# zhang-tao-whu/DVIS_Plus

Measured on AMD Instinct MI355X. Metric: frames/sec DVIS++ R50 offline, 720p T=30 synthetic, higher is better.
Workload: dtype f32 (storage, accumulation, results; the segmenter's dense layers - R50 convolutions from 128 channels on, pixel-decoder projections and FPN output convolution, the deformable encoder's projections and FFN, the decoder's key / value projections - multiply each fp32 operand as two f16 terms on the f1

## Files before the change

dvis_plus_amd/csrc/conv1x1_x3.hip:

```cpp
#include "dvis_common.h"
#include "x3_common.h"

DVIS_EXPORT int64_t dvis_conv_x3_image_bytes(int64_t N, int C, int H, int W);
DVIS_EXPORT int dvis_conv_x3_gn_fold_supported(int K, int G, int64_t HW);

namespace {

constexpr unsigned kOOB = 0x80000000u;

struct CxArgs {
  const float *x, *bias, *res;
  const void *wp;
  float *y;
  int N, C, K, relu, npass;
  int stride, W_in, OW, H_in;
  int taps;
  long long HW, HW_in, pixels;
  long long tiles;
  float xscale, inv;
  int *flag;
  int tag;
  const float *x2;
  int C2, stride2, W2_in;
  long long HW2_in;
// ... 193 lines not shown
              hi4[e] = a.in_relu ? fmaxf(t1, 0.f) : t1;
            }
            asm volatile("" : "+v"(lo4), "+v"(hi4));
            __builtin_amdgcn_sched_barrier(0);
          }
          split8(lo4, hi4, a.xscale, xh[s], xl[s]);
        }
        if constexpr (kAffine)
          if (kc + 1 == NC && more) load_tab(ntile);
        if (++cc == NCC) cc = 0, ++tap;
        const bool first = kc + 1 < NC1, sec = !first && kc + 1 < NC;
        const unsigned po = first ? cx_tap_offset(a, gm, tap) : (sec ? gm2 : cx_tap_offset(a, ngm, 0));
        load_raw(po, first ? cc : (sec ? kc + 1 - NC1 : 0), sec);
      }
#pragma unroll
      for (int part = 0; part < IPC; ++part) {
        const char *stage = ring.wait(false);
        ring.begin(ring.more() ? next_offset() : 0);
        mma_item<IK, NB, PW>(stage, lane, acc, xh + IK * part, xl + IK * part, [&](int i) { ring.piece(i); });
      }
    }
    float chk = 0.f;
    if constexpr (NB == 2 || IMGOUT) {
      if (a.img != nullptr) {
        const unsigned gs = (unsigned)(a.K / 64) * 8192u;
        const __amdgpu_buffer_rsrc_t ri = dvis_make_rsrc_uniform(a.img, (unsigned)((long long)a.N * a.OH * a.XG * gs));
        const __amdgpu_buffer_rsrc_t rb = dvis_make_rsrc_uniform(a.bias ? (const void *)a.bias : (const void *)a.img, a.bias ? (unsigned)a.K * 4u : 0u);
        unsigned ibase = kOOB;
        if (p < a.pixels) {
          const int pix = (int)(p - n * a.HW), oy = pix / a.OW, ox = pix - oy * a.OW;
          ibase = (unsigned)(((n * a.OH + oy) * a.XG + (ox >> 5)) * gs + (co0 / 64) * 8192 + g * 512 + (ox & 31) * 16);
        }
#pragma unroll
        for (int nb = 0; nb < NB; ++nb) {
          float v[16];
#pragma unroll
          for (int q = 0; q < 4; ++q) {
            const f4 b = __builtin_bit_cast(f4, __builtin_amdgcn_raw_buffer_load_b128(rb, (unsigned)(co0 + 32 * nb + 8 * q + 4 * g) * 4u, 0, 0));
#pragma unroll
            for (int i = 0; i < 4; ++i) {
              const float t = acc[nb][4 * q + i] * a.inv + b[i];
              chk = __builtin_fmaf(t, 0.f, chk);
              v[4 * q + i] = a.relu ? x3_relu(t) : t;
            }
          }
          h8 hi[2], lo[2];
#pragma unroll
          for (int u = 0; u < 2; ++u) {
            const f4 p0 = {v[8 * u], v[8 * u + 1], v[8 * u + 2], v[8 * u + 3]}, p1 = {v[8 * u + 4], v[8 * u + 5], v[8 * u + 6], v[8 * u + 7]};
            split8(p0, p1, a.oscale, hi[u], lo[u]);
          }
          const h8 ls = lo[0] + lo[1];
          chk = __builtin_fmaf((float)((ls[0] + ls[1]) + (ls[2] + ls[3]) + (ls[4] + ls[5]) + (ls[6] + ls[7])), 0.f, chk);
          store_fragments4(ri, ibase, hi[0], 4096 * nb, lo[0], 4096 * nb + 1024, hi[1], 4096 * nb + 2048, lo[1], 4096 * nb + 3072);
        }
        if (a.flag != nullptr && chk != chk && p < a.pixels) atomicCAS(a.flag, 0, a.tag);
        tile = ntile, pass = npass_, gm = ngm, gm2 = ngm2;
        continue;
      }
    }
    double gw[8], gw2[4], gw4[2], gtot = 0.0;
#pragma unroll
    for (int nb = 0; nb < NB; ++nb) {
      float rv[16];
      double gq[4];
#pragma unroll
      for (int r = 0; r < 16; ++r)
        rv[r] = a.res ? __builtin_bit_cast(float, __builtin_amdgcn_raw_buffer_load_b32(
                                                      rr, obase + (unsigned)(co0 + 32 * nb + 8 * (r >> 2) + 4 * g + (r & 3)) * ochan, 0, 0))
                      : 0.f;
#pragma unroll
      for (int q = 0; q < 4; ++q) {
        const int co = co0 + 32 * nb + 8 * q + 4 * g;
        f4 b = {0.f, 0.f, 0.f, 0.f};
        if (a.bias) b = *(const f4 *)(a.bias + co);
        double gsum = 0.0, gsq = 0.0;
#pragma unroll
        for (int i = 0; i < 4; ++i) {
          const unsigned o = obase + (unsigned)(co + i) * ochan;
          float v = acc[nb][4 * q + i] * a.inv + b[i] + rv[4 * q + i];
          chk = __builtin_fmaf(v, 0.f, chk);
          if (a.relu) v = x3_relu(v);
          __builtin_amdgcn_raw_buffer_store_b32(__builtin_bit_cast(unsigned, v), ry, o, 0, 0);
          if constexpr (kStats) {
            const double d = p < a.pixels ? (double)v : 0.0;
            gsum = i == 0 ? d : gsum + d;
            gsq = i == 0 ? d * d : __builtin_fma(d, d, gsq);
          }
        }
        if constexpr (kStats) gq[q] = cx_fold<5>(gsum, gsq, lane);
      }
      if constexpr (kStats) {
        gw[nb] = cx_fold<3>(cx_fold<4>(gq[0], gq[1], lane), cx_fold<4>(gq[2], gq[3], lane), lane);
        if (nb % 2 == 1) gw2[nb / 2] = cx_fold<2>(gw[nb - 1], gw[nb], lane);
        if (nb % 4 == 3) gw4[nb / 4] = cx_fold<1>(gw2[nb / 2 - 1], gw2[nb / 2], lane);
        if (nb == NB - 1) gtot = cx_fold<0>(gw4[0], gw4[1], lane);
      }
    }
    if constexpr (kStats) {
      const long long pw = tile * kTile + wave * 32;
      if (pw < a.pixels) {
        const long long nw = pw / a.HW, slot = (pw - nw * a.HW) >> 5;
        const int group = co0 / 8 + 4 * (((lane >> 2) & 1) + 2 * ((lane >> 1) & 1) + 4 * (lane & 1)) + ((lane >> 4) & 1) + 2 * ((lane >> 3) & 1);
        a.gn_part[((nw * (a.K / 8) + group) * a.slots + slot) * 2 + (lane >> 5)] = gtot;
      }
    }
    if (a.flag != nullptr && chk != chk && p < a.pixels) atomicCAS(a.flag, 0, a.tag);
    tile = ntile, pass = npass_, gm = ngm, gm2 = ngm2;
  }
}

__global__ __launch_bounds__(256) void upsample_add_image_kernel(const float *__restrict__ lateral, const float *__restrict__ top,
                                                                 void *__restrict__ img, int N, int C, int H, int W, int h, int w,
                                                                 const float *__restrict__ lat_scale, const float *__restrict__ lat_shift,
                                                                 float oscale) {
  const int NCC = C / 64, XG = (W + 31) / 32;
  const int cc = blockIdx.x, xg = blockIdx.y;
  const int x = threadIdx.x & 31, g = (threadIdx.x >> 5) & 1, S = threadIdx.x >> 6;
  const int px = 32 * xg + x;
  const float sy = (float)h / (float)H, sx = (float)w / (float)W;
  const int pxc = px < W ? px : W - 1;
  float fx = sx * ((float)pxc + 0.5f) - 0.5f;
  fx = fx < 0.f ? 0.f : fx;
  const int x0 = min((int)fx, w - 1), x1 = x0 + (x0 < w - 1 ? 1 : 0);
  const float lx1 = fx - (float)x0, lx0 = 1.f - lx1;
  const __amdgpu_buffer_rsrc_t ri = dvis_make_rsrc_uniform(img, (unsigned)((long long)N * H * XG * NCC * 8192));
  const unsigned rows = (unsigned)N * (unsigned)H;
  for (unsigned row = blockIdx.z * 16u; row < blockIdx.z * 16u + 16u && row < rows; ++row) {
    const unsigned n = row / (unsigned)H;
    const int y = (int)(row - n * (unsigned)H);
    float fy = sy * ((float)y + 0.5f) - 0.5f;
    fy = fy < 0.f ? 0.f : fy;
    const int y0 = min((int)fy, h - 1), y1 = y0 + (y0 < h - 1 ? 1 : 0);
    const float ly1 = fy - (float)y0, ly0 = 1.f - ly1;
    float v[8];
#pragma unroll
    for (int e = 0; e < 8; ++e) {
      const int c = 64 * cc + 32 * (S >> 1) + 16 * (S & 1) + 8 * (e >> 2) + 4 * g + (e & 3);
      const unsigned pl = n * (unsigned)C + (unsigned)c;
      const float *t0 = top + ((size_t)pl * h + y0) * (size_t)w, *t1 = top + ((size_t)pl * h + y1) * (size_t)w;
      float lat = lateral[((size_t)pl * H + y) * (size_t)W + pxc];
      if (lat_scale) lat = lat * lat_scale[pl] + lat_shift[pl];
      v[e] = lat + (ly0 * (lx0 * t0[x0] + lx1 * t0[x1]) + ly1 * (lx0 * t1[x0] + lx1 * t1[x1]));
    }
    const f4 p0 = {v[0], v[1], v[2], v[3]}, p1 = {v[4], v[5], v[6], v[7]};
    h8 hi, lo;
    split8(p0, p1, oscale, hi, lo);
    const unsigned G = row * (unsigned)XG + (unsigned)xg;
    const unsigned off = (G * (unsigned)NCC + (unsigned)cc) * 8192u + (unsigned)(S * 2048 + g * 512 + x * 16);
    store_fragments2(ri, off, hi, 0, lo, 1024);
  }
}

}

DVIS_EXPORT int dvis_upsample_add_image(const float *lateral, const float *lat_scale, const float *lat_shift, const float *top, void *image,
                                        int N, int C, int H, int W, int h, int w, int oexp, void *stream) {
  DVIS_REQUIRE(lateral && top && image, "dvis_upsample_add_image: null pointer");
  DVIS_REQUIRE((lat_scale == nullptr) == (lat_shift == nullptr), "dvis_upsample_add_image: scale and shift together");
  DVIS_REQUIRE(N > 0 && C > 0 && C % 64 == 0 && H > 0 && W > 0 && h > 0 && w > 0, "dvis_upsample_add_image: bad sizes");
  DVIS_REQUIRE((uintptr_t)image % 16 == 0 && dvis_conv_x3_image_bytes(N, C, H, W) < ((int64_t)1 << 31), "dvis_upsample_add_image: a 16-byte "
               "aligned image below 2 GiB");
  const int per = 16 * 65535 / H;
  DVIS_REQUIRE(per >= 1 && (W + 31) / 32 <= 65535, "dvis_upsample_add_image: map too large (%d x %d)", H, W);
  for (int i = 0; i < N; i += per) {
    const int n = N - i < per ? N - i : per;
    hipLaunchKernelGGL(upsample_add_image_kernel, dim3(C / 64, (W + 31) / 32, (n * H + 15) / 16), dim3(256), 0, (hipStream_t)stream,
                       lateral + (size_t)i * C * H * W, top + (size_t)i * C * h * w,
                       (char *)image + (size_t)i * H * ((W + 31) / 32) * (C / 64) * 8192, n, C, H, W, h, w,
                       lat_scale ? lat_scale + (size_t)i * C : nullptr, lat_shift ? lat_shift + (size_t)i * C : nullptr, ldexpf(1.f, oexp));
  }
  return dvis_check_launch("dvis_upsample_add_image");
}

DVIS_EXPORT int dvis_conv1x1_x3_supported(int C, int K, int64_t N, int64_t HW_in, int64_t HW_out) {
  if (C < 64 || C % 64 != 0 || C > 4096) return 0;
  if (!(K == 64 || K == 128 || (K > 0 && K % 256 == 0 && K <= 8192))) return 0;
  if (N <= 0 || HW_out <= 0 || HW_in < HW_out) return 0;
  if (N * C * HW_in * 4 >= ((int64_t)1 << 31) || N * K * HW_out * 4 >= ((int64_t)1 << 31)) return 0;
  return 1;
}

DVIS_EXPORT int64_t dvis_conv1x1_x3_packed_bytes(int C, int K) {
  if (!dvis_conv1x1_x3_supported(C, K, 1, 1, 1)) return -1;
  return (int64_t)(C / 16) * (K / 32) * 2 * kPiece;
}

DVIS_EXPORT int dvis_conv1x1_x3_pack(const float *w, int K, int C, int wexp, void *packed, void *stream) {
  DVIS_REQUIRE(w && packed, "dvis_conv1x1_x3_pack: null operand");
  DVIS_REQUIRE(dvis_conv1x1_x3_supported(C, K, 1, 1, 1), "dvis_conv1x1_x3_pack: (C, K) = (%d, %d) is not served", C, K);
  DVIS_REQUIRE(wexp >= -60 && wexp <= 60, "dvis_conv1x1_x3_pack: wexp = %d", wexp);
  const int NB = K == 64 ? 2 : K == 128 ? 4 : 8;
  const int64_t fragments = (int64_t)(C / 16) * (K / 32) * 64;
  hipLaunchKernelGGL(x3_pack_kernel, dim3((unsigned)((fragments + 255) / 256)), dim3(256), 0, (hipStream_t)stream, w, (int64_t)C, K, C,
                     NB, 0, ldexpf(1.f, wexp), (_Float16 *)packed, fragments);
  return dvis_check_launch("dvis_conv1x1_x3_pack");
}

struct CxFold {
  double *gn_part;
  const float *in_scale, *in_shift;
  int in_relu;
};

static int cx_launch(const float *x, const void *packed, const float *bias, const float *res, float *y, int N, int C, int K, int H, int W,
                     int stride, int taps, int xexp, int wexp, int relu, void *stream, const float *x2 = nullptr, int C2 = 0, int H2 = 0,
                     int W2 = 0, int stride2 = 1, void *image = nullptr, int oexp = 0, const void *ximg = nullptr,
                     const CxFold *fold = nullptr);

DVIS_EXPORT int dvis_conv1x1_x3_dual(const float *x, const float *x2, const void *packed, const float *bias, const float *res, float *y,
                                     int N, int C, int C2, int K, int H, int W, int H2, int W2, int stride2, int xexp, int wexp, int relu,
                                     void *stream) {
  DVIS_REQUIRE(x2 != nullptr && C2 >= 64 && C2 % 64 == 0 && C2 <= 4096, "dvis_conv1x1_x3_dual: C2 %% 64 == 0 (got %d)", C2);
  DVIS_REQUIRE((stride2 == 1 || stride2 == 2) && (H2 + stride2 - 1) / stride2 == H && (W2 + stride2 - 1) / stride2 == W,
               "dvis_conv1x1_x3_dual: x2 (%d x %d, stride %d) must down-sample onto x's %d x %d map", H2, W2, stride2, H, W);
  DVIS_REQUIRE((long long)N * C2 * H2 * W2 * 4 < ((long long)1 << 31) && (uintptr_t)x2 % 16 == 0, "dvis_conv1x1_x3_dual: x2 below 2 GiB, 16-byte aligned");
  return cx_launch(x, packed, bias, res, y, N, C, K, H, W, 1, 1, xexp, wexp, relu, stream, x2, C2, H2, W2, stride2);
}

DVIS_EXPORT int dvis_conv1x1_x3(const float *x, const void *packed, const float *bias, const float *res, float *y, int N, int C, int K,
                                int H, int W, int stride, int xexp, int wexp, int relu, void *stream, const float *in_scale,
                                const float *in_shift, int in_relu, double *gn_part) {
  DVIS_REQUIRE((in_scale == nullptr) == (in_shift == nullptr), "dvis_conv1x1_x3: in_scale and in_shift together");
  const CxFold fold = {gn_part, in_scale, in_shift, in_relu};
  return cx_launch(x, packed, bias, res, y, N, C, K, H, W, stride, 1, xexp, wexp, relu, stream, nullptr, 0, 0, 0, 1, nullptr, 0, nullptr,
                   (gn_part || in_scale) ? &fold : nullptr);
}

DVIS_EXPORT int dvis_conv_x3_gn_fold_supported(int K, int G, int64_t HW) {
  return K > 0 && K % 256 == 0 && G > 0 && K == 8 * G && HW > 0 && HW % 32 == 0;
}

DVIS_EXPORT int dvis_conv1x1_x3_image(const float *x, const void *packed, const float *bias, void *image, int N, int C, int H, int W, int xexp,
                                      int wexp, int oexp, int relu, void *stream) {
  DVIS_REQUIRE(image != nullptr && (uintptr_t)image % 16 == 0, "dvis_conv1x1_x3_image: null / unaligned image");
  DVIS_REQUIRE((long long)N * H * ((W + 31) / 32) * 8192 < ((long long)1 << 31), "dvis_conv1x1_x3_image: the image must stay below 2 GiB");
  return cx_launch(x, packed, bias, nullptr, nullptr, N, C, 64, H, W, 1, 1, xexp, wexp, relu, stream, nullptr, 0, 0, 0, 1, image, oexp);
}

DVIS_EXPORT int64_t dvis_conv_x3_image_bytes(int64_t N, int C, int H, int W) {
  if (N < 0 || C <= 0 || C % 64 != 0 || H <= 0 || W <= 0) return -1;
  return N * H * ((W + 31) / 32) * (int64_t)(C / 64) * 8192;
}

DVIS_EXPORT int dvis_conv_x3_pack_image(const float *w, int K, int C, int taps, int wexp, void *packed, void *stream) {
  DVIS_REQUIRE(w && packed, "dvis_conv_x3_pack_image: null operand");
  DVIS_REQUIRE(taps == 1 || taps == 9, "dvis_conv_x3_pack_image: taps = %d", taps);
  DVIS_REQUIRE(dvis_conv1x1_x3_supported(C, K, 1, 1, 1) && K >= 128, "dvis_conv_x3_pack_image: (C, K) = (%d, %d) is not served", C, K);
  DVIS_REQUIRE(wexp >= -60 && wexp <= 60, "dvis_conv_x3_pack_image: wexp = %d", wexp);
  const int NB = K == 128 ? 4 : 8;
  const int64_t fragments = (int64_t)(taps * C / 16) * (K / 32) * 64;
  hipLaunchKernelGGL(x3_pack_kernel, dim3((unsigned)((fragments + 255) / 256)), dim3(256), 0, (hipStream_t)stream, w, (int64_t)taps * C, K,
                     taps * C, NB, 1, ldexpf(1.f, wexp), (_Float16 *)packed, fragments, taps);
  return dvis_check_launch("dvis_conv_x3_pack_image");
}

DVIS_EXPORT int dvis_conv_x3_image(const void *ximg, const float *x, const void *packed, const float *bias, const float *res, float *y,
                                   void *image, int N, int C, int K, int H, int W, int stride, int taps, int xexp, int wexp, int oexp, int relu,
                                   void *stream, double *gn_part) {
  DVIS_REQUIRE(ximg != nullptr || image != nullptr, "dvis_conv_x3_image: neither side is an operand image (use dvis_conv1x1_x3 / dvis_conv3x3_x3)");
  DVIS_REQUIRE((ximg != nullptr) != (x != nullptr), "dvis_conv_x3_image: exactly one of ximg and x");
  DVIS_REQUIRE((image != nullptr) != (y != nullptr), "dvis_conv_x3_image: exactly one of image and y");
  DVIS_REQUIRE(K == 128 || K % 256 == 0, "dvis_conv_x3_image: K = %d (128 or a multiple of 256)", K);
  DVIS_REQUIRE(taps == 1 || taps == 9, "dvis_conv_x3_image: taps = %d", taps);
  DVIS_REQUIRE(image == nullptr || res == nullptr, "dvis_conv_x3_image: an image output takes no residual");
  DVIS_REQUIRE(((uintptr_t)ximg | (uintptr_t)image) % 16 == 0, "dvis_conv_x3_image: images must be 16-byte aligned");
  const int OH = (H + stride - 1) / stride, OW = (W + stride - 1) / stride;
  DVIS_REQUIRE(dvis_conv_x3_image_bytes(N, C, H, W) < ((int64_t)1 << 31) && dvis_conv_x3_image_bytes(N, K, OH, OW) < ((int64_t)1 << 31),
               "dvis_conv_x3_image: images must stay below 2 GiB");
  DVIS_REQUIRE(gn_part == nullptr || (ximg != nullptr && y != nullptr), "dvis_conv_x3_image: statistics with an image in and an fp32 map out");
  const CxFold fold = {gn_part, nullptr, nullptr, 0};
  return cx_launch(x, packed, bias, res, y, N, C, K, H, W, stride, taps, xexp, wexp, relu, stream, nullptr, 0, 0, 0, 1, image, oexp, ximg,
                   gn_part ? &fold : nullptr);
}

DVIS_EXPORT int64_t dvis_conv3x3_x3_packed_bytes(int C, int K) {
  const int64_t b = dvis_conv1x1_x3_packed_bytes(C, K);
  return b < 0 ? b : 9 * b;
}

DVIS_EXPORT int dvis_conv3x3_x3_pack(const float *w, int K, int C, int wexp, void *packed, void *stream) {
  DVIS_REQUIRE(w && packed, "dvis_conv3x3_x3_pack: null operand");
  DVIS_REQUIRE(dvis_conv1x1_x3_supported(C, K, 1, 1, 1), "dvis_conv3x3_x3_pack: (C, K) = (%d, %d) is not served", C, K);
  DVIS_REQUIRE(wexp >= -60 && wexp <= 60, "dvis_conv3x3_x3_pack: wexp = %d", wexp);
  const int NB = K == 64 ? 2 : K == 128 ? 4 : 8;
  const int64_t fragments = (int64_t)(9 * C / 16) * (K / 32) * 64;
  hipLaunchKernelGGL(x3_pack_kernel, dim3((unsigned)((fragments + 255) / 256)), dim3(256), 0, (hipStream_t)stream, w, (int64_t)9 * C, K, 9 * C,
                     NB, 0, ldexpf(1.f, wexp), (_Float16 *)packed, fragments, 9);
  return dvis_check_launch("dvis_conv3x3_x3_pack");
}

DVIS_EXPORT int dvis_conv3x3_x3(const float *x, const void *packed, const float *bias, const float *res, float *y, int N, int C, int K,
                                int H, int W, int stride, int xexp, int wexp, int relu, void *stream) {
  return cx_launch(x, packed, bias, res, y, N, C, K, H, W, stride, 9, xexp, wexp, relu, stream);
}

static int cx_launch(const float *x, const void *packed, const float *bias, const float *res, float *y, int N, int C, int K, int H, int W,
                     int stride, int taps, int xexp, int wexp, int relu, void *stream, const float *x2, int C2, int H2, int W2, int stride2,
                     void *image, int oexp, const void *ximg, const CxFold *fold) {
  DVIS_REQUIRE((x || ximg) && packed && (y || image), "dvis_conv1x1_x3: null operand");
  DVIS_REQUIRE(stride == 1 || stride == 2, "dvis_conv1x1_x3: stride %d", stride);
  const int OH = (H + stride - 1) / stride, OW = (W + stride - 1) / stride;
  DVIS_REQUIRE(dvis_conv1x1_x3_supported(C, K, N, (int64_t)H * W, (int64_t)OH * OW), "dvis_conv1x1_x3: shape (N %d, C %d, K %d, %d x %d, "
               "stride %d) is not served (C %% 64 == 0, K = 64 / 128 or K %% 256 == 0, tensors below 2 GiB)", N, C, K, H, W, stride);
  DVIS_REQUIRE((uintptr_t)x % 16 == 0 && (uintptr_t)y % 16 == 0 && (uintptr_t)packed % 16 == 0 && (bias == nullptr || (uintptr_t)bias % 16 == 0),
               "dvis_conv1x1_x3: operands must be 16-byte aligned");
  CxArgs a = {};
  a.x = x, a.bias = bias, a.res = res, a.wp = packed, a.y = y, a.N = N, a.C = C, a.K = K, a.relu = relu;
  a.stride = stride, a.W_in = W, a.H_in = H, a.taps = taps, a.OW = OW, a.HW = (long long)OH * OW, a.HW_in = (long long)H * W;
  a.pixels = a.HW * N;
  a.xscale = ldexpf(1.f, xexp), a.inv = ldexpf(1.f, -(xexp + wexp));
  const X3Guard gd = dvis_x3_guard();
  a.flag = gd.flag, a.tag = gd.tag;
  a.x2 = x2, a.C2 = x2 ? C2 : 0, a.stride2 = stride2, a.W2_in = W2, a.HW2_in = (long long)H2 * W2;
  a.img = image, a.XG = (OW + 31) / 32, a.oscale = ldexpf(1.f, oexp), a.OH = OH;
// ... 75 lines not shown
```

dvis_plus_amd/csrc/gemm_x3.hip:

```cpp
#define DVIS_X3_DMA_MUBUF 1
#include "dvis_common.h"
#include "x3_common.h"

#include <stdlib.h>

namespace {

template <int KS>
__device__ __forceinline__ void load_x(const float *x, int64_t ldx, int64_t row, int g, float s, h8 *xh, h8 *xl,
                                       const float *addp = nullptr) {
  const float *p = x + row * ldx + 8 * g;
  f4 raw[2 * KS];
#pragma unroll
  for (int S = 0; S < KS; ++S) raw[2 * S] = *(const f4 *)(p + 16 * S), raw[2 * S + 1] = *(const f4 *)(p + 16 * S + 4);
  if (addp != nullptr) {
#pragma unroll
    for (int S = 0; S < KS; ++S) raw[2 * S] += *(const f4 *)(addp + 16 * S), raw[2 * S + 1] += *(const f4 *)(addp + 16 * S + 4);
  }
#pragma unroll
  for (int S = 0; S < KS; ++S) split8(raw[2 * S], raw[2 * S + 1], s, xh[S], xl[S]);
}

__device__ __forceinline__ void store_block(char *scr, int lane, const f4 *v, float *dst, int64_t ld, int rows_valid,
                                            const float *radd = nullptr, int64_t ldr = 0) {
  const int j = lane & 31, g = lane >> 5, sw = (j >> 1) & 7;
#pragma unroll
  for (int q = 0; q < 4; ++q) *(f4 *)(scr + j * 128 + (((2 * q + g) ^ sw) << 4)) = v[q];
  __builtin_amdgcn_wave_barrier();
#pragma unroll
  for (int t = 0; t < 4; ++t) {
    const int jr = 8 * t + (lane >> 3), pp = lane & 7;
    f4 o = *(const f4 *)(scr + jr * 128 + ((pp ^ ((jr >> 1) & 7)) << 4));
    if (radd != nullptr && jr < rows_valid) o += *(const f4 *)(radd + jr * ldr + 4 * pp);
    if (jr < rows_valid) *(f4 *)(dst + jr * ld + 4 * pp) = o;
  }
  __builtin_amdgcn_wave_barrier();
}

struct EpiArgs {
  const float *bias;
  const float *res;
  int64_t ldres;
  const float *gamma, *beta;
  float eps;
  const float *pos;
  int64_t pos_rows;
  float *out, *out2;
  int64_t ldo;
  float inv;
  int relu;
  const float *radd;
  int *flag;
  int tag;
};

template <int NB, bool LN, bool EX = false>
__device__ __forceinline__ void epilogue(f16v *acc, const EpiArgs &e, const float *cb, const float *cg, const float *cbeta, char *scr,
                                         int lane, int64_t tok0, int64_t M, int col0 = 0) {
  const int j = lane & 31, g = lane >> 5;
  const int64_t tok = tok0 + j < M ? tok0 + j : M - 1;
  const int rows_valid = M - tok0 < 32 ? (int)(M - tok0) : 32;
  constexpr int N = 32 * NB;
  float mean = 0.f, rstd = 1.f;
  if constexpr (LN) {
    const float *rp = e.res + tok * e.ldres + 4 * g;
    f4 r[2][4];
    auto fetch = [&](int nb, f4 *dst) {
#pragma unroll
      for (int q = 0; q < 4; ++q) dst[q] = *(const f4 *)(rp + 32 * nb + 8 * q);
    };
    fetch(0, r[0]);
    float sum = 0.f;
#pragma unroll
    for (int nb = 0; nb < NB; ++nb) {
      if (nb + 1 < NB) fetch(nb + 1, r[(nb + 1) & 1]);
#pragma unroll
      for (int q = 0; q < 4; ++q) {
        const f4 b = *(const f4 *)(cb + 32 * nb + 8 * q + 4 * g);
#pragma unroll
        for (int i = 0; i < 4; ++i) {
          const float v = acc[nb][4 * q + i] * e.inv + b[i] + r[nb & 1][q][i];
          acc[nb][4 * q + i] = v;
          sum += v;
        }
      }
    }
    sum += __shfl_xor(sum, 32);
    if (e.flag != nullptr && !(fabsf(sum) <= 3.4028235e38f)) atomicCAS(e.flag, 0, e.tag);
    mean = sum * (1.f / N);
    float sq = 0.f;
#pragma unroll
    for (int nb = 0; nb < NB; ++nb)
#pragma unroll
      for (int i = 0; i < 16; ++i) {
        const float d = acc[nb][i] - mean;
        sq += d * d;
      }
    sq += __shfl_xor(sq, 32);
    rstd = rsqrtf(sq * (1.f / N) + e.eps);
  }
  float chk = 0.f;
  const float *pr = nullptr;
  f4 pv[2][4];
  auto fetch_pos = [&](int nb, f4 *dst) {
#pragma unroll
    for (int q = 0; q < 4; ++q) dst[q] = *(const f4 *)(pr + 32 * nb + 8 * q);
  };
  if constexpr (LN) {
    if (e.pos != nullptr) {
      pr = e.pos + (tok % e.pos_rows) * N + 4 * g;
      fetch_pos(0, pv[0]);
    }
  }
#pragma unroll
  for (int nb = 0; nb < NB; ++nb) {
    f4 v[4];
    if constexpr (LN) {
      if (e.pos != nullptr && nb + 1 < NB) fetch_pos(nb + 1, pv[(nb + 1) & 1]);
    }
#pragma unroll
    for (int q = 0; q < 4; ++q) {
      const int n = 32 * nb + 8 * q + 4 * g;
      if constexpr (LN) {
        const f4 ga = *(const f4 *)(cg + n), be = *(const f4 *)(cbeta + n);
#pragma unroll
        for (int i = 0; i < 4; ++i) v[q][i] = (acc[nb][4 * q + i] - mean) * rstd * ga[i] + be[i];
      } else {
        const f4 b = *(const f4 *)(cb + n);
#pragma unroll
        for (int i = 0; i < 4; ++i) {
          const float t = acc[nb][4 * q + i] * e.inv + b[i];
          chk = __builtin_fmaf(t, 0.f, chk);
          if constexpr (EX)
            v[q][i] = e.relu == 1 ? x3_relu(t) : e.relu == 2 ? 0.5f * t * (1.f + erff(t * 0.70710678118654752440f)) : t;
          else
            v[q][i] = e.relu ? x3_relu(t) : t;
        }
      }
    }
    if constexpr (!EX)
      store_block(scr, lane, v, e.out + tok0 * e.ldo + col0 + 32 * nb, e.ldo, rows_valid);
    else
      store_block(scr, lane, v, e.out + tok0 * e.ldo + col0 + 32 * nb, e.ldo, rows_valid,
                  e.radd ? e.radd + tok0 * e.ldres + col0 + 32 * nb : nullptr, e.ldres);
    if constexpr (LN) {
      if (e.pos != nullptr) {
#pragma unroll
        for (int q = 0; q < 4; ++q) v[q] += pv[nb & 1][q];
        store_block(scr, lane, v, e.out2 + tok0 * e.ldo + 32 * nb, e.ldo, rows_valid);
      }
    }
  }
  if constexpr (!LN) {
    if (e.flag != nullptr && chk != chk) atomicCAS(e.flag, 0, e.tag);
  }
}

template <int NB>
__global__ __launch_bounds__(kThreads) void x3_linear_kernel(const float *__restrict__ x, int64_t ldx, int64_t M,
                                                             const void *__restrict__ wp, float xscale, int npass,
                                                             const float *__restrict__ xadd, int64_t xadd_rows, EpiArgs e) {
  extern __shared__ __attribute__((aligned(1024))) char lds[];
  constexpr int K = 256, KS = K / 16, NI = K / 32;
  const int wave = threadIdx.x >> 6, lane = threadIdx.x & 63, j = lane & 31, g = lane >> 5;
  const int64_t ntiles = (M + kTileTok - 1) / kTileTok;
  const int64_t my = blockIdx.x < ntiles ? (ntiles - blockIdx.x + gridDim.x - 1) / gridDim.x : 0;
  Ring<NB> ring;
  ring.start(wp, lds, NI * npass, (int)(my * NI * npass), wave, lane);
  char *scr = lds + kStages * Ring<NB>::kItemBytes + wave * kScratch;
  float *cst = (float *)(lds + kStages * Ring<NB>::kItemBytes + kWaves * kScratch);
  const int ntot = 32 * NB * npass;
  for (int i = threadIdx.x; i < ntot; i += kThreads) cst[i] = e.bias ? e.bias[i] : 0.f;
  __syncthreads();
  for (int64_t tile = blockIdx.x; tile < ntiles; tile += gridDim.x) {
    const int64_t tok0 = tile * kTileTok + wave * 32;
    const int64_t row = tok0 + j < M ? tok0 + j : M - 1;
    h8 xh[KS], xl[KS];
    load_x<KS>(x, ldx, row, g, xscale, xh, xl, xadd ? xadd + (row % xadd_rows) * K + 8 * g : nullptr);
    for (int pass = 0; pass < npass; ++pass) {
      f16v acc[NB];
#pragma unroll
      for (int nb = 0; nb < NB; ++nb)
#pragma unroll
        for (int i = 0; i < 16; ++i) acc[nb][i] = 0.f;
#pragma unroll
      for (int c = 0; c < NI; ++c) {
        const char *stage = ring.wait(c == 0);
        ring.begin_periodic();
        mma_item<2, NB, NB>(stage, lane, acc, xh + 2 * c, xl + 2 * c, [&](int i) { ring.piece(i); });
      }
      if (tok0 < M) epilogue<NB, false>(acc, e, cst + pass * 32 * NB, cst + ntot, cst + ntot + 32 * NB, scr, lane, tok0, M, pass * 32 * NB);
    }
  }
}

constexpr int x3_stream_layout_blocks(int nb) { return 4 * nb % 8 == 0 ? nb : nb + 1; }

template <int NB, bool LN, bool EX = false, bool ADD = false>
__global__ __launch_bounds__(512) void x3_linear_stream_kernel(const float *__restrict__ x, int64_t ldx, int64_t M, int K,
                                                               const void *__restrict__ wp, float xscale, int npass,
                                                               const float *__restrict__ xadd, int64_t xadd_rows, EpiArgs e) {
  extern __shared__ __attribute__((aligned(1024))) char lds[];
  constexpr int NBL = x3_stream_layout_blocks(NB);
  constexpr int NW = 8, PW = 4 * NBL / NW, kTile = NW * 32;
  typedef Ring<PW, 8, NW> RingT;
  const int wave = threadIdx.x >> 6, lane = threadIdx.x & 63, j = lane & 31, g = lane >> 5;
  const int NI = K / 32, NC = K / 64;
  const int64_t ntiles = (M + kTile - 1) / kTile;
  const int64_t my = blockIdx.x < ntiles ? (ntiles - blockIdx.x + gridDim.x - 1) / gridDim.x : 0;
  if (my == 0) return;
  RingT ring;
  ring.start(wp, lds, NI * npass, (int)(my * NI * npass), wave, lane);
  char *scr = lds + kStages * RingT::kItemBytes + wave * kScratch;
  float *cst = (float *)(lds + kStages * RingT::kItemBytes + NW * kScratch);
  const int ntot = 32 * NB * npass;
  for (int i = threadIdx.x; i < ntot; i += 512) cst[i] = e.bias ? e.bias[i] : 0.f;
  if constexpr (LN)
    for (int i = threadIdx.x; i < 32 * NB; i += 512) cst[ntot + i] = e.gamma[i], cst[ntot + 32 * NB + i] = e.beta[i];
  __syncthreads();
  auto products = [&](const char *stage, f16v *acc, const h8 *xh, const h8 *xl) {
    if constexpr (NBL == NB) {
      mma_item<2, NB, PW>(stage, lane, acc, xh, xl, [&](int i) { ring.piece(i); });
    } else {
      mma_item<1, NB, 3>(stage, lane, acc, xh, xl, [&](int i) { ring.piece(i); });
      mma_item<1, NB, PW - 3>(stage + NBL * 2 * kPiece, lane, acc, xh + 1, xl + 1, [&](int i) { ring.piece(3 + i); });
    }
  };
  auto row_of = [&](int64_t tile) {
    const int64_t t = tile * kTile + wave * 32 + j;
    return t < M ? t : M - 1;
  };
  if constexpr (ADD) {
    f4 raw[4], rawp[4];
    auto load_raw = [&](const float *rowp, const float *posp, int it) {
#pragma unroll
      for (int s = 0; s < 2; ++s) {
        raw[2 * s] = *(const f4 *)(rowp + 32 * it + 16 * s), raw[2 * s + 1] = *(const f4 *)(rowp + 32 * it + 16 * s + 4);
        rawp[2 * s] = *(const f4 *)(posp + 32 * it + 16 * s), rawp[2 * s + 1] = *(const f4 *)(posp + 32 * it + 16 * s + 4);
      }
    };
    int64_t r0 = row_of(blockIdx.x);
    const float *rowp = x + r0 * ldx + 8 * g, *posp = xadd + (r0 % xadd_rows) * K + 8 * g;
    load_raw(rowp, posp, 0);
    for (int64_t tile = blockIdx.x; tile < ntiles; tile += gridDim.x) {
      const int64_t tok0 = tile * kTile + wave * 32;
      const int64_t rn = row_of(tile + gridDim.x < ntiles ? tile + gridDim.x : tile);
      const float *nrowp = x + rn * ldx + 8 * g, *nposp = xadd + (rn % xadd_rows) * K + 8 * g;
      for (int pass = 0; pass < npass; ++pass) {
        f16v acc[NB];
#pragma unroll
        for (int nb = 0; nb < NB; ++nb)
#pragma unroll
          for (int i = 0; i < 16; ++i) acc[nb][i] = 0.f;
        for (int it = 0; it < NI; ++it) {
#pragma unroll
          for (int i = 0; i < 4; ++i) asm volatile("" : "+v"(raw[i]), "+v"(rawp[i]));
          h8 xh[2], xl[2];
#pragma unroll
          for (int s = 0; s < 2; ++s) split8(raw[2 * s] + rawp[2 * s], raw[2 * s + 1] + rawp[2 * s + 1], xscale, xh[s], xl[s]);
          if (it + 1 < NI)
            load_raw(rowp, posp, it + 1);
          else if (pass + 1 < npass)
            load_raw(rowp, posp, 0);
          else
            load_raw(nrowp, nposp, 0);
          const char *stage = ring.wait(false);
          ring.begin_periodic();
          products(stage, acc, xh, xl);
        }
        if (tok0 < M) epilogue<NB, LN, EX>(acc, e, cst + pass * 32 * NB, cst + ntot, cst + ntot + 32 * NB, scr, lane, tok0, M, pass * 32 * NB);
      }
      rowp = nrowp, posp = nposp;
    }
    return;
  }
  f4 raw[8];
  auto load_raw = [&](const float *rowp, int kc) {
#pragma unroll
    for (int s = 0; s < 4; ++s) raw[2 * s] = *(const f4 *)(rowp + 64 * kc + 16 * s), raw[2 * s + 1] = *(const f4 *)(rowp + 64 * kc + 16 * s + 4);
  };
  auto row_ptr = [&](int64_t tile) { return x + row_of(tile) * ldx + 8 * g; };
  const float *rowp = row_ptr(blockIdx.x);
  load_raw(rowp, 0);
  for (int64_t tile = blockIdx.x; tile < ntiles; tile += gridDim.x) {
    const int64_t tok0 = tile * kTile + wave * 32;
    const float *nrowp = row_ptr(tile + gridDim.x < ntiles ? tile + gridDim.x : tile);
    for (int pass = 0; pass < npass; ++pass) {
      f16v acc[NB];
#pragma unroll
      for (int nb = 0; nb < NB; ++nb)
#pragma unroll
        for (int i = 0; i < 16; ++i) acc[nb][i] = 0.f;
      for (int kc = 0; kc < NC; ++kc) {
#pragma unroll
        for (int i = 0; i < 8; ++i) asm volatile("" : "+v"(raw[i]));
        h8 xh[4], xl[4];
#pragma unroll
        for (int s = 0; s < 4; ++s) split8(raw[2 * s], raw[2 * s + 1], xscale, xh[s], xl[s]);
        if (kc + 1 < NC)
          load_raw(rowp, kc + 1);
        else
          load_raw(pass + 1 < npass ? rowp : nrowp, 0);
#pragma unroll
        for (int half = 0; half < 2; ++half) {
          const char *stage = ring.wait(false);
          ring.begin_periodic();
          products(stage, acc, xh + 2 * half, xl + 2 * half);
        }
      }
      if (tok0 < M) epilogue<NB, LN, EX>(acc, e, cst + pass * 32 * NB, cst + ntot, cst + ntot + 32 * NB, scr, lane, tok0, M, pass * 32 * NB);
    }
    rowp = nrowp;
  }
}

struct FfnArgs {
  const float *b1;
  float inv1, hscale;
  int HB;
};

__global__ __launch_bounds__(kThreads) void x3_ffn_kernel(const float *__restrict__ x, int64_t ldx, int64_t M,
                                                          const void *__restrict__ wp, float xscale, FfnArgs f, EpiArgs e) {
  extern __shared__ __attribute__((aligned(1024))) char lds[];
  constexpr int KS = 16;
  const int wave = threadIdx.x >> 6, lane = threadIdx.x & 63, j = lane & 31, g = lane >> 5;
  const int64_t ntiles = (M + kTileTok - 1) / kTileTok;
  const int64_t my = blockIdx.x < ntiles ? (ntiles - blockIdx.x + gridDim.x - 1) / gridDim.x : 0;
  const int per_tile = 8 * f.HB;
  Ring<8> ring;
  ring.start(wp, lds, per_tile, (int)(my * per_tile), wave, lane);
  char *scr = lds + kStages * Ring<8>::kItemBytes + wave * kScratch;
  float *b1s = (float *)(lds + kStages * Ring<8>::kItemBytes + kWaves * kScratch);
  for (int i = threadIdx.x; i < 128 * f.HB; i += kThreads) b1s[i] = f.b1[i];
  float *cst = b1s + 128 * f.HB;
  for (int i = threadIdx.x; i < 256; i += kThreads) cst[i] = e.bias[i], cst[256 + i] = e.gamma[i], cst[512 + i] = e.beta[i];
  __syncthreads();
  for (int64_t tile = blockIdx.x; tile < ntiles; tile += gridDim.x) {
    const int64_t tok0 = tile * kTileTok + wave * 32;
    const int64_t row = tok0 + j < M ? tok0 + j : M - 1;
    h8 xh[KS], xl[KS];
    load_x<KS>(x, ldx, row, g, xscale, xh, xl);
    f16v acc2[8];
#pragma unroll
    for (int nb = 0; nb < 8; ++nb)
#pragma unroll
      for (int i = 0; i < 16; ++i) acc2[nb][i] = 0.f;
    for (int hb = 0; hb < f.HB; ++hb) {
      f16v acc1[4];
#pragma unroll
      for (int t = 0; t < 4; ++t)
#pragma unroll
        for (int i = 0; i < 16; ++i) acc1[t][i] = 0.f;
      h8 hh[8], hl[8];
      f2 cv = {0.f, 0.f};
      auto convert = [&](int tc, int t) {
        const int pair = t >> 1, u = pair >> 2, pp = pair & 3;
        if ((t & 1) == 0) {
          const f2 b = *(const f2 *)(b1s + 128 * hb + 32 * tc + 16 * u + 8 * (pp >> 1) + 4 * g + 2 * (pp & 1));
          cv[0] = x3_relu(acc1[tc][8 * u + 2 * pp] * f.inv1 + b[0]) * f.hscale;
          cv[1] = x3_relu(acc1[tc][8 * u + 2 * pp + 1] * f.inv1 + b[1]) * f.hscale;
        } else {
          const h2 h = __builtin_convertvector(cv, h2);
          const f2 r = cv - __builtin_convertvector(h, f2);
          const h2 l = __builtin_convertvector(r, h2);
          hh[2 * tc + u][2 * pp] = h.x, hh[2 * tc + u][2 * pp + 1] = h.y;
          hl[2 * tc + u][2 * pp] = l.x, hl[2 * tc + u][2 * pp + 1] = l.y;
        }
      };
#pragma unroll
      for (int c = 0; c < 4; ++c) {
        const char *stage = ring.wait(hb == 0 && c == 0);
        ring.begin_periodic();
        mma_item<16, 1, 8>(stage, lane, acc1 + c, xh, xl, [&](int i) { ring.piece(i); }, [&](int t) {
          if (c > 0) convert(c - 1, t);
        });
      }
#pragma unroll
      for (int c = 0; c < 4; ++c) {
        const char *stage = ring.wait(false);
        ring.begin_periodic();
        if (c == 0) {
          mma_item<2, 8, 8>(stage, lane, acc2, hh, hl, [&](int i) { ring.piece(i); }, [&](int t) { convert(3, t); });
        } else {
          mma_item<2, 8, 8>(stage, lane, acc2, hh + 2 * c, hl + 2 * c, [&](int i) { ring.piece(i); });
        }
      }
    }
    if (tok0 < M) epilogue<8, true>(acc2, e, cst, cst + 256, cst + 512, scr, lane, tok0, M);
  }
}

__global__ void x3_ffn_pack_kernel(const float *w1, int64_t ldw1, const float *w2, int64_t ldw2, int H, float s1, float s2,
                                   _Float16 *out, int64_t fragments) {
  const int64_t idx = (int64_t)blockIdx.x * blockDim.x + threadIdx.x;
  if (idx >= fragments) return;
  const int lane = idx & 63;
  int64_t t = idx >> 6;
  const int fr = t & 15;
  t >>= 4;
  const int item = t & 7, hb = t >> 3;
  _Float16 *o = out + (((int64_t)hb * 8 + item) * 16 + fr) * 1024 + lane * 8;
  if (item < 4) {
    x3_pack_fragment(w1, ldw1, H, 256, 128 * hb + 32 * item + (lane & 31), 0, fr, lane >> 5, s1, o, o + 512);
  } else {
    const int s = fr >> 3, nb = fr & 7;
    x3_pack_fragment(w2, ldw2, 256, H, 32 * nb + (lane & 31), 1, 8 * hb + 2 * (item - 4) + s, lane >> 5, s2, o, o + 512);
  }
}

int x3_grid(int64_t ntiles) {
  const int cus = dvis_x3_persistent_cus();
  return (int)(ntiles < cus ? ntiles : cus);
}

float x3_pow2(int e) { return ldexpf(1.f, e); }

template <typename Kern, typename... Args>
int x3_launch(Kern kern, DvisLdsOptIn *opted, size_t lds_bytes, int64_t M, hipStream_t st, const char *what, Args... args) {
  const int rc = dvis_lds_opt_in((const void *)kern, lds_bytes, opted, what);
  if (rc != DVIS_OK) return rc;
  const int64_t ntiles = (M + kTileTok - 1) / kTileTok;
  hipLaunchKernelGGL(kern, dim3(x3_grid(ntiles)), dim3(kThreads), lds_bytes, st, args...);
  return dvis_check_launch(what);
}

int x3_check_common(const float *x, int64_t ldx, int64_t M, const void *wp, const float *out, int64_t ldo) {
  DVIS_REQUIRE(x && wp && out, "dvis_x3: null operand");
  DVIS_REQUIRE(M >= 0 && M < (int64_t)1 << 31, "dvis_x3: M = %lld out of range", (long long)M);
  DVIS_REQUIRE(ldx % 4 == 0 && ldo % 4 == 0 && (uintptr_t)x % 16 == 0 && (uintptr_t)out % 16 == 0 && (uintptr_t)wp % 16 == 0,
               "dvis_x3: operands must be 16-byte aligned with row strides %% 4 == 0");
  return DVIS_OK;
}

}

static int x3_passes(int N, int *nb) {
  if (N == 128 || N == 192 || N == 256 || N == 288) return *nb = N / 32, 1;
  if (N > 0 && N % 256 == 0 && N <= 8192) return *nb = 8, N / 256;
  return *nb = 0, 0;
}

static int g_x3_reserve = [] {
  const char *e = getenv("DVIS_X3_RESERVE");
  const int r = e ? atoi(e) : 0;
  return r < 0 ? 0 : r / 8 * 8;
}();

int dvis_x3_persistent_cus() {
  int dev = 0, cus = 256;
  if (hipGetDevice(&dev) == hipSuccess) {
    int v = 0;
    if (hipDeviceGetAttribute(&v, hipDeviceAttributeMultiprocessorCount, dev) == hipSuccess && v >= 8) cus = v;
  }
  cus = cus / 8 * 8;
  const int r = __atomic_load_n(&g_x3_reserve, __ATOMIC_RELAXED);
  return cus - r >= 8 ? cus - r : cus;
}

DVIS_EXPORT int dvis_x3_set_reserve(int cus) {
  const int r = cus < 0 ? 0 : cus / 8 * 8;
  return __atomic_exchange_n(&g_x3_reserve, r, __ATOMIC_RELAXED);
}

static int *g_x3_flag[64] = {};
static thread_local int t_x3_tag = 1;

X3Guard dvis_x3_guard() {
  int dev = 0;
  if (hipGetDevice(&dev) != hipSuccess || dev < 0 || dev >= 64) return X3Guard{nullptr, 0};
  return X3Guard{__atomic_load_n(&g_x3_flag[dev], __ATOMIC_RELAXED), t_x3_tag};
}

DVIS_EXPORT int dvis_x3_set_range_flag(int32_t *flag) {
  int dev = 0;
  if (hipGetDevice(&dev) != hipSuccess || dev < 0 || dev >= 64) {
    dvis_set_error("dvis_x3_set_range_flag: no current device");
    return DVIS_E_ARG;
  }
  __atomic_store_n(&g_x3_flag[dev], (int *)flag, __ATOMIC_RELAXED);
  return DVIS_OK;
}

DVIS_EXPORT int dvis_x3_set_tag(int tag) {
  const int prev = t_x3_tag;
  t_x3_tag = tag > 0 ? tag : 1;
  return prev;
}

DVIS_EXPORT int dvis_x3_linear_supported(int N, int K, int ln) {
  int nb;
  if (K < 64 || K % 64 != 0 || K > 8192) return 0;
  if (ln) return N == 256;
  if (N == 288) return K == 256;
  return x3_passes(N, &nb) > 0;
}

DVIS_EXPORT int64_t dvis_x3_packed_bytes(int N, int K) {
  if (!dvis_x3_linear_supported(N, K, 0)) return -1;
  int NB;
  const int npass = x3_passes(N, &NB);
  return (int64_t)(K / 16) * npass * x3_stream_layout_blocks(NB) * 2 * kPiece;
}

DVIS_EXPORT int dvis_x3_pack(const float *w, int64_t ldw, int N, int K, int wexp, void *packed, void *stream) {
  DVIS_REQUIRE(w && packed, "dvis_x3_pack: null operand");
  DVIS_REQUIRE(dvis_x3_linear_supported(N, K, 0), "dvis_x3_pack: (N, K) = (%d, %d) is not served (K %% 64 == 0; N in 128 / 192 / 256 or N %% 256 == 0; N = 288 at K = 256)", N, K);
  DVIS_REQUIRE(wexp >= -60 && wexp <= 60, "dvis_x3_pack: wexp = %d", wexp);
  int NB;
  const int npass = x3_passes(N, &NB);
  const int NBL = x3_stream_layout_blocks(NB);
  const int64_t fragments = (int64_t)(K / 16) * npass * NBL * 64;
  hipLaunchKernelGGL(x3_pack_kernel, dim3((unsigned)((fragments + 255) / 256)), dim3(256), 0, (hipStream_t)stream, w, ldw, N, K,
                     NBL, 0, x3_pow2(wexp), (_Float16 *)packed, fragments);
  return dvis_check_launch("dvis_x3_pack");
}

static int x3_linear_impl(const float *x, int64_t ldx, int64_t M, int K, const void *wp, int N, int xexp, int wexp, const float *xadd,
                          int64_t xadd_rows, const float *bias, int relu, float *out, int64_t ldo, void *stream,
                          const float *radd = nullptr, int64_t ldr = 0);

DVIS_EXPORT int dvis_x3_linear(const float *x, int64_t ldx, int64_t M, int K, const void *wp, int N, int xexp, int wexp,
                               const float *bias, int relu, float *out, int64_t ldo, void *stream) {
  return x3_linear_impl(x, ldx, M, K, wp, N, xexp, wexp, nullptr, 0, bias, relu, out, ldo, stream);
}

DVIS_EXPORT int dvis_x3_linear_add(const float *x, int64_t ldx, int64_t M, int K, const void *wp, int N, int xexp, int wexp,
                                   const float *xadd, int64_t xadd_rows, const float *bias, int relu, float *out, int64_t ldo,
                                   void *stream) {
  DVIS_REQUIRE(xadd && xadd_rows > 0 && (uintptr_t)xadd % 16 == 0, "dvis_x3_linear_add: xadd (xadd_rows x K, 16-byte aligned) is required");
  DVIS_REQUIRE(K == 256 && dvis_x3_linear_supported(N, K, 0), "dvis_x3_linear_add: served for K = 256 (N %d, K %d)", N, K);
  return x3_linear_impl(x, ldx, M, K, wp, N, xexp, wexp, xadd, xadd_rows, bias, relu, out, ldo, stream);
}

DVIS_EXPORT int dvis_x3_linear_res(const float *x, int64_t ldx, int64_t M, int K, const void *wp, int N, int xexp, int wexp,
                                   const float *bias, int act, const float *res, int64_t ldres, float *out, int64_t ldo, void *stream) {
  DVIS_REQUIRE(act >= 0 && act <= 2, "dvis_x3_linear_res: act must be 0 (none), 1 (ReLU) or 2 (GELU)");
  DVIS_REQUIRE(res == nullptr || ((uintptr_t)res % 16 == 0 && ldres % 4 == 0 && ldres >= N),
               "dvis_x3_linear_res: res must be 16-byte aligned with a row stride that is a multiple of 4 floats and >= N");
  return x3_linear_impl(x, ldx, M, K, wp, N, xexp, wexp, nullptr, 0, bias, act, out, ldo, stream, res, ldres);
}

static int x3_linear_impl(const float *x, int64_t ldx, int64_t M, int K, const void *wp, int N, int xexp, int wexp, const float *xadd,
                          int64_t xadd_rows, const float *bias, int relu, float *out, int64_t ldo, void *stream, const float *radd,
                          int64_t ldr) {
  DVIS_REQUIRE(dvis_x3_linear_supported(N, K, 0), "dvis_x3_linear: (N, K) = (%d, %d) is not served (K %% 64 == 0; N in 128 / 192 / 256 or N %% 256 == 0; N = 288 at K = 256)", N, K);
  const int rc = x3_check_common(x, ldx, M, wp, out, ldo);
  if (rc != DVIS_OK) return rc;
  if (M == 0) return DVIS_OK;
  EpiArgs e = {};
  e.bias = bias, e.out = out, e.ldo = ldo, e.inv = x3_pow2(-(xexp + wexp)), e.relu = relu;
  e.radd = radd, e.ldres = ldr;
  const X3Guard gd = dvis_x3_guard();
  e.flag = gd.flag, e.tag = gd.tag;
  const float xs = x3_pow2(xexp);
  hipStream_t st = (hipStream_t)stream;
  int NB;
  const int npass = x3_passes(N, &NB);
#define DVIS_X3_STREAM_FORM(NBV, LNV, EXV, ADDV, XADD, XROWS, WHAT, LDS_EXTRA)                                        \
  {                                                                                                                  \
    static DvisLdsOptIn opted;                                                                                       \
    typedef Ring<4 * x3_stream_layout_blocks(NBV) / 8, 8, 8> R;                                                      \
    const size_t lds_bytes = kStages * R::kItemBytes + 8 * kScratch + (LDS_EXTRA);                                   \
    const int rc2 = dvis_lds_opt_in((const void *)x3_linear_stream_kernel<NBV, LNV, EXV, ADDV>, lds_bytes, &opted, WHAT);  \
    if (rc2 != DVIS_OK) return rc2;                                                                                  \
    const int64_t ntiles = (M + 255) / 256;                                                                          \
    hipLaunchKernelGGL((x3_linear_stream_kernel<NBV, LNV, EXV, ADDV>), dim3(x3_grid(ntiles)), dim3(512), lds_bytes, st, x, ldx, M, K, wp, \
                       xs, npass, XADD, XROWS, e);                                                                   \
    return dvis_check_launch(WHAT);                                                                                  \
  }
#define DVIS_X3_STREAM_EX(NBV, LNV, EXV, WHAT, LDS_EXTRA) DVIS_X3_STREAM_FORM(NBV, LNV, EXV, false, (const float *)nullptr, (int64_t)0, WHAT, LDS_EXTRA)
#define DVIS_X3_STREAM(NBV, LNV, WHAT, LDS_EXTRA) DVIS_X3_STREAM_EX(NBV, LNV, false, WHAT, LDS_EXTRA)
#define DVIS_X3_RESIDENT(NBV)                                                                                        \
  {                                                                                                                  \
    static DvisLdsOptIn opted;                                                                                       \
    return x3_launch(x3_linear_kernel<NBV>, &opted, kStages * Ring<NBV>::kItemBytes + kWaves * kScratch + (size_t)N * 4, \
                     M, st, "dvis_x3_linear", x, ldx, M, wp, xs, npass, xadd, xadd_rows, e);                         \
  }
  if (relu == 2 || radd) {
    DVIS_REQUIRE(NB == 8 && !xadd, "dvis_x3_linear_res: the GELU / residual epilogue is served for N %% 256 == 0 (N = %d)", N);
    DVIS_X3_STREAM_EX(8, false, true, "dvis_x3_linear_res", (size_t)N * 4)
  }
  if (xadd) {
    switch (NB) {
      case 4: DVIS_X3_RESIDENT(4)
      case 6: DVIS_X3_RESIDENT(6)
      case 8: DVIS_X3_RESIDENT(8)
      default: DVIS_X3_STREAM_FORM(9, false, false, true, xadd, xadd_rows, "dvis_x3_linear_add", (size_t)N * 4)
    }
  }
  switch (NB) {
    case 4: DVIS_X3_STREAM(4, false, "dvis_x3_linear", (size_t)N * 4)
    case 6: DVIS_X3_STREAM(6, false, "dvis_x3_linear", (size_t)N * 4)
    case 8: DVIS_X3_STREAM(8, false, "dvis_x3_linear", (size_t)N * 4)
    default: DVIS_X3_STREAM(9, false, "dvis_x3_linear", (size_t)N * 4)
  }
#undef DVIS_X3_RESIDENT
}

DVIS_EXPORT int dvis_x3_linear_ln(const float *x, int64_t ldx, int64_t M, int K, const void *wp, int N, int xexp, int wexp,
                                  const float *bias, const float *res, int64_t ldres, const float *gamma, const float *beta,
                                  float eps, const float *pos, int64_t pos_rows, float *out, float *out2, int64_t ldo,
                                  void *stream) {
  DVIS_REQUIRE(dvis_x3_linear_supported(N, K, 1), "dvis_x3_linear_ln: (N, K) = (%d, %d) is not served (256, 256)", N, K);
  DVIS_REQUIRE(bias && res && gamma && beta, "dvis_x3_linear_ln: bias, res, gamma, beta are required");
  DVIS_REQUIRE(ldres % 4 == 0 && (uintptr_t)res % 16 == 0, "dvis_x3_linear_ln: res must be 16-byte aligned, ldres %% 4 == 0");
  DVIS_REQUIRE(pos == nullptr || (out2 && pos_rows > 0 && (uintptr_t)pos % 16 == 0 && (uintptr_t)out2 % 16 == 0),
               "dvis_x3_linear_ln: pos needs out2, pos_rows > 0 and 16-byte alignment");
  const int rc = x3_check_common(x, ldx, M, wp, out, ldo);
  if (rc != DVIS_OK) return rc;
  if (M == 0) return DVIS_OK;
  EpiArgs e = {};
  e.bias = bias, e.res = res, e.ldres = ldres, e.gamma = gamma, e.beta = beta, e.eps = eps, e.pos = pos, e.pos_rows = pos_rows;
  e.out = out, e.out2 = out2, e.ldo = ldo, e.inv = x3_pow2(-(xexp + wexp));
  const X3Guard gd = dvis_x3_guard();
  e.flag = gd.flag, e.tag = gd.tag;
  const float xs = x3_pow2(xexp);
  const int npass = 1;
  hipStream_t st = (hipStream_t)stream;
  DVIS_X3_STREAM(8, true, "dvis_x3_linear_ln", (size_t)3 * 256 * 4)
#undef DVIS_X3_STREAM
#undef DVIS_X3_STREAM_EX
#undef DVIS_X3_STREAM_FORM
}

DVIS_EXPORT int64_t dvis_x3_ffn_packed_bytes(int K, int H, int N) {
  if (K != 256 || N != 256 || H <= 0 || H % 128 != 0 || H > 4096) return -1;
  return (int64_t)(H / 128) * 8 * Ring<8>::kItemBytes;
}

DVIS_EXPORT int dvis_x3_ffn_pack(const float *w1, int64_t ldw1, const float *w2, int64_t ldw2, int K, int H, int N, int w1exp,
                                 int w2exp, void *packed, void *stream) {
  DVIS_REQUIRE(w1 && w2 && packed, "dvis_x3_ffn_pack: null operand");
  DVIS_REQUIRE(dvis_x3_ffn_packed_bytes(K, H, N) > 0, "dvis_x3_ffn_pack: needs K = N = 256, H %% 128 == 0 (K %d, H %d, N %d)", K, H, N);
  const int64_t fragments = (int64_t)(H / 128) * 8 * 16 * 64;
  hipLaunchKernelGGL(x3_ffn_pack_kernel, dim3((unsigned)((fragments + 255) / 256)), dim3(256), 0, (hipStream_t)stream, w1, ldw1,
                     w2, ldw2, H, x3_pow2(w1exp), x3_pow2(w2exp), (_Float16 *)packed, fragments);
  return dvis_check_launch("dvis_x3_ffn_pack");
}

DVIS_EXPORT int dvis_x3_ffn_ln(const float *x, int64_t ldx, int64_t M, int K, int H, int N, const void *wp, int xexp, int w1exp,
                               int hexp, int w2exp, const float *b1, const float *b2, const float *gamma, const float *beta,
                               float eps, const float *pos, int64_t pos_rows, float *out, float *out2, int64_t ldo,
                               void *stream) {
  DVIS_REQUIRE(dvis_x3_ffn_packed_bytes(K, H, N) > 0, "dvis_x3_ffn_ln: needs K = N = 256, H %% 128 == 0 (K %d, H %d, N %d)", K, H, N);
  DVIS_REQUIRE(b1 && b2 && gamma && beta, "dvis_x3_ffn_ln: biases, gamma, beta are required");
  DVIS_REQUIRE(pos == nullptr || (out2 && pos_rows > 0 && (uintptr_t)pos % 16 == 0 && (uintptr_t)out2 % 16 == 0),
               "dvis_x3_ffn_ln: pos needs out2, pos_rows > 0 and 16-byte alignment");
  const int rc = x3_check_common(x, ldx, M, wp, out, ldo);
  if (rc != DVIS_OK) return rc;
  if (M == 0) return DVIS_OK;
  EpiArgs e = {};
  e.bias = b2, e.res = x, e.ldres = ldx, e.gamma = gamma, e.beta = beta, e.eps = eps, e.pos = pos, e.pos_rows = pos_rows;
  e.out = out, e.out2 = out2, e.ldo = ldo, e.inv = x3_pow2(-(hexp + w2exp));
  const X3Guard gd = dvis_x3_guard();
  e.flag = gd.flag, e.tag = gd.tag;
  FfnArgs f = {b1, x3_pow2(-(xexp + w1exp)), x3_pow2(hexp), H / 128};
  static DvisLdsOptIn opted;
  return x3_launch(x3_ffn_kernel, &opted, kStages * Ring<8>::kItemBytes + kWaves * kScratch + (size_t)(H + 3 * 256) * 4, M,
                   (hipStream_t)stream, "dvis_x3_ffn_ln", x, ldx, M, wp, x3_pow2(xexp), f, e);
}
```

dvis_plus_amd/functions.py:

```python
import collections
import ctypes
import math
import os
import threading

import torch
from torch.autograd import Function
from torch.autograd.function import once_differentiable

from . import cpu_ops, derived, native
from .cpu_ops import ms_deform_attn_core_pytorch


def _torch_path(op, x, why):
    if os.environ.get("DVIS_STRICT", "1") != "0" and x.is_cuda and not torch.is_grad_enabled():
        raise RuntimeError(f"DVIS_STRICT: {op} would run its torch formulation on a GPU tensor ({why}; shape "
                           f"{tuple(x.shape)}, dtype {x.dtype}, contiguous {x.is_contiguous()})")


class no_autocast:

    def __enter__(self):
        import contextlib
        self._stack = contextlib.ExitStack()
# ... 1569 lines not shown
        return n


def _rows_image_buffer(M, K, device):
    nbytes = native.lib().dvis_x3_rows_image_bytes(M, K)
    if nbytes < 0:
        raise RuntimeError(f"row image: K % 32 == 0 is required (K {K})")
    return torch.empty(nbytes, dtype=torch.uint8, device=device)


def x3_rows_image(x, xexp=None):
    K = x.shape[-1]
    x2, ldx = _x3_rows(x, "x")
    e = X3_XEXP if xexp is None else xexp
    buf = _rows_image_buffer(x2.shape[0], K, x.device)
    with torch.cuda.device(x.device):
        native.check(native.lib().dvis_x3_rows_image(ctypes.c_void_p(x2.data_ptr()), ldx, x2.shape[0], K, e, ctypes.c_void_p(buf.data_ptr()),
                                                     native.stream_ptr(x.device)), "dvis_x3_rows_image")
    return RowImage(buf, x.shape, e, 0)


def layer_norm_rows_image_ok(x, norm):
    C = x.shape[-1]
    return (X3_ROW_IMAGES and x3_on() and x.is_cuda and x.dtype == torch.float32 and x.is_contiguous() and x.data_ptr() % 16 == 0
            and C % 32 == 0 and C <= 1024 and norm.weight is not None and norm.bias is not None and not torch.is_grad_enabled()
            and not torch.is_autocast_enabled())


def layer_norm_rows_image(x, norm, xexp=None):
    C = x.shape[-1]
    M = x.numel() // C
    e = X3_XEXP if xexp is None else xexp
    buf = _rows_image_buffer(M, C, x.device)
    with torch.cuda.device(x.device):
        native.check(native.lib().dvis_layernorm_rows_image(
            ctypes.c_void_p(x.data_ptr()), native.dev_ptr(norm.weight, "gamma"), native.dev_ptr(norm.bias, "beta"), M, C, float(norm.eps), e,
            ctypes.c_void_p(buf.data_ptr()), native.stream_ptr(x.device)), "dvis_layernorm_rows_image")
    return RowImage(buf, x.shape, e, 0)


def x3_tile_linear(x, weight, bias, act=None, residual=None, xexp=None):
    N, K = weight.shape
    if isinstance(x, RowImage):
        return _x3_tile_linear_image(x, weight, bias, act, residual)
    x2, ldx = _x3_rows(x, "x")
    buf, wexp = x3_tile_pack(weight)
    out = torch.empty((*x.shape[:-1], N), dtype=torch.float32, device=x.device)
    rptr, ldr = None, 0
    if residual is not None:
        if residual.shape != out.shape or residual.dtype != torch.float32 or not residual.is_cuda:
            raise RuntimeError("x3_tile_linear: residual must be a float32 GPU tensor of the output's shape")
        r2, ldr = _rows2d(residual, N)
        rptr = ctypes.c_void_p(r2.data_ptr())
    with torch.cuda.device(x.device):
        native.check(native.lib().dvis_x3_tile_linear(
            ctypes.c_void_p(x2.data_ptr()), ldx, x2.shape[0], K, ctypes.c_void_p(buf.data_ptr()), N,
            X3_XEXP if xexp is None else xexp, wexp, None if bias is None else native.dev_ptr(bias.detach(), "bias"),
            {None: 0, "relu": 1, "gelu": 2}[act], rptr, ldr, ctypes.c_void_p(out.data_ptr()), N, native.stream_ptr(x.device)),
            "dvis_x3_tile_linear")
    return out


def _x3_tile_linear_image(img, weight, bias, act, residual):
    N, K = weight.shape
    if img.shape[-1] != K:
        raise RuntimeError(f"x3_tile_linear: image of {img.shape} rows against a weight of {tuple(weight.shape)}")
    M = img.rows
    buf, wexp = x3_tile_pack(weight, img.order)
    bptr = None if bias is None else native.dev_ptr(bias.detach(), "bias")
    lib = native.lib()
    with torch.cuda.device(img.device):
        if act == "gelu":
            if residual is not None:
                raise RuntimeError("x3_tile_linear: the GELU form of a row image writes a row image (no residual)")
            out = _rows_image_buffer(M, N, img.device)
            native.check(lib.dvis_x3_tile_linear_image(ctypes.c_void_p(img.data.data_ptr()), M, K, ctypes.c_void_p(buf.data_ptr()), N, img.exp, wexp,
                                                       bptr, 2, None, 0, None, 0, ctypes.c_void_p(out.data_ptr()), X3_XEXP,
                                                       native.stream_ptr(img.device)), "dvis_x3_tile_linear_image")
            return RowImage(out, (*img.shape[:-1], N), X3_XEXP, 1)
        out = torch.empty((*img.shape[:-1], N), dtype=torch.float32, device=img.device)
        rptr, ldr = None, 0
        if residual is not None:
            if residual.shape != out.shape or residual.dtype != torch.float32 or not residual.is_cuda:
                raise RuntimeError("x3_tile_linear: residual must be a float32 GPU tensor of the output's shape")
            r2, ldr = _rows2d(residual, N)
            rptr = ctypes.c_void_p(r2.data_ptr())
        native.check(lib.dvis_x3_tile_linear_image(ctypes.c_void_p(img.data.data_ptr()), M, K, ctypes.c_void_p(buf.data_ptr()), N, img.exp, wexp,
                                                   bptr, {None: 0, "relu": 1}[act], rptr, ldr, ctypes.c_void_p(out.data_ptr()), N, None, 0,
                                                   native.stream_ptr(img.device)), "dvis_x3_tile_linear_image")
    return out


X3_QKV_FUSED = os.environ.get("DVIS_X3_QKV_FUSED", "1") != "0"


def x3_qkv_attention_ok(x, weight, heads):
    if isinstance(x, RowImage):
        if len(x.shape) != 3 or not (X3_QKV_FUSED and weight.dim() == 2 and weight._base is None):
            return False
        B, L, C = x.shape
        return (C == heads * 64 and weight.shape == (3 * C, C) and L >= 1024 and C >= X3_TILE_MIN_K
                and bool(native.lib().dvis_x3_tile_supported(3 * C, C)))
    if not (X3_QKV_FUSED and x.dim() == 3 and x.is_cuda and x.dtype == torch.float32 and not torch.is_grad_enabled()
            and not torch.is_autocast_enabled() and x3_on() and weight.dim() == 2 and weight._base is None):
        return False
    B, L, C = x.shape
    return (C == heads * 64 and weight.shape == (3 * C, C) and L >= 1024 and x.is_contiguous() and x.data_ptr() % 16 == 0
            and x3_tile_ok(x, 3 * C, C))


def x3_qkv_attention(x, weight, bias, heads, out_image=False):
    B, L, C = x.shape
    image_in = isinstance(x, RowImage)
    buf, wexp = x3_tile_pack(weight, x.order if image_in else 0)
    lib = native.lib()
    nbytes = lib.dvis_attention_ws_bytes_k(B * heads, L, L, 64, 2)
    ws = torch.empty((nbytes + 3) // 4, dtype=torch.float32, device=x.device)
    qscale = (1.0 / 8.0) * 1.4426950408889634 * 16.0
    bptr = None if bias is None else native.dev_ptr(bias.detach(), "bias")
    with torch.cuda.device(x.device):
        if image_in:
            native.check(lib.dvis_x3_tile_linear_qkv_image(
                ctypes.c_void_p(x.data.data_ptr()), B * L, C, ctypes.c_void_p(buf.data_ptr()), 3 * C, x.exp, wexp, bptr, heads, L, qscale,
                ctypes.c_void_p(ws.data_ptr()), native.stream_ptr(x.device)), "dvis_x3_tile_linear_qkv_image")
        else:
            native.check(lib.dvis_x3_tile_linear_qkv(
                ctypes.c_void_p(x.data_ptr()), C, B * L, C, ctypes.c_void_p(buf.data_ptr()), 3 * C, X3_XEXP, wexp, bptr, heads, L, qscale,
                ctypes.c_void_p(ws.data_ptr()), native.stream_ptr(x.device)), "dvis_x3_tile_linear_qkv")
        if out_image:
            out = _rows_image_buffer(B * L, C, x.device)
            native.check(lib.dvis_attention_x3_packed_image(ctypes.c_void_p(ws.data_ptr()), ctypes.c_void_p(out.data_ptr()), B, heads, L, X3_XEXP,
                                                            native.stream_ptr(x.device)), "dvis_attention_x3_packed_image")
            return RowImage(out, (B, L, C), X3_XEXP, 2)
        out = torch.empty((B, L, C), dtype=torch.float32, device=x.device)
        strides = (ctypes.c_int64 * 3)(L * C, 64, C)
        native.check(lib.dvis_attention_x3_packed(ctypes.c_void_p(ws.data_ptr()), ctypes.c_void_p(out.data_ptr()), strides, B, heads, L,
                                                  native.stream_ptr(x.device)), "dvis_attention_x3_packed")
    return out


def x3_ok(x, N, K, ln=False, add=False):
    return (x.is_cuda and x.dtype == torch.float32 and not torch.is_grad_enabled() and x.shape[-1] == K
            and (not add or K == 256) and bool(native.lib().dvis_x3_linear_supported(N, K, int(ln))))


def _x3_rows(x, name):
    K = x.shape[-1]
    x2, ld = _rows2d(x, K)
    if x2.data_ptr() % 16 or ld % 4:
        raise RuntimeError(f"x3: {name} must be 16-byte aligned with a row stride % 4 == 0")
    return x2, ld


def x3_linear(x, weight, bias, relu=False, xexp=None, xadd=None, act=None, residual=None):
    N, K = weight.shape
    x2, ldx = _x3_rows(x, "x")
    buf, wexp = x3_pack(weight)
    out = torch.empty((*x.shape[:-1], N), dtype=torch.float32, device=x.device)
    if act is not None or residual is not None:
        if xadd is not None:
            raise RuntimeError("x3_linear: xadd and act / residual are served by different entry points")
        code = {None: int(bool(relu)), "relu": 1, "gelu": 2}[act]
        rptr, ldr = None, 0
        if residual is not None:
            if residual.shape != out.shape or residual.dtype != torch.float32 or not residual.is_cuda:
                raise RuntimeError("x3_linear: residual must be a float32 GPU tensor of the output's shape")
            r2, ldr = _x3_rows(residual, "residual")
            rptr = ctypes.c_void_p(r2.data_ptr())
        with torch.cuda.device(x.device):
            native.check(native.lib().dvis_x3_linear_res(
                ctypes.c_void_p(x2.data_ptr()), ldx, x2.shape[0], K, ctypes.c_void_p(buf.data_ptr()), N,
                X3_XEXP if xexp is None else xexp, wexp, None if bias is None else native.dev_ptr(bias.detach(), "bias"), code,
                rptr, ldr, ctypes.c_void_p(out.data_ptr()), N, native.stream_ptr(x.device)), "dvis_x3_linear_res")
        return out
    if xadd is not None:
        if x.dim() != 3 or xadd.numel() != x.shape[1] * K or xadd.dtype != torch.float32 or not xadd.is_cuda:
            raise RuntimeError("x3_linear: xadd must be a float32 GPU (S, K) embedding for x of shape (B, S, K)")
        xadd = xadd.contiguous()
        with torch.cuda.device(x.device):
            native.check(native.lib().dvis_x3_linear_add(
                ctypes.c_void_p(x2.data_ptr()), ldx, x2.shape[0], K, ctypes.c_void_p(buf.data_ptr()), N,
                X3_XEXP if xexp is None else xexp, wexp, ctypes.c_void_p(xadd.data_ptr()), x.shape[1],
                None if bias is None else native.dev_ptr(bias.detach(), "bias"), int(relu), ctypes.c_void_p(out.data_ptr()), N,
                native.stream_ptr(x.device)), "dvis_x3_linear_add")
        return out
    with torch.cuda.device(x.device):
        native.check(native.lib().dvis_x3_linear(
            ctypes.c_void_p(x2.data_ptr()), ldx, x2.shape[0], K, ctypes.c_void_p(buf.data_ptr()), N,
            X3_XEXP if xexp is None else xexp, wexp, None if bias is None else native.dev_ptr(bias.detach(), "bias"), int(relu),
            ctypes.c_void_p(out.data_ptr()), N, native.stream_ptr(x.device)), "dvis_x3_linear")
    return out


def _x3_pos(pos, x, N):
    if pos is None:
        return None, 0, None
    if x.dim() != 3 or pos.numel() != x.shape[1] * N or pos.dtype != torch.float32 or not pos.is_cuda:
        raise RuntimeError("x3: pos must be a float32 GPU (S, C) embedding for x of shape (N, S, C)")
    return pos.contiguous(), x.shape[1], torch.empty((*x.shape[:-1], N), dtype=torch.float32, device=x.device)


def x3_linear_ln(x, weight, bias, res, norm, pos=None, xexp=None):
    N, K = weight.shape
    x2, ldx = _x3_rows(x, "x")
    r2, ldr = _x3_rows(res, "res")
    buf, wexp = x3_pack(weight)
    out = torch.empty((*x.shape[:-1], N), dtype=torch.float32, device=x.device)
    pos, pos_rows, out2 = _x3_pos(pos, x, N)
    with torch.cuda.device(x.device):
        native.check(native.lib().dvis_x3_linear_ln(
            ctypes.c_void_p(x2.data_ptr()), ldx, x2.shape[0], K, ctypes.c_void_p(buf.data_ptr()), N,
            X3_XEXP if xexp is None else xexp, wexp, native.dev_ptr(bias.detach(), "bias"), ctypes.c_void_p(r2.data_ptr()), ldr,
            native.dev_ptr(norm.weight.detach(), "gamma"), native.dev_ptr(norm.bias.detach(), "beta"), float(norm.eps),
            None if pos is None else ctypes.c_void_p(pos.data_ptr()), pos_rows, ctypes.c_void_p(out.data_ptr()),
            None if out2 is None else ctypes.c_void_p(out2.data_ptr()), N, native.stream_ptr(x.device)), "dvis_x3_linear_ln")
    return out if out2 is None else (out, out2)


def x3_ffn_ok(x, lin1, lin2):
    K, H, N = lin1.weight.shape[1], lin1.weight.shape[0], lin2.weight.shape[0]
    return (x.is_cuda and x.dtype == torch.float32 and not torch.is_grad_enabled() and x.shape[-1] == K
            and lin2.weight.shape[1] == H and lin1.bias is not None and lin2.bias is not None
            and native.lib().dvis_x3_ffn_packed_bytes(K, H, N) > 0)


def x3_ffn_ln(x, lin1, lin2, norm, pos=None, xexp=None, hexp=None):
    w1, w2 = lin1.weight, lin2.weight
    H, K = w1.shape
    N = w2.shape[0]
    x2, ldx = _x3_rows(x, "x")

    def make():
        a, b = w1.detach().contiguous(), w2.detach().contiguous()
        e1, e2 = _x3_wexp(a), _x3_wexp(b)
        buf = torch.empty(native.lib().dvis_x3_ffn_packed_bytes(K, H, N), dtype=torch.uint8, device=a.device)
        with torch.cuda.device(a.device):
            native.check(native.lib().dvis_x3_ffn_pack(ctypes.c_void_p(a.data_ptr()), K, ctypes.c_void_p(b.data_ptr()), H, K, H,
                                                       N, e1, e2, ctypes.c_void_p(buf.data_ptr()),
                                                       native.stream_ptr(a.device)), "dvis_x3_ffn_pack")
        return buf, e1, e2
    buf, e1, e2 = _x3_cache(w1, [w1, w2], make, kind="ffn")
    out = torch.empty((*x.shape[:-1], N), dtype=torch.float32, device=x.device)
    pos, pos_rows, out2 = _x3_pos(pos, x, N)
    with torch.cuda.device(x.device):
        native.check(native.lib().dvis_x3_ffn_ln(
            ctypes.c_void_p(x2.data_ptr()), ldx, x2.shape[0], K, H, N, ctypes.c_void_p(buf.data_ptr()),
            X3_XEXP if xexp is None else xexp, e1, X3_XEXP if hexp is None else hexp, e2,
            native.dev_ptr(lin1.bias.detach(), "b1"), native.dev_ptr(lin2.bias.detach(), "b2"),
            native.dev_ptr(norm.weight.detach(), "gamma"), native.dev_ptr(norm.bias.detach(), "beta"), float(norm.eps),
            None if pos is None else ctypes.c_void_p(pos.data_ptr()), pos_rows, ctypes.c_void_p(out.data_ptr()),
            None if out2 is None else ctypes.c_void_p(out2.data_ptr()), N, native.stream_ptr(x.device)), "dvis_x3_ffn_ln")
    return out if out2 is None else (out, out2)


def maps_to_tokens(maps, affines=None, pos=None):
    affines = affines or [None] * len(maps)
    N, C = maps[0].shape[:2]
    if not all(m.is_cuda and m.dtype == torch.float32 and m.is_contiguous() for m in maps) or torch.is_grad_enabled():
        _torch_path("maps_to_tokens", maps[0], "needs contiguous fp32 NCHW maps")
        maps = [m if a is None else m * a[0].view(N, C, 1, 1) + a[1].view(N, C, 1, 1) for m, a in zip(maps, affines)]
        out = torch.cat([m.flatten(2).transpose(1, 2) for m in maps], 1)
        return out if pos is None else (out, out + pos.reshape(1, -1, C))
    S = sum(m.shape[2] * m.shape[3] for m in maps)
    out = torch.empty((N, S, C), dtype=torch.float32, device=maps[0].device)
    out_pos = pp = None
    if pos is not None:
        if pos.numel() != S * C or pos.dtype != torch.float32 or not pos.is_cuda:
            raise RuntimeError("maps_to_tokens: pos must be a float32 GPU (S, C) embedding")
        pos = pos.contiguous()
        out_pos = torch.empty_like(out)
        pp = native.dev_ptr(pos, "pos")
    row0 = 0
    with torch.cuda.device(out.device):
        for m, a in zip(maps, affines):
            HW = m.shape[2] * m.shape[3]
            rc = native.lib().dvis_nchw_to_tokens_affine(
                ctypes.c_void_p(m.data_ptr()), None if a is None else native.dev_ptr(a[0], "scale"),
                None if a is None else native.dev_ptr(a[1], "shift"), pp, ctypes.c_void_p(out.data_ptr()),
                None if out_pos is None else ctypes.c_void_p(out_pos.data_ptr()), N, C, HW, S, row0,
                native.stream_ptr(out.device))
            native.check(rc, "dvis_nchw_to_tokens_affine")
            row0 += HW
    return out if pos is None else (out, out_pos)


def normalize_pad_ok(x, mean):
    return bool(x.is_cuda and x.dim() == 4 and x.dtype in (torch.uint8, torch.float32) and x.is_contiguous()
                and mean.numel() == x.shape[1] and mean.dtype == torch.float32 and not torch.is_grad_enabled())


def normalize_pad(x, mean, std, Hp, Wp):
    N, C, H, W = x.shape
    out = torch.empty((N, C, Hp, Wp), dtype=torch.float32, device=x.device)
    with torch.cuda.device(x.device):
        native.check(native.lib().dvis_normalize_pad(
            native.dev_ptr(x, "frames"), int(x.dtype == torch.uint8), native.dev_ptr(out, "out"), N * C, C, H, W, Hp, Wp,
            native.dev_ptr(mean.detach().reshape(-1), "pixel_mean"), native.dev_ptr(std.detach().reshape(-1), "pixel_std"),
            native.stream_ptr(x.device)), "dvis_normalize_pad")
    return out


def tokens_to_map(tokens, row0, h, w):
    N, S, C = tokens.shape
    if not (tokens.is_cuda and tokens.dtype == torch.float32 and tokens.is_contiguous() and not torch.is_grad_enabled()):
        return tokens[:, row0:row0 + h * w].transpose(1, 2).reshape(N, C, h, w)
    out = torch.empty((N, C, h, w), dtype=torch.float32, device=tokens.device)
    with torch.cuda.device(tokens.device):
        native.check(native.lib().dvis_tokens_to_nchw(ctypes.c_void_p(tokens.data_ptr()), ctypes.c_void_p(out.data_ptr()), N, C, h * w,
# ... 65 lines not shown
def gn_fold_ok(norm, K, HW):
    return bool(PD_GN_FOLD and isinstance(norm, torch.nn.GroupNorm) and norm.num_channels == K
                and native.lib().dvis_conv_x3_gn_fold_supported(K, norm.num_groups, HW))


def affine_in_ok(x, weight):
    return bool(PD_GN_FOLD and conv1x1_x3_ok(x, weight) and x.shape[1] == 256 and x.shape[0] > 0
                and native.lib().dvis_conv_x3_gn_fold_supported(weight.shape[0], weight.shape[0] // 8, x.shape[2] * x.shape[3]))


def _gn_partials(N, K, HW, device):
    return torch.empty((N, K // 8, HW // 32, 2), dtype=torch.float64, device=device)


def _gn_finalize(part, norm, N, K, HW):
    scale = torch.empty(N * K, dtype=torch.float32, device=part.device)
    shift = torch.empty(N * K, dtype=torch.float32, device=part.device)
    with torch.cuda.device(part.device):
        native.check(native.lib().dvis_group_norm_finalize(
            native.dev_ptr(part, "partials"), None if norm.weight is None else native.dev_ptr(norm.weight.detach(), "gamma"),
            None if norm.bias is None else native.dev_ptr(norm.bias.detach(), "beta"), native.dev_ptr(scale, "scale"),
            native.dev_ptr(shift, "shift"), N, K, norm.num_groups, HW, float(norm.eps), native.stream_ptr(part.device)),
            "dvis_group_norm_finalize")
    return scale, shift


def conv1x1_x3(x, weight, bias=None, res=None, relu=False, stride=1, xexp=None, affine=None, affine_relu=False, gn=None):
    N, Ci, H, W = x.shape
    Co = weight.shape[0]

    def make():
        return _x3_pack_conv1x1(weight.detach().reshape(Co, Ci).contiguous())
    buf, wexp = _x3_cache(weight, [weight], make, kind="conv1x1")
    OH, OW = (H + stride - 1) // stride, (W + stride - 1) // stride
    out = torch.empty((N, Co, OH, OW), dtype=torch.float32, device=x.device)
    step = _conv_x3_chunks(N, Ci, Co, H * W, OH * OW)
    if affine is not None and not (affine_in_ok(x, weight) and stride == 1 and gn is None):
        raise RuntimeError("conv1x1_x3: this launch takes no input affine (see affine_in_ok); apply scale_shift_act_ first")
    part = _gn_partials(N, Co, OH * OW, x.device) if gn is not None and N > 0 and gn_fold_ok(gn, Co, OH * OW) else None
    with torch.cuda.device(x.device):
        for i in range(0, N, step):
            n = min(step, N - i)
            native.check(native.lib().dvis_conv1x1_x3(
                native.dev_ptr(x[i:i + n], "x"), ctypes.c_void_p(buf.data_ptr()),
                None if bias is None else native.dev_ptr(bias.detach(), "bias"),
                None if res is None else native.dev_ptr(res[i:i + n], "res"), native.dev_ptr(out[i:i + n], "out"), n, Ci, Co, H, W,
                stride, X3_CONV_XEXP if xexp is None else xexp, wexp, 1 if relu else 0, native.stream_ptr(x.device),
                None if affine is None else native.dev_ptr(affine[0].reshape(N, Ci)[i:i + n], "scale"),
                None if affine is None else native.dev_ptr(affine[1].reshape(N, Ci)[i:i + n], "shift"), 1 if affine_relu else 0,
                None if part is None else native.dev_ptr(part[i:i + n], "partials")), "dvis_conv1x1_x3")
    if gn is None:
        return out
    return out, (_gn_finalize(part, gn, N, Co, OH * OW) if part is not None else group_norm_affine(out, gn))


X3_DUAL = os.environ.get("DVIS_X3_DUAL", "1") != "0"


def conv1x1_x3_dual_ok(a, w3, x, ws, stride2):
    if not (X3_DUAL and conv1x1_x3_ok(a, w3) and x.is_cuda and x.dim() == 4 and x.dtype == torch.float32 and x.is_contiguous()
            and ws.dtype == torch.float32 and ws.shape[0] == w3.shape[0] and stride2 in (1, 2)):
        return False
    N, C, H, W = a.shape
    N2, C2, H2, W2 = x.shape
    Co = w3.shape[0]
    return (N2 == N and C2 % 64 == 0 and 64 <= C2 <= 4096 and (H2 + stride2 - 1) // stride2 == H and (W2 + stride2 - 1) // stride2 == W
            and (C + C2) <= 4096 and bool(native.lib().dvis_conv1x1_x3_supported(C + C2, Co, 1, H * W, H * W))
            and C2 * H2 * W2 * 4 < 2 ** 31)


def conv1x1_x3_dual(a, w3, b3, x, ws, bs, relu=True, stride2=1, xexp=None):
    N, C, H, W = a.shape
    _, C2, H2, W2 = x.shape
    Co = w3.shape[0]

    def make():
        wcat = torch.cat([w3.detach().reshape(Co, C), ws.detach().reshape(Co, C2)], 1).contiguous()
        buf, e = _x3_pack_conv1x1(wcat)
        bias = None
        if b3 is not None or bs is not None:
            bias = (0 if b3 is None else b3.detach()) + (0 if bs is None else bs.detach())
        return buf, e, bias
    buf, wexp, bias = _x3_cache(w3, [w3, ws, b3, bs], make, kind="conv1x1 + shortcut")
    out = torch.empty((N, Co, H, W), dtype=torch.float32, device=a.device)
    step = min(_conv_x3_chunks(N, C, Co, H * W, H * W), _conv_x3_chunks(N, C2, Co, H2 * W2, H * W))
    with torch.cuda.device(a.device):
        for i in range(0, N, step):
            n = min(step, N - i)
            native.check(native.lib().dvis_conv1x1_x3_dual(
                native.dev_ptr(a[i:i + n], "a"), native.dev_ptr(x[i:i + n], "x"), ctypes.c_void_p(buf.data_ptr()),
                None if bias is None else native.dev_ptr(bias, "bias"), None, native.dev_ptr(out[i:i + n], "out"), n, C, C2, Co, H, W,
                H2, W2, stride2, X3_CONV_XEXP if xexp is None else xexp, wexp, 1 if relu else 0, native.stream_ptr(a.device)),
                "dvis_conv1x1_x3_dual")
    return out


def conv3x3_x3_ok(x, weight, stride=1, res=None):
    return weight.dim() == 4 and tuple(weight.shape[2:]) == (3, 3) and conv1x1_x3_ok(x, weight, stride, res)


def conv3x3_x3(x, weight, bias=None, res=None, relu=False, stride=1, xexp=None):
    N, Ci, H, W = x.shape
    Co = weight.shape[0]

    def make():
        return _x3_pack_conv3x3(weight.detach().contiguous())
    buf, wexp = _x3_cache(weight, [weight], make, kind="conv3x3")
    OH, OW = (H + stride - 1) // stride, (W + stride - 1) // stride
    out = torch.empty((N, Co, OH, OW), dtype=torch.float32, device=x.device)
    step = _conv_x3_chunks(N, Ci, Co, H * W, OH * OW)
    with torch.cuda.device(x.device):
        for i in range(0, N, step):
            n = min(step, N - i)
            native.check(native.lib().dvis_conv3x3_x3(
                native.dev_ptr(x[i:i + n], "x"), ctypes.c_void_p(buf.data_ptr()),
                None if bias is None else native.dev_ptr(bias.detach(), "bias"),
                None if res is None else native.dev_ptr(res[i:i + n], "res"), native.dev_ptr(out[i:i + n], "out"), n, Ci, Co, H, W,
                stride, X3_CONV_XEXP if xexp is None else xexp, wexp, 1 if relu else 0, native.stream_ptr(x.device)),
                "dvis_conv3x3_x3")
    return out


X3_IMAGES = os.environ.get("DVIS_X3_IMAGES", "1") != "0"


class OperandImage:

    def __init__(self, data, N, C, H, W, exp):
        self.data, self.N, self.C, self.H, self.W, self.exp = data, N, C, H, W, exp

    @property
    def device(self):
        return self.data.device

    def images(self, i, n):
        per = self.data.numel() // self.N
        return self.data[i * per:(i + n) * per]


def x3_images_ok(N, C, K, H, W, device, taps=1, stride=1):
    if not (X3_IMAGES and x3_on() and device.type == "cuda" and not torch.is_grad_enabled()):
        return False
    if taps not in (1, 9) or C % 64 != 0 or not (K == 128 or K % 256 == 0) or N <= 0:
        return False
    OH, OW = (H + stride - 1) // stride, (W + stride - 1) // stride
    return bool(native.lib().dvis_conv1x1_x3_supported(C, K, 1, H * W, OH * OW))


def _image_chunks(N, C, K, H, W, OH, OW):
    per = max(C * H * ((W + 31) // 32 * 32), K * OH * ((OW + 31) // 32 * 32)) * 4
    return max(1, min(N, (2 ** 31 - 1) // per))


def upsample_add_image(lateral, top, lat_affine=None, oexp=None):
    N, C, H, W = lateral.shape
    lib = native.lib()
    oe = X3_CONV_XEXP if oexp is None else oexp
    top = top.contiguous()
    data = torch.empty(lib.dvis_conv_x3_image_bytes(N, C, H, W), dtype=torch.uint8, device=lateral.device)
    img = OperandImage(data, N, C, H, W, oe)
    step = _image_chunks(N, C, C, H, W, H, W)
    with torch.cuda.device(lateral.device):
        for i in range(0, N, step):
            n = min(step, N - i)
            sc = None if lat_affine is None else native.dev_ptr(lat_affine[0].reshape(N, C)[i:i + n], "scale")
            sh = None if lat_affine is None else native.dev_ptr(lat_affine[1].reshape(N, C)[i:i + n], "shift")
            native.check(lib.dvis_upsample_add_image(native.dev_ptr(lateral[i:i + n], "lateral"), sc, sh, native.dev_ptr(top[i:i + n], "top"),
                                                     ctypes.c_void_p(img.images(i, n).data_ptr()), n, C, H, W, top.shape[-2], top.shape[-1], oe,
                                                     native.stream_ptr(lateral.device)), "dvis_upsample_add_image")
    return img


def conv_x3_image(src, weight, bias=None, res=None, relu=False, stride=1, out_image=False, oexp=None, xexp=None, gn=None):
    lib = native.lib()
    from_img = isinstance(src, OperandImage)
    if not (from_img or out_image):
        raise ValueError("conv_x3_image: neither side is an operand image")
    N, C, H, W = (src.N, src.C, src.H, src.W) if from_img else src.shape
    K, taps = weight.shape[0], weight.shape[2] * weight.shape[3]
    dev = weight.device

    def make():
        w2 = weight.detach().contiguous()
        if from_img:
            return _x3_packed(w2, lib.dvis_conv1x1_x3_packed_bytes(C, K) * taps, lambda e, buf, st: lib.dvis_conv_x3_pack_image(
                native.dev_ptr(w2, "weight"), K, C, taps, e, buf, st), "dvis_conv_x3_pack_image")
        return _x3_pack_conv1x1(w2.reshape(K, C)) if taps == 1 else _x3_pack_conv3x3(w2)
    kind = ("conv%dx%d" % ((1, 1) if taps == 1 else (3, 3))) + (" image-in" if from_img else "")
    buf, wexp = _x3_cache(weight, [weight], make, kind=kind)
    OH, OW = (H + stride - 1) // stride, (W + stride - 1) // stride
    xe = src.exp if from_img else (X3_CONV_XEXP if xexp is None else xexp)
    oe = X3_CONV_XEXP if oexp is None else oexp
    if out_image:
        out = OperandImage(torch.empty(lib.dvis_conv_x3_image_bytes(N, K, OH, OW), dtype=torch.uint8, device=dev), N, K, OH, OW, oe)
    else:
        out = torch.empty((N, K, OH, OW), dtype=torch.float32, device=dev)
    step = _image_chunks(N, C, K, H, W, OH, OW)
    if gn is not None and not (from_img and not out_image):
        raise ValueError("conv_x3_image: gn needs an operand image in and an fp32 map out")
    part = _gn_partials(N, K, OH * OW, dev) if gn is not None and N > 0 and gn_fold_ok(gn, K, OH * OW) else None
    with torch.cuda.device(dev):
        for i in range(0, N, step):
            n = min(step, N - i)
            native.check(lib.dvis_conv_x3_image(
                ctypes.c_void_p(src.images(i, n).data_ptr()) if from_img else None, None if from_img else native.dev_ptr(src[i:i + n], "x"),
                ctypes.c_void_p(buf.data_ptr()), None if bias is None else native.dev_ptr(bias.detach(), "bias"),
                None if res is None else native.dev_ptr(res[i:i + n], "res"), None if out_image else native.dev_ptr(out[i:i + n], "out"),
                ctypes.c_void_p(out.images(i, n).data_ptr()) if out_image else None, n, C, K, H, W, stride, taps, xe, wexp, oe, 1 if relu else 0,
                native.stream_ptr(dev), None if part is None else native.dev_ptr(part[i:i + n], "partials")), "dvis_conv_x3_image")
    if gn is None:
        return out
    return out, (_gn_finalize(part, gn, N, K, OH * OW) if part is not None else group_norm_affine(out, gn))


X3_BNECK = os.environ.get("DVIS_X3_BNECK", "1") != "0"


def bneck_stage_x3_ok(x, blocks):
    if not (X3_BNECK and x3_on() and x.is_cuda and x.dim() == 4 and x.dtype == torch.float32 and x.is_contiguous()
            and not torch.is_grad_enabled() and len(blocks) >= 2 and x.shape[1] == 64 and x.shape[0] > 0):
        return False
    for i, b in enumerate(blocks):
        cin = 64 if i == 0 else 256
        if tuple(b["w1"].shape) != (64, cin, 1, 1) or tuple(b["w2"].shape) != (64, 64, 3, 3) or tuple(b["w3"].shape) != (256, 64, 1, 1):
            return False
        if (b["ws"] is not None) != (i == 0) or (i == 0 and tuple(b["ws"].shape) != (256, 64, 1, 1)):
            return False
        if any(b[k] is not None and (b[k].dtype != torch.float32 or b[k].device != x.device) for k in b):
            return False
    return bool(native.lib().dvis_bneck_x3_supported(1, x.shape[2], x.shape[3]))


def bneck_stage_x3(x, blocks, xexp=None):
    N, _, H, W = x.shape
    lib = native.lib()
    xe = X3_CONV_XEXP if xexp is None else xexp
    dev = x.device

    def packed_conv1():
        w = blocks[0]["w1"]

        return _x3_cache(w, [w], lambda: _x3_pack_conv1x1(w.detach().reshape(64, 64).contiguous()), kind="conv1x1")

    def packed_block(i):
        b, nxt = blocks[i], (blocks[i + 1] if i + 1 < len(blocks) else None)
        ws, w1n = b["ws"], (None if nxt is None else nxt["w1"])

        def make():
            w2 = b["w2"].detach().contiguous()
            w3 = b["w3"].detach().reshape(256, 64).contiguous()
            wsd = None if ws is None else ws.detach().reshape(256, 64).contiguous()
            w1d = None if w1n is None else w1n.detach().reshape(64, 256).contiguous()
            e2, e1 = _x3_wexp(w2), (0 if w1d is None else _x3_wexp(w1d))
            e3 = _x3_wexp(w3 if wsd is None else torch.cat([w3, wsd], 1))
            buf = torch.empty(lib.dvis_bneck_x3_packed_bytes(0 if w1d is None else 1, 0 if wsd is None else 1), dtype=torch.uint8, device=dev)
            with torch.cuda.device(dev):
                native.check(lib.dvis_bneck_x3_pack(native.dev_ptr(w2, "w2"), native.dev_ptr(w3, "w3"),
                                                    None if wsd is None else native.dev_ptr(wsd, "ws"),
                                                    None if w1d is None else native.dev_ptr(w1d, "w1"), e2, e3, e1,
                                                    ctypes.c_void_p(buf.data_ptr()), native.stream_ptr(dev)), "dvis_bneck_x3_pack")
            b3 = b["b3"]
            if b["bs"] is not None:
                b3 = b["bs"].detach() if b3 is None else b3.detach() + b["bs"].detach()
            return buf, e2, e3, e1, (None if b3 is None else b3.detach().clone())
        return _x3_cache(b["w2"], [b["w2"], b["w3"], ws, w1n, b["b3"], b["bs"]], make, kind="bottleneck chain")

    img_bytes = lib.dvis_bneck_x3_image_bytes(N, H, W)
    imgs = [torch.empty(img_bytes, dtype=torch.uint8, device=dev) for _ in range(2)]
    ys = [torch.empty((N, 256, H, W), dtype=torch.float32, device=dev) for _ in range(min(2, len(blocks)))]
    step = max(1, min(N, (2 ** 31 - 1) // (256 * H * W * 4)))
    per_img = img_bytes // N

    def ptr(t):
        return None if t is None else native.dev_ptr(t.detach(), "shift")

    with torch.cuda.device(dev):
        for i0 in range(0, N, step):
            n = min(step, N - i0)
            isl = slice(i0 * per_img, (i0 + n) * per_img)
            buf1, e1 = packed_conv1()
            native.check(lib.dvis_conv1x1_x3_image(native.dev_ptr(x[i0:i0 + n], "x"), ctypes.c_void_p(buf1.data_ptr()), ptr(blocks[0]["b1"]),
                                                   ctypes.c_void_p(imgs[0][isl].data_ptr()), n, 64, H, W, xe, e1, xe, 1, native.stream_ptr(dev)),
                         "dvis_conv1x1_x3_image")
            for i, b in enumerate(blocks):
                buf, e2, e3, e1n, b3 = packed_block(i)
                last = i + 1 == len(blocks)
                y, yprev = ys[i % 2], ys[(i + 1) % 2]
                native.check(lib.dvis_bneck_x3(
                    ctypes.c_void_p(imgs[i % 2][isl].data_ptr()), None if i == 0 else native.dev_ptr(yprev[i0:i0 + n], "res"),
                    native.dev_ptr(x[i0:i0 + n], "x") if i == 0 else None, ctypes.c_void_p(buf.data_ptr()), ptr(b["b2"]), ptr(b3),
                    None if last else ptr(blocks[i + 1]["b1"]), native.dev_ptr(y[i0:i0 + n], "y"),
                    None if last else ctypes.c_void_p(imgs[(i + 1) % 2][isl].data_ptr()), n, H, W, xe, e2, e3, e1n, native.stream_ptr(dev)),
                    "dvis_bneck_x3")
    return ys[(len(blocks) - 1) % 2]


def _fp32_pack(weight, kind, numel, pack, name):
    def make():
        w = weight.detach().contiguous()
        uf = torch.empty(numel, dtype=torch.float32, device=w.device)
        with torch.cuda.device(w.device):
            native.check(pack(native.dev_ptr(w, "weight"), native.dev_ptr(uf, "uf"), native.stream_ptr(w.device)), name)
        return uf
    return derived.TABLE.get(weight, kind, [weight], make)


CONV1X1_MFMA = os.environ.get("DVIS_CONV1X1_MFMA", "1") != "0"


def conv1x1s2_supported(x, weight):
    N, Ci, H, W = x.shape
    return CONV1X1_MFMA and x.is_cuda and x.dtype == torch.float32 and x.is_contiguous() and not torch.is_grad_enabled() \
        and bool(native.lib().dvis_conv1x1_mfma_supported(Ci, weight.shape[0], ((H + 1) // 2) * ((W + 1) // 2))) \
        and 2 * Ci * H * W * 4 < 2 ** 31


def conv1x1_mfma(x, weight, bias=None, res=None, relu=False, stride=1):
    N, Ci, H, W = x.shape
    Co = weight.shape[0]
# ... 822 lines not shown
```

dvis_plus_amd/native.py:

```python
import ctypes
import os

import torch

_HERE = os.path.dirname(os.path.abspath(__file__))
LIB_PATH = os.environ.get("DVIS_HIP_LIB") or os.path.join(_HERE, "lib", "libdvis_hip.so")

F32, F64, F16, BF16 = 0, 1, 2, 3
_DTYPE = {torch.float32: F32, torch.float64: F64, torch.float16: F16, torch.bfloat16: BF16}

_c = ctypes
_i, _i64, _p, _f = _c.c_int, _c.c_int64, _c.c_void_p, _c.c_float

SIGNATURES = {
    "dvis_last_error": (_c.c_char_p, []),
    "dvis_version": (_i, []),
    "dvis_msda_forward": (_i, [_i, _p, _p, _p, _p, _p, _i, _i, _i, _i, _i, _i, _i, _p, _p]),
    "dvis_msda_backward": (_i, [_i, _p, _p, _p, _p, _p, _p, _i, _i, _i, _i, _i, _i, _i, _p, _p, _p, _p]),
    "dvis_msda_backward_det_ws_bytes": (_i64, [_i, _i, _i, _i]),
    "dvis_msda_backward_det": (_i, [_p, _p, _p, _p, _p, _p, _i, _i, _i, _i, _i, _i, _i, _p, _p, _p, _p, _p]),
    "dvis_msda_fused_backward_ws_bytes": (_i64, [_i, _i, _i, _i]),
    "dvis_msda_fused_backward": (_i, [_p, _p, _p, _p, _i, _p, _i64, _p, _i64, _p, _i, _i, _i, _i, _i, _i, _i, _p, _p, _p, _p, _p]),
    "dvis_msda_fused_forward": (_i, [_p, _p, _p, _p, _i, _p, _i64, _p, _i64, _i, _i, _i, _i, _i, _i, _i, _p, _p, _p]),
    "dvis_msda_fused_forward_h": (_i, [_i, _p, _p, _p, _p, _i, _p, _i64, _p, _i64, _i, _i, _i, _i, _i, _i, _i, _p, _p, _p]),
    "dvis_nchw_to_tokens": (_i, [_p, _p, _i64, _i, _i64, _i64, _i64, _p]),
    "dvis_tokens_to_nchw": (_i, [_p, _p, _i64, _i, _i64, _i64, _i64, _p]),
    "dvis_normalize_pad": (_i, [_p, _i, _p, _i64, _i, _i, _i, _i, _i, _p, _p, _p]),
    "dvis_nchw_to_tokens_affine": (_i, [_p, _p, _p, _p, _p, _p, _i64, _i, _i64, _i64, _i64, _p]),
    "dvis_mask_logits": (_i, [_p, _p, _i, _i, _i, _i64, _p, _p]),
    "dvis_mask_logits_backward_ws_bytes": (_i64, [_i, _i, _i, _i64]),
    "dvis_mask_logits_backward": (_i, [_p, _p, _i, _i, _i, _i64, _p, _p, _p, _p]),
    "dvis_attn_mask": (_i, [_p, _p, _i, _i, _i, _i, _i, _i, _i, _p, _p, _p]),
    "dvis_center_pool3": (_i, [_p, _i64, _i, _i, _p, _p, _p, _p]),
    "dvis_attn_mask_pooled": (_i, [_p, _p, _i, _i, _i, _i, _i, _p, _p, _p]),
    "dvis_mask_gemm_plan": (_i, [_i, _i, _i, _i, _i, _i, _i, _i, _i, _i, _p, _i]),
    "dvis_attention_ws_bytes": (_i64, [_i, _i, _i, _i]),
    "dvis_attention_ws_bytes_k": (_i64, [_i, _i, _i, _i, _i]),
    "dvis_attention_plan": (_i, [_i, _i, _i, _i, _i, _i64, _i64, _i, _p]),
    "dvis_attention_forward": (_i, [_p, _p, _p, _p, _p, _p, _p, _p, _p, _p, _i, _i, _i, _i, _i, _f, _p, _p]),
    "dvis_attention_forward_k": (_i, [_p, _p, _p, _p, _p, _p, _p, _p, _p, _p, _i, _i, _i, _i, _i, _f, _p, _p, _i]),
    "dvis_attention_backward": (_i, [_p, _p, _p, _p, _p, _p, _p, _p, _p, _p, _p, _i, _i, _i, _i, _i, _f, _p]),
    "dvis_attention_backward_threads": (_i, [_i]),
    "dvis_masked_attention_backward_ws_bytes": (_i64, [_i, _i, _i, _i]),
    "dvis_masked_attention_backward": (_i, [_p, _p, _p, _p, _p, _p, _p, _p, _p, _p, _p, _p, _p, _i, _i, _i, _i, _i, _f, _p, _p]),
    "dvis_masked_attention_backward_plan": (_i, [_i, _i, _i, _p]),
    "dvis_add_layernorm": (_i, [_p, _p, _i64, _p, _p, _p, _i64, _i, _f, _p]),
    "dvis_add_layernorm_pos": (_i, [_p, _p, _i64, _p, _p, _p, _p, _i64, _p, _i64, _i, _f, _p]),
    "dvis_bias_act": (_i, [_p, _p, _p, _i64, _i, _i64, _i, _p]),
    "dvis_conv3x3_winograd_supported": (_i, [_i, _i, _i, _i]),
    "dvis_conv3x3_winograd_pack": (_i, [_p, _p, _i, _i, _p]),
    "dvis_conv3x3_winograd": (_i, [_p, _p, _p, _p, _i, _i, _i, _i, _i, _i, _p]),
    "dvis_conv3x3s2_supported": (_i, [_i, _i, _i, _i]),
    "dvis_conv3x3s2_pack": (_i, [_p, _p, _i, _i, _p]),
    "dvis_conv3x3s2": (_i, [_p, _p, _p, _p, _i, _i, _i, _i, _i, _i, _p]),
    "dvis_conv7x7s2_supported": (_i, [_i, _i, _i, _i]),
    "dvis_conv7x7s2_pack": (_i, [_p, _p, _p]),
    "dvis_conv7x7s2": (_i, [_p, _p, _p, _p, _i, _i, _i, _i, _p]),
    "dvis_conv1x1_mfma_supported": (_i, [_i, _i, _i64]),
    "dvis_conv1x1_mfma_pack": (_i, [_p, _p, _i, _i, _p]),
    "dvis_conv1x1_mfma": (_i, [_p, _p, _p, _p, _p, _i, _i, _i, _i64, _i, _p]),
    "dvis_conv1x1s2_mfma": (_i, [_p, _p, _p, _p, _p, _i, _i, _i, _i, _i, _i, _p]),
    "dvis_conv1x1_supported": (_i, [_i, _i, _i64]),
    "dvis_conv1x1_bias_act": (_i, [_p, _p, _p, _p, _p, _i, _i, _i, _i64, _i, _p]),
    "dvis_bias_relu_maxpool": (_i, [_p, _p, _p, _i64, _i, _i, _i, _p]),
    "dvis_group_norm_affine": (_i, [_p, _p, _p, _p, _p, _i64, _i, _i, _i64, _f, _p]),
    "dvis_scale_shift_act": (_i, [_p, _p, _p, _i64, _i64, _i, _p]),
    "dvis_group_norm_finalize": (_i, [_p, _p, _p, _p, _p, _i64, _i, _i, _i64, _f, _p]),
    "dvis_upsample_add_affine": (_i, [_p, _p, _p, _p, _p, _i64, _i, _i, _i, _i, _p]),
    "dvis_upsample_add": (_i, [_p, _p, _p, _i64, _i, _i, _i, _i, _p]),
    "dvis_dwconv3x3_tokens": (_i, [_p, _p, _i64, _i, _i, _i, _i, _p, _p, _i, _p]),
    "dvis_dwconv3x3_tokens_backward_ws_bytes": (_i64, [_i, _i, _i, _i]),
    "dvis_dwconv3x3_tokens_backward": (_i, [_p, _p, _p, _p, _i, _i64, _i, _i, _i, _i, _p, _p, _p, _p, _p]),
    "dvis_adapter_res2": (_i, [_p, _p, _p, _p, _p, _p, _i, _i, _i, _i, _p]),
    "dvis_vps_argmax": (_i, [_p, _i64, _i64, _p, _i, _i, _i, _i, _i, _i, _i, _i, _i, _i, _p, _p, _p, _p]),
    "dvis_vss_argmax": (_i, [_p, _i64, _i64, _p, _i, _i, _i, _i, _i, _i, _i, _i, _i, _i, _i, _i, _p, _p]),
    "dvis_resize2_gt0": (_i, [_p, _i64, _i64, _i, _i, _i, _i, _i, _i, _i, _i, _i, _i, _p, _p]),
    "dvis_resize2": (_i, [_p, _i64, _i64, _i, _i, _i, _i, _i, _i, _i, _i, _i, _i, _i, _p, _p]),
    "dvis_lsap_solve": (_i, [_p, _i, _i, _p]),
    "dvis_match_chain": (_i, [_p, _i, _i, _p]),
    "dvis_gemm_nt": (_i, [_p, _i64, _i64, _p, _i64, _i64, _p, _p, _i64, _i64, _p, _i64, _i64, _i, _i, _i, _i, _i, _i, _p]),
    "dvis_gemm_nt_bb": (_i, [_p, _i64, _i64, _p, _i64, _i64, _p, _i64, _p, _i64, _i64, _p, _i64, _i64, _i, _i, _i, _i, _i, _i,
                             _p]),
    "dvis_gemm_ln": (_i, [_p, _i64, _p, _i64, _p, _p, _f, _p, _p, _f, _p, _i64, _p, _i64, _p, _p, _i64, _p, _i64, _i, _i, _i,
                          _i, _i, _p]),
    "dvis_gemm_ln_supported": (_i, [_i, _i, _i, _i]),
    "dvis_gemm_ln_num_configs": (_i, []),
    "dvis_gemm_ln_pick_config": (_i, [_i, _i, _i]),
    "dvis_x3_packed_bytes": (_i64, [_i, _i]),
    "dvis_x3_set_reserve": (_i, [_i]),
    "dvis_x3_set_range_flag": (_i, [_p]),
    "dvis_x3_set_tag": (_i, [_i]),
    "dvis_x3_pack": (_i, [_p, _i64, _i, _i, _i, _p, _p]),
    "dvis_x3_linear_supported": (_i, [_i, _i, _i]),
    "dvis_x3_linear": (_i, [_p, _i64, _i64, _i, _p, _i, _i, _i, _p, _i, _p, _i64, _p]),
    "dvis_x3_tile_supported": (_i, [_i, _i]),
    "dvis_x3_tile_packed_bytes": (_i64, [_i, _i]),
    "dvis_x3_tile_pack": (_i, [_p, _i64, _i, _i, _i, _p, _p]),
    "dvis_x3_tile_linear_qkv": (_i, [_p, _i64, _i64, _i, _p, _i, _i, _i, _p, _i, _i, _f, _p, _p]),
    "dvis_attention_x3_packed": (_i, [_p, _p, _p, _i, _i, _i, _p]),
    "dvis_x3_rows_image_bytes": (_i64, [_i64, _i]),
    "dvis_x3_rows_image": (_i, [_p, _i64, _i64, _i, _i, _p, _p]),
    "dvis_layernorm_rows_image": (_i, [_p, _p, _p, _i64, _i, _f, _i, _p, _p]),
    "dvis_x3_tile_pack_order": (_i, [_p, _i64, _i, _i, _i, _i, _p, _p]),
    "dvis_x3_tile_linear_image": (_i, [_p, _i64, _i, _p, _i, _i, _i, _p, _i, _p, _i64, _p, _i64, _p, _i, _p]),
    "dvis_x3_tile_linear_qkv_image": (_i, [_p, _i64, _i, _p, _i, _i, _i, _p, _i, _i, _f, _p, _p]),
    "dvis_attention_x3_packed_image": (_i, [_p, _p, _i, _i, _i, _i, _p]),
    "dvis_x3_tile_linear": (_i, [_p, _i64, _i64, _i, _p, _i, _i, _i, _p, _i, _p, _i64, _p, _i64, _p]),
    "dvis_x3_linear_res": (_i, [_p, _i64, _i64, _i, _p, _i, _i, _i, _p, _i, _p, _i64, _p, _i64, _p]),
    "dvis_x3_linear_add": (_i, [_p, _i64, _i64, _i, _p, _i, _i, _i, _p, _i64, _p, _i, _p, _i64, _p]),
    "dvis_x3_linear_ln": (_i, [_p, _i64, _i64, _i, _p, _i, _i, _i, _p, _p, _i64, _p, _p, _f, _p, _i64, _p, _p, _i64, _p]),
    "dvis_x3_ffn_packed_bytes": (_i64, [_i, _i, _i]),
    "dvis_x3_ffn_pack": (_i, [_p, _i64, _p, _i64, _i, _i, _i, _i, _i, _p, _p]),
    "dvis_x3_ffn_ln": (_i, [_p, _i64, _i64, _i, _i, _i, _p, _i, _i, _i, _i, _p, _p, _p, _p, _f, _p, _i64, _p, _p, _i64, _p]),
    "dvis_conv1x1_x3_supported": (_i, [_i, _i, _i64, _i64, _i64]),
    "dvis_conv1x1_x3_packed_bytes": (_i64, [_i, _i]),
    "dvis_conv1x1_x3_pack": (_i, [_p, _i, _i, _i, _p, _p]),
    "dvis_conv_x3_gn_fold_supported": (_i, [_i, _i, _i64]),
    "dvis_conv1x1_x3": (_i, [_p, _p, _p, _p, _p, _i, _i, _i, _i, _i, _i, _i, _i, _i, _p, _p, _p, _i, _p]),
    "dvis_conv1x1_x3_dual": (_i, [_p, _p, _p, _p, _p, _p, _i, _i, _i, _i, _i, _i, _i, _i, _i, _i, _i, _i, _p]),
    "dvis_conv3x3_x3_packed_bytes": (_i64, [_i, _i]),
    "dvis_conv3x3_x3_pack": (_i, [_p, _i, _i, _i, _p, _p]),
    "dvis_conv3x3_x3": (_i, [_p, _p, _p, _p, _p, _i, _i, _i, _i, _i, _i, _i, _i, _i, _p]),
    "dvis_bneck_x3_supported": (_i, [_i64, _i, _i]),
    "dvis_bneck_x3_image_bytes": (_i64, [_i64, _i, _i]),
    "dvis_bneck_x3_packed_bytes": (_i64, [_i, _i]),
    "dvis_bneck_x3_pack": (_i, [_p, _p, _p, _p, _i, _i, _i, _p, _p]),
    "dvis_bneck_x3": (_i, [_p, _p, _p, _p, _p, _p, _p, _p, _p, _i, _i, _i, _i, _i, _i, _i, _p]),
    "dvis_conv1x1_x3_image": (_i, [_p, _p, _p, _p, _i, _i, _i, _i, _i, _i, _i, _i, _p]),
    "dvis_conv_x3_image_bytes": (_i64, [_i64, _i, _i, _i]),
    "dvis_conv_x3_pack_image": (_i, [_p, _i, _i, _i, _i, _p, _p]),
    "dvis_conv_x3_image": (_i, [_p, _p, _p, _p, _p, _p, _p, _i, _i, _i, _i, _i, _i, _i, _i, _i, _i, _i, _p, _p]),
    "dvis_upsample_add_image": (_i, [_p, _p, _p, _p, _p, _i, _i, _i, _i, _i, _i, _i, _p]),
    "dvis_gemm_num_configs": (_i, []),
    "dvis_gemm_pick_config": (_i, [_i, _i, _i, _i]),
    "dvis_gemm_pick_config_nw": (_i, [_i, _i, _i, _i, _i]),
    "dvis_gemm_config_waves": (_i, [_i]),
    "dvis_pan_pair_hist": (_i, [_p, _p, _p, _i, _i, _i, _i64, _p, _p, _p]),
    "dvis_sem_confusion": (_i, [_p, _p, _i64, _i, _p, _p, _p]),
    "dvis_video_consistency": (_i, [_p, _p, _i, _i64, _p, _i, _p, _p, _p]),
    "dvis_rle_encode": (_i, [_p, _i64, _i, _i, _i, _p, _p, _p, _p, _p, _p, _p]),
    "dvis_rle_strings": (_i, [_p, _p, _i64, _p, _p, _p, _p]),
    "dvis_rle_decode": (_i, [_p, _p, _i64, _i, _i, _p, _p]),
    "dvis_track_intersections": (_i, [_p, _i64, _i, _p, _i64, _i, _i, _i64, _i, _p, _p]),
    "dvis_pan_segment_stats": (_i, [_p, _i, _i, _i, _i, _p, _p, _p]),
    "dvis_pan_paint_rgb": (_i, [_p, _i64, _p, _i, _p, _p]),
    "dvis_sem_paint": (_i, [_p, _i64, _p, _p, _p, _p]),
    "dvis_resize_frames_u8": (_i, [_p, _i, _i, _i, _p, _i, _i, _p, _i, _p, _i, _i, _p]),
    "dvis_match_cost_ws_bytes": (_i64, [_i, _i, _i, _i]),
    "dvis_match_cost": (_i, [_p, _p, _i, _p, _p, _p, _i, _i, _i, _i, _i, _i, _i, _i, _i, _f, _f, _f, _p, _p, _p, _p]),
    "dvis_point_sample_rows": (_i, [_p, _i, _p, _i64, _i, _i, _i, _p, _p]),
    "dvis_point_loss_ws_bytes": (_i64, [_i64]),
    "dvis_point_loss_fwd": (_i, [_p, _p, _i, _p, _i, _i, _i, _i, _i, _i, _p, _p, _p]),
    "dvis_point_loss_bwd": (_i, [_p, _p, _i, _p, _p, _p, _p, _i, _i, _i, _i, _i, _i, _f, _p, _p, _p]),
    "dvis_contrastive_items_tile": (_i, []),
    "dvis_contrastive_items": (_i, [_p, _i64, _i, _p, _p, _p, _p, _p, _i, _i64, _p, _p, _p, _p, _p, _p]),
    "dvis_contrastive_items_backward_ws_bytes": (_i64, [_i, _i64, _i]),
    "dvis_contrastive_items_backward": (_i, [_p, _i64, _i, _p, _p, _p, _p, _p, _i, _i64, _p, _p, _p, _p, _p, _p, _p, _p, _p, _p,
                                             _p, _p, _p]),
    "dvis_window_attention_supported": (_i, [_i, _i]),
    "dvis_window_attention": (_i, [_p, _p, _p, _p, _i, _i, _i, _i, _i, _i, _i, _f, _p]),
    "dvis_mask_pool_plan": (_i, [_i, _i, _i, _i64, _p]),
    "dvis_mask_pool_ws_bytes": (_i64, [_i, _i, _i, _i64]),
    "dvis_mask_pool": (_i, [_p, _p, _i64, _i64, _i, _i, _i, _i64, _p, _p, _p, _p]),
    "dvis_text_class_logits": (_i, [_p, _i64, _p, _i64, _p, _p, _i, _i, _i, _i, _p, _p]),
    "dvis_ov_ensemble": (_i, [_p, _p, _p, _p, _f, _f, _i, _i, _p, _p]),
}

_lib = None


def lib():
    global _lib
    if _lib is None:
        if not os.path.exists(LIB_PATH):
            raise RuntimeError(
                f"{LIB_PATH} not found: build it with `python -m dvis_plus_amd.build` "
                "(__graft_entry__.build()).  dvis_plus_amd has no CPU/eager fallback.")
        l = ctypes.CDLL(LIB_PATH)
        for name, (res, args) in SIGNATURES.items():
            fn = getattr(l, name)
            fn.restype, fn.argtypes = res, args
        _lib = l
    return _lib


def check(rc, what):
    if rc != 0:
        msg = lib().dvis_last_error().decode()
        raise RuntimeError(f"{what} failed (code {rc}): {msg}")


def dtype_code(t):
    try:
        return _DTYPE[t.dtype]
    except KeyError:
        raise RuntimeError(f"unsupported dtype {t.dtype}") from None


def dev_ptr(t, name):
    if not t.is_cuda:
        raise RuntimeError(f"{name} must be a GPU tensor (dvis_plus_amd has no CPU path); got device {t.device}")
    if not t.is_contiguous():
        raise RuntimeError(f"{name} tensor has to be contiguous")
    return ctypes.c_void_p(t.data_ptr())


def stream_ptr(device=None):
    return ctypes.c_void_p(torch.cuda.current_stream(device).cuda_stream)
```

dvis_plus_amd/pixel_decoder.py:

```python
import math
import warnings

import torch
import torch.nn.functional as F
from torch import nn
from torch.nn.init import constant_, normal_, xavier_uniform_

from . import derived, functions as Fn
from .d2 import configurable
from .registry import SEM_SEG_HEADS_REGISTRY, ShapeSpec


def _is_power_of_2(n):
    if (not isinstance(n, int)) or (n < 0):
        raise ValueError("invalid input for _is_power_of_2: {} (type: {})".format(n, type(n)))
    return (n & (n - 1) == 0) and n != 0


class PositionEmbeddingSine(nn.Module):

    def __init__(self, num_pos_feats=64, temperature=10000, normalize=False, scale=None):
        super().__init__()
        if scale is not None and normalize is False:
            raise ValueError("normalize should be True if scale is passed")
# ... 323 lines not shown

    def __init__(self, *args, norm=None, activation=None, **kwargs):
        super().__init__(*args, **kwargs)
        self.norm, self.activation = norm, activation

    def _plain_1x1(self):
        return self.kernel_size == (1, 1) and self.stride == (1, 1) and self.groups == 1 and self.padding == (0, 0)

    def affine_input_ok(self, x):
        return self._plain_1x1() and torch.is_tensor(x) and Fn.affine_in_ok(x, self.weight)

    def conv(self, x, in_affine=None):
        if in_affine is not None:
            return Fn.conv1x1_x3(x, self.weight, self.bias, affine=in_affine[:2], affine_relu=in_affine[2])
        if self._plain_1x1():
            return Fn.conv1x1(x, self.weight, self.bias)
        if self.kernel_size == (3, 3) and self.stride == (1, 1) and self.padding == (1, 1) and self.dilation == (1, 1) \
                and self.groups == 1 and x.is_cuda and not torch.is_grad_enabled():
            return Fn.conv3x3_bias_act(x, self.weight, self.bias)
        return F.conv2d(x, self.weight, self.bias, self.stride, self.padding, self.dilation, self.groups)

    def conv_and_affine(self, x):
        if isinstance(self.norm, nn.GroupNorm) and self.activation is None:
            if self._plain_1x1() and Fn.conv1x1_x3_ok(x, self.weight) \
                    and Fn.gn_fold_ok(self.norm, self.out_channels, x.shape[2] * x.shape[3]):
                return Fn.conv1x1_x3(x, self.weight, self.bias, gn=self.norm)
            y = self.conv(x)
            aff = Fn.group_norm_affine(y, self.norm)
            if aff is not None:
                return y, aff
            return self.norm(y), None
        return self.forward(x), None

    def image_input_ok(self, N, C, H, W, device):
        return self.stride == (1, 1) and self.dilation == (1, 1) and self.groups == 1 and self.weight.dtype == torch.float32 \
            and ((self.kernel_size == (3, 3) and self.padding == (1, 1)) or (self.kernel_size == (1, 1) and self.padding == (0, 0))) \
            and C == self.in_channels and Fn.x3_images_ok(N, C, self.out_channels, H, W, device, taps=self.kernel_size[0] ** 2)

    def forward(self, x, in_affine=None, defer_to=None):
        aff = None
        gn_relu = isinstance(self.norm, nn.GroupNorm) and self.activation in (None, F.relu)
        if isinstance(x, Fn.OperandImage):
            if gn_relu:
                x, aff = Fn.conv_x3_image(x, self.weight, self.bias, gn=self.norm)
            else:
                x = Fn.conv_x3_image(x, self.weight, self.bias)
        else:
            x = self.conv(x, in_affine)
        if gn_relu:
            if aff is None:
                aff = Fn.group_norm_affine(x, self.norm)
            if aff is not None:
                if defer_to is not None and defer_to.affine_input_ok(x):
                    return x, (aff[0], aff[1], self.activation is not None)
                return Fn.scale_shift_act_(x, aff[0], aff[1], relu=self.activation is not None)
        if self.norm is not None:
            x = self.norm(x)
        if self.activation is not None:
            x = self.activation(x)
        return x


def get_norm(norm, out_channels):
    if norm is None or norm == "":
        return None
    if norm != "GN":
        raise NotImplementedError(f"norm {norm!r}: the DVIS++ configs use GN")
    return nn.GroupNorm(32, out_channels)


def c2_xavier_fill(module):
    nn.init.kaiming_uniform_(module.weight, a=1)
    if module.bias is not None:
        nn.init.constant_(module.bias, 0)


@SEM_SEG_HEADS_REGISTRY.register()
class MSDeformAttnPixelDecoder(nn.Module):
    @configurable
    def __init__(self, input_shape, *, transformer_dropout, transformer_nheads, transformer_dim_feedforward,
                 transformer_enc_layers, conv_dim, mask_dim, norm=None, transformer_in_features, common_stride):
        super().__init__()
        transformer_input_shape = {k: v for k, v in input_shape.items() if k in transformer_in_features}
        input_shape = sorted(input_shape.items(), key=lambda x: x[1].stride)
        self.in_features = [k for k, v in input_shape]
        self.feature_strides = [v.stride for k, v in input_shape]
        self.feature_channels = [v.channels for k, v in input_shape]
        transformer_input_shape = sorted(transformer_input_shape.items(), key=lambda x: x[1].stride)
        self.transformer_in_features = [k for k, v in transformer_input_shape]
        transformer_in_channels = [v.channels for k, v in transformer_input_shape]
        self.transformer_feature_strides = [v.stride for k, v in transformer_input_shape]
        self.transformer_num_feature_levels = len(self.transformer_in_features)
        chans = transformer_in_channels[::-1] if self.transformer_num_feature_levels > 1 \
            else [transformer_in_channels[-1]]
        self.input_proj = nn.ModuleList([
            nn.Sequential(nn.Conv2d(c, conv_dim, kernel_size=1), nn.GroupNorm(32, conv_dim)) for c in chans])
        for proj in self.input_proj:
            nn.init.xavier_uniform_(proj[0].weight, gain=1)
            nn.init.constant_(proj[0].bias, 0)
        self.transformer = MSDeformAttnTransformerEncoderOnly(
            d_model=conv_dim, dropout=transformer_dropout, nhead=transformer_nheads,
            dim_feedforward=transformer_dim_feedforward, num_encoder_layers=transformer_enc_layers,
            num_feature_levels=self.transformer_num_feature_levels)
        self.pe_layer = PositionEmbeddingSine(conv_dim // 2, normalize=True)
        self.mask_dim = mask_dim
        self.mask_features = ConvNorm(conv_dim, mask_dim, kernel_size=1, stride=1, padding=0)
        c2_xavier_fill(self.mask_features)
        self.maskformer_num_feature_levels = 3
        self.common_stride = common_stride
        stride = min(self.transformer_feature_strides)
        self.num_fpn_levels = int(math.log2(stride) - math.log2(self.common_stride))
        lateral_convs, output_convs = [], []
        use_bias = norm == ""
        for idx, in_channels in enumerate(self.feature_channels[:self.num_fpn_levels]):
            lateral_conv = ConvNorm(in_channels, conv_dim, kernel_size=1, bias=use_bias, norm=get_norm(norm, conv_dim))
            output_conv = ConvNorm(conv_dim, conv_dim, kernel_size=3, stride=1, padding=1, bias=use_bias,
                                   norm=get_norm(norm, conv_dim), activation=F.relu)
            c2_xavier_fill(lateral_conv)
            c2_xavier_fill(output_conv)
            self.add_module("adapter_{}".format(idx + 1), lateral_conv)
            self.add_module("layer_{}".format(idx + 1), output_conv)
            lateral_convs.append(lateral_conv)
            output_convs.append(output_conv)
        self.lateral_convs = lateral_convs[::-1]
        self.output_convs = output_convs[::-1]

    @classmethod
    def from_config(cls, cfg, input_shape):
        hd = cfg.MODEL.SEM_SEG_HEAD
        return dict(
            input_shape={k: v for k, v in input_shape.items() if k in hd.IN_FEATURES},
            conv_dim=hd.CONVS_DIM, mask_dim=hd.MASK_DIM, norm=hd.NORM,
            transformer_dropout=cfg.MODEL.MASK_FORMER.DROPOUT, transformer_nheads=cfg.MODEL.MASK_FORMER.NHEADS,
            transformer_dim_feedforward=1024, transformer_enc_layers=hd.TRANSFORMER_ENC_LAYERS,
            transformer_in_features=hd.DEFORMABLE_TRANSFORMER_ENCODER_IN_FEATURES, common_stride=hd.COMMON_STRIDE)

    def forward_features(self, features):
        with torch.autocast(device_type="cuda", enabled=False), Fn.x3_stage("pd_proj"):
            if self.training:
                return self._train_features(features)
            srcs, pos, affines = [], [], []
            for idx, f in enumerate(self.transformer_in_features[::-1]):
                x = features[f].float().contiguous()
                conv, gn = self.input_proj[idx][0], self.input_proj[idx][1]
                s_ = Fn.conv1x1(x, conv.weight, conv.bias) if conv.kernel_size == (1, 1) and conv.stride == (1, 1) \
                    and conv.padding == (0, 0) and conv.groups == 1 else conv(x)
                affine = Fn.group_norm_affine(s_, gn)
                srcs.append(s_ if affine is not None else gn(s_))
                affines.append(affine)
                pos.append(self.pe_layer.compute(x.shape[2], x.shape[3], x.device))
            with Fn.x3_stage("encoder"):
                y, _, _, shapes_py = self.transformer(srcs, pos, affines)
            bs = y.shape[0]
            out, tokens, start = [], [], 0
            for li, (h, w) in enumerate(shapes_py):
                tokens.append(y[:, start:start + h * w])
                if li + 1 == len(shapes_py) and self.num_fpn_levels > 0:
                    out.append(Fn.tokens_to_map(y, start, h, w))
                else:
                    out.append(tokens[-1].transpose(1, 2).reshape(bs, -1, h, w))
                start += h * w
            with Fn.x3_stage("mask_path"):
                deferred = None
                for idx, f in enumerate(self.in_features[:self.num_fpn_levels][::-1]):
                    x = features[f].float().contiguous()
                    cur_fpn, affine = self.lateral_convs[idx].conv_and_affine(x)
                    oc = self.output_convs[idx]
                    if cur_fpn.is_cuda and cur_fpn.dtype == torch.float32 and cur_fpn.is_contiguous() and out[-1].dtype == torch.float32 \
                            and oc.image_input_ok(*cur_fpn.shape, cur_fpn.device):
                        last = idx + 1 == self.num_fpn_levels and len(out) >= self.maskformer_num_feature_levels
                        y = oc(Fn.upsample_add_image(cur_fpn, out[-1], affine), defer_to=self.mask_features if last else None)
                        if isinstance(y, tuple):
                            y, deferred = y
                        out.append(y)
                    else:
                        out.append(oc(Fn.upsample_add(cur_fpn, out[-1], affine)))
                multi_scale_features = TokenMaps(out[:self.maskformer_num_feature_levels])
                multi_scale_features.tokens = tokens[:self.maskformer_num_feature_levels]
                return self.mask_features(out[-1], in_affine=deferred), out[0], multi_scale_features

    @staticmethod
    def _conv_norm(layer, x):
        x = F.conv2d(x, layer.weight, layer.bias, layer.stride, layer.padding, layer.dilation, layer.groups)
        if layer.norm is not None:
            x = F.group_norm(x, layer.norm.num_groups, layer.norm.weight, layer.norm.bias, layer.norm.eps)
        return x if layer.activation is None else layer.activation(x)

    def _train_features(self, features):
        dtype = self.mask_features.weight.dtype
        cast = lambda t: t.to(dtype) if dtype == torch.float64 else t.float()
        srcs, pos = [], []
        for idx, f in enumerate(self.transformer_in_features[::-1]):
            x = cast(features[f])
            conv, gn = self.input_proj[idx][0], self.input_proj[idx][1]
            s_ = F.conv2d(x, conv.weight, conv.bias, conv.stride, conv.padding, conv.dilation, conv.groups)
            srcs.append(F.group_norm(s_, gn.num_groups, gn.weight, gn.bias, gn.eps))
            pos.append(self.pe_layer.compute(x.shape[2], x.shape[3], x.device))
        y, shapes_py = self.transformer.train_forward(srcs, pos)
        bs = y.shape[0]
        out, start = [], 0
        for h, w in shapes_py:
            out.append(y[:, start:start + h * w].transpose(1, 2).reshape(bs, -1, h, w))
            start += h * w
        for idx, f in enumerate(self.in_features[:self.num_fpn_levels][::-1]):
            cur_fpn = self._conv_norm(self.lateral_convs[idx], cast(features[f]))
            top = F.interpolate(out[-1], size=cur_fpn.shape[-2:], mode="bilinear", align_corners=False)
            out.append(self._conv_norm(self.output_convs[idx], cur_fpn + top))
        return self._conv_norm(self.mask_features, out[-1]), out[0], TokenMaps(out[:self.maskformer_num_feature_levels])


class TokenMaps(list):
    tokens = None


def r50_input_shape():
    return {"res2": ShapeSpec(channels=256, stride=4), "res3": ShapeSpec(channels=512, stride=8),
            "res4": ShapeSpec(channels=1024, stride=16), "res5": ShapeSpec(channels=2048, stride=32)}
```

dvis_plus_amd/transformer_decoder.py:

```python
import math

import torch
import torch.nn.functional as F
from torch import nn

from . import derived, functions as Fn
from .pixel_decoder import ConvNorm, PositionEmbeddingSine, c2_xavier_fill
from .d2 import configurable
from .registry import TRANSFORMER_DECODER_REGISTRY


def _xavier_(module):
    for p in module.parameters():
        if p.dim() > 1:
            nn.init.xavier_uniform_(p)


class SelfAttentionLayer(nn.Module):
    own_gemm = None

    def __init__(self, d_model, nhead, dropout=0.0, activation="relu", normalize_before=False):
        super().__init__()
        if normalize_before:
            raise NotImplementedError("PRE_NORM=True is not used by the DVIS++ configs")
# ... 87 lines not shown
        self.linear2 = nn.Linear(dim_feedforward, d_model)
        self.norm = nn.LayerNorm(d_model)
        _xavier_(self)

    def forward(self, tgt):
        h = Fn.linear_relu(tgt, self.linear1, own=self.own_gemm)
        return Fn.add_layer_norm(Fn.linear(h, self.linear2.weight, self.linear2.bias, own=self.own_gemm), tgt, self.norm)

    def train_forward(self, tgt):
        h = torch.relu(F.linear(tgt, self.linear1.weight, self.linear1.bias))
        return self.norm(tgt + F.linear(h, self.linear2.weight, self.linear2.bias))


class MLP(nn.Module):
    own_gemm = None

    def __init__(self, input_dim, hidden_dim, output_dim, num_layers):
        super().__init__()
        self.num_layers = num_layers
        h = [hidden_dim] * (num_layers - 1)
        self.layers = nn.ModuleList(nn.Linear(n, k) for n, k in zip([input_dim] + h, h + [output_dim]))

    def forward(self, x):
        for i, layer in enumerate(self.layers):
            x = Fn.linear(x, layer.weight, layer.bias, relu=i < self.num_layers - 1, own=self.own_gemm)
        return x

    def train_forward(self, x):
        for i, layer in enumerate(self.layers):
            x = F.linear(x, layer.weight, layer.bias)
            x = torch.relu(x) if i < self.num_layers - 1 else x
        return x


def layer_predictions(logits, masks):
    return {"pred_logits": logits[-1], "pred_masks": masks[-1],
            "aux_outputs": [{"pred_logits": a, "pred_masks": m} for a, m in zip(logits[:-1], masks[:-1])]}


def layer_mask_logits(mask_embed, mask_features, mask_logits):
    L, _, T, Q, cm = mask_embed.shape
    h, w = mask_features.shape[-2:]
    rows = mask_embed[:, 0].permute(1, 0, 2, 3).reshape(T, L * Q, cm)
    logits = mask_logits(rows, mask_features[0].detach().contiguous())
    return logits.view(T, L, Q, h, w).permute(1, 2, 0, 3, 4).unsqueeze(1)


class _MaskedDecoderBase(nn.Module):

    _version = 2

    @configurable
    def __init__(self, in_channels, mask_classification=True, *, num_classes, hidden_dim, num_queries, nheads,
                 dim_feedforward, dec_layers, pre_norm, mask_dim, enforce_input_project):
        super().__init__()
        assert mask_classification, "Only support mask classification model"
        self.mask_classification = mask_classification
        self.pe_layer = PositionEmbeddingSine(hidden_dim // 2, normalize=True)
        self.num_heads, self.num_layers = nheads, dec_layers
        self.transformer_self_attention_layers = nn.ModuleList()
        self.transformer_cross_attention_layers = nn.ModuleList()
        self.transformer_ffn_layers = nn.ModuleList()
        for _ in range(self.num_layers):
            self.transformer_self_attention_layers.append(
                SelfAttentionLayer(d_model=hidden_dim, nhead=nheads, dropout=0.0, normalize_before=pre_norm))
            self.transformer_cross_attention_layers.append(
                CrossAttentionLayer(d_model=hidden_dim, nhead=nheads, dropout=0.0, normalize_before=pre_norm))
            self.transformer_ffn_layers.append(
                FFNLayer(d_model=hidden_dim, dim_feedforward=dim_feedforward, dropout=0.0, normalize_before=pre_norm))
        self.decoder_norm = nn.LayerNorm(hidden_dim)
        self.num_queries = num_queries
        self.query_feat = nn.Embedding(num_queries, hidden_dim)
        self.query_embed = nn.Embedding(num_queries, hidden_dim)
        self.num_feature_levels = 3
        self.level_embed = nn.Embedding(self.num_feature_levels, hidden_dim)
        self.input_proj = nn.ModuleList()
        for _ in range(self.num_feature_levels):
            if in_channels != hidden_dim or enforce_input_project:
                self.input_proj.append(ConvNorm(in_channels, hidden_dim, kernel_size=1))
                c2_xavier_fill(self.input_proj[-1])
            else:
                self.input_proj.append(nn.Sequential())
        self.class_embed = nn.Linear(hidden_dim, num_classes + 1)
        self.mask_embed = MLP(hidden_dim, hidden_dim, mask_dim, 3)
        self._kv_cache = derived.Derived()
        self.debug_masks = None

    def _load_from_state_dict(self, state_dict, prefix, local_metadata, strict, missing_keys, unexpected_keys,
                              error_msgs):
        version = local_metadata.get("version", None)
        if version is None or version < 2:
            for k in list(state_dict.keys()):
                if k.startswith(prefix) and "static_query" in k:
                    state_dict[k.replace("static_query", "query_feat")] = state_dict.pop(k)
        super()._load_from_state_dict(state_dict, prefix, local_metadata, strict, missing_keys, unexpected_keys,
                                      error_msgs)

    @staticmethod
    def _base_from_config(cfg, in_channels, mask_classification):
        mf = cfg.MODEL.MASK_FORMER
        assert mf.DEC_LAYERS >= 1
        return dict(in_channels=in_channels, mask_classification=mask_classification,
                    num_classes=cfg.MODEL.SEM_SEG_HEAD.NUM_CLASSES, hidden_dim=mf.HIDDEN_DIM,
                    num_queries=mf.NUM_OBJECT_QUERIES, nheads=mf.NHEADS, dim_feedforward=mf.DIM_FEEDFORWARD,
                    dec_layers=mf.DEC_LAYERS - 1, pre_norm=mf.PRE_NORM, enforce_input_project=mf.ENFORCE_INPUT_PROJ,
                    mask_dim=cfg.MODEL.SEM_SEG_HEAD.MASK_DIM)

    def _level_kv_weights(self):
        def make():
            per_level = []
            for lvl in range(self.num_feature_levels):
                idx = [i for i in range(self.num_layers) if i % self.num_feature_levels == lvl]
                ws = [self.transformer_cross_attention_layers[i].kv_weights() for i in idx]
                if not ws:
                    per_level.append(None)
                    continue
                Wv, bv = torch.cat([w[2] for w in ws], 0).detach(), torch.cat([w[3] for w in ws], 0).detach()
                bv_le = (bv.double() + Wv.double() @ self.level_embed.weight[lvl].detach().double()).float()
                per_level.append((tuple(idx), torch.cat([w[0] for w in ws], 0).detach(), torch.cat([w[1] for w in ws], 0).detach(),
                                  Wv, bv, bv_le))
            return tuple(per_level)
        return self._kv_cache.get([t for l in self.transformer_cross_attention_layers
                                   for t in (l.multihead_attn.in_proj_weight, l.multihead_attn.in_proj_bias)]
                                  + [self.level_embed.weight], make)

    @staticmethod
    def _f32_inputs(x, mask_features):
        if any(m.dtype != torch.float32 for m in x):
            tokens = getattr(x, "tokens", None)
            x = type(x)(Fn.f32(m) for m in x)
            if tokens is not None:
                x.tokens = [Fn.f32(t) for t in tokens]
        return x, Fn.f32(mask_features)

    def _run_layers(self, x, mask_features):
        C = self.decoder_norm.weight.shape[0]
        N = x[0].shape[0]
        size_list, kproj, vproj = [], {}, {}
        kvw = self._level_kv_weights()
        tokens = getattr(x, "tokens", None)
        with Fn.x3_stage("decoder_kv"):
            for lvl in range(self.num_feature_levels):
                h, w = x[lvl].shape[-2:]
                size_list.append((h, w))
                if kvw[lvl] is None:
                    continue
                idx, Wk, bk, Wv, bv, bv_le = kvw[lvl]
                le = self.level_embed.weight[lvl]
                ident = isinstance(self.input_proj[lvl], nn.Sequential) and len(self.input_proj[lvl]) == 0
                if tokens is not None and ident and not torch.is_grad_enabled():
                    tok = tokens[lvl]
                    pos_t = self.pe_layer.compute(h, w, tok.device).flatten(2).transpose(1, 2)
                    if Fn.x3_on() and Fn.x3_ok(tok, Wk.shape[0], Wk.shape[1], add=True):
                        tok = tok.contiguous()
                        kall = Fn.x3_linear(tok, Wk, bk, xadd=pos_t + le).transpose(0, 1)
                        vall = Fn.x3_linear(tok, Wv, bv_le).transpose(0, 1)
                    else:
                        kall = Fn.linear(tok + (pos_t + le), Wk, bk, tall=True).transpose(0, 1)
                        vall = Fn.linear(tok, Wv, bv_le, tall=True).transpose(0, 1)
                else:
                    src = (self.input_proj[lvl](x[lvl]).flatten(2) + le[None, :, None]).permute(2, 0, 1)
                    pos = self.pe_layer.compute(h, w, x[lvl].device).flatten(2).permute(2, 0, 1)
                    kall = Fn.linear(src + pos, Wk, bk, tall=True)
                    vall = Fn.linear(src, Wv, bv, tall=True)
                for n, i in enumerate(idx):
                    kproj[i], vproj[i] = kall[..., n * C:(n + 1) * C], vall[..., n * C:(n + 1) * C]
        query_embed = self.query_embed.weight.unsqueeze(1)
        output = self.query_feat.weight.unsqueeze(1).repeat(1, N, 1)
        pyramid = Fn.center_pool3(mask_features)
        if pyramid is not None and [tuple(p.shape[-2:]) for p in pyramid] != [tuple(sz) for sz in size_list[:3]]:
            pyramid = None
        for i in range(self.num_layers):
            lvl = i % self.num_feature_levels
            emb = self.mask_embed(self.decoder_norm(output).transpose(0, 1))
            if pyramid is not None:
                mask, allowed = Fn.attn_mask_pooled(emb.contiguous(), pyramid[lvl])
            else:
                mask, allowed = Fn.attn_mask(emb.contiguous(), mask_features, size_list[lvl])
            if self.debug_masks is not None:
                self.debug_masks.append(mask.bool() & (allowed > 0)[..., None])
            layer = self.transformer_cross_attention_layers[i]
            output = layer.attend(output, output + query_embed, kproj[i], vproj[i], mask, allowed)
            output = self.transformer_self_attention_layers[i](output, query_pos=query_embed)
            output = self.transformer_ffn_layers[i](output)
        return output

    def _final_heads(self, output, mask_features, need_masks):
        dec = self.decoder_norm(output).transpose(0, 1)
        logits = Fn.linear(dec, self.class_embed.weight, self.class_embed.bias)
        masks = Fn.mask_logits(self.mask_embed(dec).contiguous(), mask_features) if need_masks else None
        return dec, logits, masks


    def _train_layers(self, x, mask_features):
        N = x[0].shape[0]
        nh, L = self.num_heads, self.num_layers
        size_list, src, pos = [], [], []
        for lvl in range(self.num_feature_levels):
            h, w = x[lvl].shape[-2:]
            size_list.append((h, w))
            proj = self.input_proj[lvl]
            m = F.conv2d(x[lvl], proj.weight, proj.bias) if isinstance(proj, nn.Conv2d) else proj(x[lvl])
            src.append((m.flatten(2) + self.level_embed.weight[lvl][None, :, None]).permute(2, 0, 1))
            pos.append(self.pe_layer.compute(h, w, x[lvl].device).to(m.dtype).flatten(2).permute(2, 0, 1))
        query_embed = self.query_embed.weight.unsqueeze(1)
        output = self.query_feat.weight.unsqueeze(1).repeat(1, N, 1)
        feats = mask_features.detach()
        logits, embs = [], []

        def heads(output):
            dec = self.decoder_norm(output).transpose(0, 1)
            logits.append(F.linear(dec, self.class_embed.weight, self.class_embed.bias))
            embs.append(self.mask_embed.train_forward(dec))
            return dec

        dec = heads(output)
        for i in range(L):
            lvl = i % self.num_feature_levels
            with torch.no_grad():
                mask, allowed = Fn.attn_mask(embs[-1].detach().contiguous(), feats, size_list[lvl])
            if self.debug_masks is not None:
                self.debug_masks.append(mask.bool() & (allowed > 0)[..., None])
            output = self.transformer_cross_attention_layers[i].train_forward(
                output, output + query_embed, src[lvl] + pos[lvl], src[lvl],
                lambda q, k, v: Fn.masked_attention(q, k, v, nh, mask, allowed))
            output = self.transformer_self_attention_layers[i].train_forward(
                output, lambda q, k, v: Fn.attention(q, k, v, nh), query_pos=query_embed)
            output = self.transformer_ffn_layers[i].train_forward(output)
            dec = heads(output)
        Q = output.shape[0]
        if mask_features.requires_grad and torch.is_grad_enabled():
            masks = [Fn.mask_logits(e.contiguous(), mask_features) for e in embs]
        else:
            masks = list(Fn.mask_logits(torch.cat(embs, dim=1), feats).split(Q, dim=1))
        return output, dec, logits, masks

    def _train_inputs(self, x, mask_features):
        assert len(x) == self.num_feature_levels
        dt = self.decoder_norm.weight.dtype
        return [m.to(dt) for m in x], mask_features.to(dt).contiguous()

    @staticmethod
    def _train_video_outputs(b, t, logits, masks):
        return layer_predictions([z.unflatten(0, (b, t)) for z in logits],
                                 [z.unflatten(0, (b, t)).transpose(1, 2) for z in masks])

    @staticmethod
    def _train_bctq(z, b, t):
        return z.unflatten(0, (b, t)).permute(0, 3, 1, 2)

    def _train_clips(self, N):
        t = self.num_frames
        if t < 1 or N % t:
            raise ValueError(f"{type(self).__name__}: a training batch holds (b t) frames with t = num_frames = {t}; got {N} frames")
        return N // t, t


@TRANSFORMER_DECODER_REGISTRY.register()
class MultiScaleMaskedTransformerDecoder(_MaskedDecoderBase):

    @classmethod
    def from_config(cls, cfg, in_channels, mask_classification):
        return cls._base_from_config(cfg, in_channels, mask_classification)

    @Fn.fp32_island
    def forward(self, x, mask_features, mask=None):
        assert len(x) == self.num_feature_levels
        if self.training:
            x, mask_features = self._train_inputs(x, mask_features)
            _, _, logits, masks = self._train_layers(x, mask_features)
            return layer_predictions(logits, masks)
        x, mask_features = self._f32_inputs(x, mask_features)
        output = self._run_layers(x, mask_features)
        _, logits, masks = self._final_heads(output, mask_features, True)
        return {"pred_logits": logits, "pred_masks": masks, "aux_outputs": []}


@TRANSFORMER_DECODER_REGISTRY.register()
class VideoMultiScaleMaskedTransformerDecoder_dvisPlus(_MaskedDecoderBase):
    @configurable
    def __init__(self, in_channels, mask_classification=True, *, num_classes, hidden_dim, num_queries, nheads,
                 dim_feedforward, dec_layers, pre_norm, mask_dim, enforce_input_project, num_frames,
                 num_reid_head_layers, reid_hidden_dim):
        super().__init__(in_channels, mask_classification, num_classes=num_classes, hidden_dim=hidden_dim,
                         num_queries=num_queries, nheads=nheads, dim_feedforward=dim_feedforward,
                         dec_layers=dec_layers, pre_norm=pre_norm, mask_dim=mask_dim,
                         enforce_input_project=enforce_input_project)
        self.num_frames = num_frames
        if num_reid_head_layers > 0:
            self.reid_embed = MLP(hidden_dim, reid_hidden_dim, hidden_dim, num_reid_head_layers)
            for layer in self.reid_embed.layers:
                c2_xavier_fill(layer)
        else:
            self.reid_embed = nn.Identity()
        self.compute_pred_masks = True

    @classmethod
    def from_config(cls, cfg, in_channels, mask_classification):
        ret = cls._base_from_config(cfg, in_channels, mask_classification)
        ret.update(num_frames=cfg.INPUT.SAMPLING_FRAME_NUM, reid_hidden_dim=cfg.MODEL.MASK_FORMER.REID_HIDDEN_DIM,
                   num_reid_head_layers=cfg.MODEL.MASK_FORMER.NUM_REID_HEAD_LAYERS)
        return ret

    @Fn.fp32_island
    def forward(self, x, mask_features, mask=None):
        assert len(x) == self.num_feature_levels
        if self.training:
# ... 172 lines not shown
```

include/dvis_hip.h:

```cpp
#ifndef DVIS_HIP_H
#define DVIS_HIP_H

#include <stdint.h>

#ifdef __cplusplus
extern "C" {
#endif

enum { DVIS_F32 = 0, DVIS_F64 = 1, DVIS_F16 = 2, DVIS_BF16 = 3 };

enum {
  DVIS_OK = 0,
  DVIS_E_ARG = -1,
  DVIS_E_LAUNCH = -2,
  DVIS_E_UNSUPPORTED = -3
};

const char *dvis_last_error(void);
int dvis_version(void);

int dvis_msda_forward(int dtype, const void *value, const int64_t *shapes, const int64_t *level_start,
                      const void *loc, const void *w, int N, int S, int M, int D, int L, int Lq, int P,
                      void *out, void *stream);

// ... 34 lines not shown
int dvis_attn_mask(const float *embed, const float *feat, int B, int Q, int C, int H, int W, int h, int w,
                   uint8_t *mask, int32_t *allowed_count, void *stream);
int dvis_center_pool3(const float *feat, int64_t planes, int H, int W, float *p2, float *p4, float *p8, void *stream);
int dvis_attn_mask_pooled(const float *embed, const float *pooled, int B, int Q, int C, int h, int w, uint8_t *mask,
                          int32_t *allowed_count, void *stream);
int dvis_mask_gemm_plan(int mode, int B, int Q, int C, int H, int W, int h, int w, int aligned, int embed_aligned, int32_t *plan,
                        int capacity);

int64_t dvis_attention_ws_bytes(int BH, int Lq, int Lk, int d);
int dvis_attention_forward(const float *q, const int64_t *q_strides, const float *k, const int64_t *k_strides,
                           const float *v, const int64_t *v_strides, float *out, const int64_t *o_strides,
                           const uint8_t *mask, const int32_t *allowed_count, int B, int heads, int Lq, int Lk,
                           int d, float scale, void *ws, void *stream);
int dvis_attention_forward_k(const float *q, const int64_t *q_strides, const float *k, const int64_t *k_strides,
                           const float *v, const int64_t *v_strides, float *out, const int64_t *o_strides,
                           const uint8_t *mask, const int32_t *allowed_count, int B, int heads, int Lq, int Lk,
                           int d, float scale, void *ws, void *stream, int kernel);
int64_t dvis_attention_ws_bytes_k(int BH, int Lq, int Lk, int d, int kernel);
enum {
  DVIS_ATTN_FWD = 0,
  DVIS_ATTN_SHORT = 1,
  DVIS_ATTN_X3 = 2,
  DVIS_ATTN_KEYSPLIT = 3
};
int dvis_attention_plan(int BH, int Lq, int Lk, int d, int has_mask, int64_t k_row, int64_t v_row, int kernel, int32_t *plan);

int dvis_attention_backward(const float *q, const int64_t *q_strides, const float *k, const int64_t *k_strides,
                            const float *v, const int64_t *v_strides, const float *grad_out, const int64_t *g_strides,
                            float *dq, float *dk, float *dv, int B, int heads, int Lq, int Lk, int d, float scale,
                            void *stream);
int dvis_attention_backward_threads(int Lk);

int64_t dvis_masked_attention_backward_ws_bytes(int BH, int Lq, int Lk, int d);
int dvis_masked_attention_backward(const float *q, const int64_t *q_strides, const float *k, const int64_t *k_strides,
                                   const float *v, const int64_t *v_strides,
                                   const float *grad_out, const int64_t *g_strides, const uint8_t *mask,
                                   const int32_t *allowed_count, float *dq, float *dk, float *dv, int B, int heads, int Lq,
                                   int Lk, int d, float scale, void *ws, void *stream);
int dvis_masked_attention_backward_plan(int Lq, int Lk, int d, int32_t *plan);

int dvis_add_layernorm(const float *x, const float *res, int64_t res_row_stride, const float *gamma, const float *beta,
                       float *out, int64_t rows, int C, float eps, void *stream);

int dvis_add_layernorm_pos(const float *x, const float *res, int64_t res_row_stride, const float *gamma, const float *beta,
                           float *out, const float *pos, int64_t pos_rows, float *out_pos, int64_t rows, int C, float eps,
                           void *stream);

int dvis_upsample_add(const float *lateral, const float *top, float *out, int64_t planes, int H, int W, int h, int w,
                      void *stream);

int dvis_nchw_to_tokens(const float *x, float *out, int64_t N, int C, int64_t HW, int64_t S, int64_t row0, void *stream);

int dvis_tokens_to_nchw(const float *tok, float *out, int64_t N, int C, int64_t HW, int64_t S, int64_t row0, void *stream);
int dvis_normalize_pad(const void *in, int is_u8, float *out, int64_t planes, int C, int H, int W, int Hp, int Wp, const float *mean,
                       const float *stdv, void *stream);
int dvis_nchw_to_tokens_affine(const float *x, const float *scale, const float *shift, const float *pos, float *out,
                               float *out_pos, int64_t N, int C, int64_t HW, int64_t S, int64_t row0, void *stream);

int dvis_conv1x1_supported(int K, int M, int64_t HW);
int dvis_conv1x1_mfma_supported(int C, int K, int64_t HW);
int dvis_conv1x1_mfma_pack(const float *w, float *uf, int K, int C, void *stream);
int dvis_conv1x1_mfma(const float *x, const float *uf, const float *bias, const float *res, float *y, int N, int C, int K, int64_t HW,
                      int relu, void *stream);
int dvis_conv1x1s2_mfma(const float *x, const float *uf, const float *bias, const float *res, float *y, int N, int C, int K, int H, int W,
                        int relu, void *stream);
int dvis_conv1x1_bias_act(const float *x, const float *w, const float *bias, const float *res, float *out,
                          int N, int K, int M, int64_t HW, int relu, void *stream);

int dvis_conv3x3_winograd_supported(int C, int K, int H, int W);
int dvis_conv3x3s2_supported(int C, int K, int H, int W);
int dvis_conv7x7s2_supported(int C, int K, int H, int W);
int dvis_conv7x7s2_pack(const float *w, float *uf, void *stream);
int dvis_conv7x7s2(const float *x, const float *uf, const float *bias, float *y, int N, int H, int W, int relu, void *stream);
int dvis_conv3x3s2_pack(const float *w, float *uf, int K, int C, void *stream);
int dvis_conv3x3s2(const float *x, const float *uf, const float *bias, float *y, int N, int C, int K, int H, int W, int relu,
                   void *stream);
int dvis_conv3x3_winograd_pack(const float *w, float *uf, int K, int C, void *stream);
int dvis_conv3x3_winograd(const float *x, const float *uf, const float *bias, float *y, int N, int C, int K, int H, int W,
                          int relu, void *stream);

int dvis_bias_act(float *x, const float *bias, const float *res, int64_t planes, int C, int64_t HW, int relu,
                  void *stream);

int dvis_bias_relu_maxpool(const float *x, const float *bias, float *out, int64_t planes, int C, int H, int W,
                           void *stream);

int dvis_group_norm_affine(const float *x, const float *gamma, const float *beta, float *scale, float *shift, int64_t N,
                           int C, int G, int64_t HW, float eps, void *stream);
int dvis_scale_shift_act(float *x, const float *scale, const float *shift, int64_t planes, int64_t HW, int relu,
                         void *stream);
int dvis_group_norm_finalize(const double *part, const float *gamma, const float *beta, float *scale, float *shift, int64_t N, int C,
                             int G, int64_t HW, float eps, void *stream);
int dvis_upsample_add_affine(const float *lateral, const float *lat_scale, const float *lat_shift, const float *top,
                             float *out, int64_t planes, int H, int W, int h, int w, void *stream);

int dvis_dwconv3x3_tokens(const float *x, float *out, int64_t batch_stride, int B, int h, int w, int C, const float *weight,
                          const float *bias, int gelu, void *stream);

int64_t dvis_dwconv3x3_tokens_backward_ws_bytes(int B, int h, int w, int C);
int dvis_dwconv3x3_tokens_backward(const float *x, const float *grad_out, const float *weight, const float *bias, int gelu,
                                   int64_t batch_stride, int B, int h, int w, int C, float *grad_x, float *grad_weight, float *grad_bias,
                                   void *ws, void *stream);

int dvis_adapter_res2(const float *g, const float *c1, const float *x1, const float *scale, const float *shift, float *out, int B, int C,
                      int h8, int w8, void *stream);

int dvis_vps_argmax(const float *logits, int64_t stride_k, int64_t stride_t, const float *scores, int K, int T,
                    int h, int w, int first_h, int first_w, int img_h, int img_w, int out_h, int out_w,
                    int32_t *ids, uint8_t *conf, int32_t *areas, void *stream);

int dvis_resize2_gt0(const float *logits, int64_t stride_k, int64_t stride_t, int K, int T, int h, int w, int first_h,
                     int first_w, int img_h, int img_w, int out_h, int out_w, uint8_t *out, void *stream);

int dvis_resize2(const float *logits, int64_t stride_k, int64_t stride_t, int K, int T, int h, int w, int first_h,
                 int first_w, int img_h, int img_w, int out_h, int out_w, int sigmoid, float *out, void *stream);

int dvis_vss_argmax(const float *logits, int64_t stride_q, int64_t stride_t, const float *cls, int cls_row_stride, int Q,
                    int C, int T, int h, int w, int first_h, int first_w, int img_h, int img_w, int out_h, int out_w,
                    int64_t *out, void *stream);

int dvis_lsap_solve(const double *cost, int nr, int nc, int64_t *col4row);

int dvis_match_chain(const float *cost, int T, int Q, int64_t *indices);

int dvis_gemm_nt(const float *A, int64_t lda, int64_t strideA, const float *W, int64_t ldw, int64_t strideW,
                 const float *bias, const float *res, int64_t ldres, int64_t strideRes, float *C, int64_t ldc,
                 int64_t strideC, int M, int N, int K, int batch, int act, int config, void *stream);
int dvis_gemm_nt_bb(const float *A, int64_t lda, int64_t strideA, const float *W, int64_t ldw, int64_t strideW,
                    const float *bias, int64_t strideBias, const float *res, int64_t ldres, int64_t strideRes, float *C,
                    int64_t ldc, int64_t strideC, int M, int N, int K, int batch, int act, int config, void *stream);
int dvis_gemm_num_configs(void);
int dvis_gemm_pick_config(int M, int N, int K, int batch);
int dvis_gemm_pick_config_nw(int M, int N, int K, int batch, int nw);
int dvis_gemm_config_waves(int config);

int dvis_gemm_ln(const float *A, int64_t lda, const float *add, int64_t ldadd, const float *gamma1, const float *beta1,
                 float eps1, const float *gamma2, const float *beta2, float eps2, float *a_out, int64_t ldaout,
                 const float *W, int64_t ldw, const float *bias, const float *res, int64_t ldres, float *C, int64_t ldc,
                 int M, int N, int K, int act, int config, void *stream);
int dvis_gemm_ln_supported(int M, int N, int K, int norms);
int dvis_gemm_ln_num_configs(void);
int dvis_gemm_ln_pick_config(int M, int N, int K);

int64_t dvis_x3_packed_bytes(int N, int K);
int dvis_x3_set_reserve(int cus);
int dvis_x3_set_range_flag(int32_t *device_word);
int dvis_x3_set_tag(int tag);
int dvis_x3_pack(const float *W, int64_t ldw, int N, int K, int wexp, void *packed, void *stream);
int dvis_x3_linear_supported(int N, int K, int ln);
int dvis_x3_linear(const float *x, int64_t ldx, int64_t M, int K, const void *packed, int N, int xexp, int wexp,
                   const float *bias, int relu, float *out, int64_t ldo, void *stream);
int dvis_x3_linear_add(const float *x, int64_t ldx, int64_t M, int K, const void *packed, int N, int xexp, int wexp,
                       const float *xadd, int64_t xadd_rows, const float *bias, int relu, float *out, int64_t ldo, void *stream);
int dvis_x3_linear_res(const float *x, int64_t ldx, int64_t M, int K, const void *wp, int N, int xexp, int wexp, const float *bias, int act,
                       const float *res, int64_t ldres, float *out, int64_t ldo, void *stream);

int dvis_x3_tile_supported(int N, int K);
int64_t dvis_x3_tile_packed_bytes(int N, int K);
int dvis_x3_tile_pack(const float *w, int64_t ldw, int N, int K, int wexp, void *packed, void *stream);
int dvis_x3_tile_linear(const float *x, int64_t ldx, int64_t M, int K, const void *wp, int N, int xexp, int wexp, const float *bias, int act,
                        const float *res, int64_t ldres, float *out, int64_t ldo, void *stream);
int dvis_x3_tile_linear_qkv(const float *x, int64_t ldx, int64_t M, int K, const void *wp, int N, int xexp, int wexp, const float *bias,
                            int heads, int L, float qscale, void *ws, void *stream);
int dvis_attention_x3_packed(const void *ws, float *out, const int64_t *o_strides, int B, int heads, int L, void *stream);
int64_t dvis_x3_rows_image_bytes(int64_t M, int K);
int dvis_x3_rows_image(const float *x, int64_t ldx, int64_t M, int K, int xexp, void *image, void *stream);
int dvis_layernorm_rows_image(const float *x, const float *gamma, const float *beta, int64_t M, int C, float eps, int xexp, void *image,
                              void *stream);
int dvis_x3_tile_pack_order(const float *w, int64_t ldw, int N, int K, int wexp, int order, void *packed, void *stream);
int dvis_x3_tile_linear_image(const void *ximg, int64_t M, int K, const void *wp, int N, int xexp, int wexp, const float *bias, int act,
                              const float *res, int64_t ldres, float *out, int64_t ldo, void *oimg, int oexp, void *stream);
int dvis_x3_tile_linear_qkv_image(const void *ximg, int64_t M, int K, const void *wp, int N, int xexp, int wexp, const float *bias, int heads,
                                  int L, float qscale, void *ws, void *stream);
int dvis_attention_x3_packed_image(const void *ws, void *image, int B, int heads, int L, int xexp, void *stream);
int dvis_x3_linear_ln(const float *x, int64_t ldx, int64_t M, int K, const void *packed, int N, int xexp, int wexp,
                      const float *bias, const float *res, int64_t ldres, const float *gamma, const float *beta, float eps,
                      const float *pos, int64_t pos_rows, float *out, float *out2, int64_t ldo, void *stream);
int64_t dvis_x3_ffn_packed_bytes(int K, int H, int N);
int dvis_conv1x1_x3_supported(int C, int K, int64_t N, int64_t HW_in, int64_t HW_out);
int64_t dvis_conv1x1_x3_packed_bytes(int C, int K);
int dvis_conv1x1_x3_pack(const float *w, int K, int C, int wexp, void *packed, void *stream);
int dvis_conv_x3_gn_fold_supported(int K, int G, int64_t HW);
int dvis_conv1x1_x3(const float *x, const void *packed, const float *bias, const float *res, float *y, int N, int C, int K, int H,
                    int W, int stride, int xexp, int wexp, int relu, void *stream, const float *in_scale, const float *in_shift,
                    int in_relu, double *gn_part);
int dvis_conv1x1_x3_dual(const float *x, const float *x2, const void *packed, const float *bias, const float *res, float *y, int N,
                         int C, int C2, int K, int H, int W, int H2, int W2, int stride2, int xexp, int wexp, int relu, void *stream);
int64_t dvis_conv3x3_x3_packed_bytes(int C, int K);
int dvis_conv3x3_x3_pack(const float *w, int K, int C, int wexp, void *packed, void *stream);
int dvis_conv3x3_x3(const float *x, const void *packed, const float *bias, const float *res, float *y, int N, int C, int K, int H,
                    int W, int stride, int xexp, int wexp, int relu, void *stream);
int dvis_bneck_x3_supported(int64_t N, int H, int W);
int64_t dvis_bneck_x3_image_bytes(int64_t N, int H, int W);
int64_t dvis_bneck_x3_packed_bytes(int tail, int dual);
int dvis_bneck_x3_pack(const float *w2, const float *w3, const float *ws, const float *w1, int e2, int e3, int e1, void *packed,
                       void *stream);
int dvis_bneck_x3(const void *a1, const float *res, const float *x2, const void *packed, const float *b2, const float *b3,
                  const float *b1, float *y, void *out, int N, int H, int W, int xexp, int e2, int e3, int e1, void *stream);
int dvis_conv1x1_x3_image(const float *x, const void *packed, const float *bias, void *image, int N, int C, int H, int W, int xexp,
                          int wexp, int oexp, int relu, void *stream);
int64_t dvis_conv_x3_image_bytes(int64_t N, int C, int H, int W);
int dvis_conv_x3_pack_image(const float *w, int K, int C, int taps, int wexp, void *packed, void *stream);
int dvis_conv_x3_image(const void *ximg, const float *x, const void *packed, const float *bias, const float *res, float *y, void *image,
                       int N, int C, int K, int H, int W, int stride, int taps, int xexp, int wexp, int oexp, int relu, void *stream,
                       double *gn_part);
int dvis_upsample_add_image(const float *lateral, const float *lat_scale, const float *lat_shift, const float *top, void *image, int N,
                            int C, int H, int W, int h, int w, int oexp, void *stream);
int dvis_x3_ffn_pack(const float *W1, int64_t ldw1, const float *W2, int64_t ldw2, int K, int H, int N, int w1exp, int w2exp,
                     void *packed, void *stream);
int dvis_x3_ffn_ln(const float *x, int64_t ldx, int64_t M, int K, int H, int N, const void *packed, int xexp, int w1exp,
                   int hexp, int w2exp, const float *b1, const float *b2, const float *gamma, const float *beta, float eps,
                   const float *pos, int64_t pos_rows, float *out, float *out2, int64_t ldo, void *stream);

int dvis_pan_pair_hist(const int32_t *gt, const int32_t *pred, const int32_t *gt_table, int Ng, int Np, int T, int64_t HW,
                       int64_t *out, int64_t *bad, void *stream);
int dvis_sem_confusion(const int32_t *gt, const int32_t *pred, int64_t n, int num_class, int64_t *out, int64_t *bad, void *stream);
int dvis_video_consistency(const int32_t *gt, const int32_t *pred, int T, int64_t HW, const int32_t *ks, int nk, int64_t *gt_const,
                           int64_t *both_const, void *stream);

int dvis_rle_encode(const uint8_t *masks, int64_t N, int H, int W, int phase, int64_t *trans, int64_t *area, const int64_t *toff,
                    const int64_t *moff, int32_t *bnd, uint32_t *runs, void *stream);
int dvis_rle_strings(const uint32_t *runs, const int64_t *run_off, int64_t N, const int64_t *str_off, int64_t *lens, uint8_t *chars,
                     void *stream);
int dvis_rle_decode(const int32_t *ends, const int64_t *run_off, int64_t N, int H, int W, uint8_t *out, void *stream);
int dvis_track_intersections(const uint8_t *pred, int64_t pred_stride, int P, const uint8_t *gt, int64_t gt_stride, int G, int T,
                             int64_t HW, int accumulate, int64_t *out, void *stream);

int dvis_pan_segment_stats(const int32_t *map, int T, int H, int W, int n, int64_t *out, int64_t *bad, void *stream);
int dvis_pan_paint_rgb(const int32_t *map, int64_t npx, const int32_t *lut, int nlut, uint8_t *out, void *stream);
int dvis_sem_paint(const int32_t *map, int64_t npx, const int32_t *lut, uint8_t *out, int64_t *bad, void *stream);

int dvis_resize_frames_u8(const uint8_t *in, int T, int H, int W, uint8_t *out, int h, int w, const int32_t *xtab, int kx,
                          const int32_t *ytab, int ky, int reverse, void *stream);

int64_t dvis_match_cost_ws_bytes(int Q, int G, int T, int K);
int dvis_match_cost(const float *pred, const void *tgt, int tgt_u8, const float *coords, const float *logits,
                    const int64_t *tgt_ids, int Q, int G, int T, int H, int W, int Ht, int Wt, int K, int NC, float w_class,
                    float w_mask, float w_dice, float *C, float *terms, void *ws, void *stream);
int dvis_point_sample_rows(const void *rows, int rows_u8, const float *coords, int64_t R, int P, int H, int W, float *out,
                           void *stream);
int64_t dvis_point_loss_ws_bytes(int64_t R);
int dvis_point_loss_fwd(const float *src, const void *tgt, int tgt_u8, const float *coords, int R, int P, int H, int W, int Ht, int Wt,
                        float *out, void *ws, void *stream);
int dvis_point_loss_bwd(const float *src, const void *tgt, int tgt_u8, const float *coords, const float *sums, const float *g_mask,
                        const float *g_dice, int R, int P, int H, int W, int Ht, int Wt, float num_masks, float *grad_src,
                        void *det_ws, void *stream);

int dvis_contrastive_items_tile(void);
int dvis_contrastive_items(const float *src, int64_t R, int C, const int32_t *anchor, const int32_t *pos_ptr, const int32_t *pos_idx,
                           const int32_t *neg_ptr, const int32_t *neg_idx, int n, int64_t S, float *reid, float *aux, float *dots,
                           float *norms, float *stats, void *stream);
int64_t dvis_contrastive_items_backward_ws_bytes(int n, int64_t S, int C);
int dvis_contrastive_items_backward(const float *src, int64_t R, int C, const int32_t *anchor, const int32_t *pos_ptr,
                                    const int32_t *pos_idx, const int32_t *neg_ptr, const int32_t *neg_idx, int n, int64_t S,
                                    const int32_t *row_ptr, const int32_t *occ_slot, const int32_t *occ_item, const int32_t *arow_ptr,
                                    const int32_t *arow_item, const float *dots, const float *norms, const float *stats,
                                    const float *grad_reid, const float *grad_aux, float *grad_src, void *ws, void *stream);

int dvis_window_attention_supported(int ws, int d);
int dvis_window_attention(const float *qkv, const float *qkv_bias, const float *bias_table, float *out, int B, int H, int W, int heads,
                          int d, int ws, int shift, float scale, void *stream);

int dvis_mask_pool_plan(int B, int Q, int C, int64_t HW, int32_t *plan);
int64_t dvis_mask_pool_ws_bytes(int B, int Q, int C, int64_t HW);
int dvis_mask_pool(const float *x, const float *logits, int64_t l_bstride, int64_t l_qstride, int B, int Q, int C, int64_t HW,
                   float *sum, int32_t *count, void *ws, void *stream);

int dvis_text_class_logits(const float *x, int64_t x_stride, const float *dots, int64_t dots_stride, const float *logit_scale,
                           const int32_t *seg_ptr, int R, int D, int N, int K1, float *out, void *stream);

int dvis_ov_ensemble(const float *in_logits, const float *out_logits, const float *overlapping, const int32_t *valid, float alpha,
                     float beta, int R, int K, float *out, void *stream);

#ifdef __cplusplus
}
#endif
#endif
```

Measured before the change: 416.5.

## Tile upsample-add through LDS and read encoder tokens in place

Result: faster. 422.5, median of 6 (+1.4%).

```diff
diff --git a/dvis_plus_amd/csrc/conv1x1_x3.hip b/dvis_plus_amd/csrc/conv1x1_x3.hip
--- a/dvis_plus_amd/csrc/conv1x1_x3.hip
+++ b/dvis_plus_amd/csrc/conv1x1_x3.hip
@@ -369,6 +369,169 @@
   }
 }
 
+constexpr int kUpRows = 8, kUpTR = 6, kUpTX = 18, kUpTXS = 19, kUpPix = 68;
+
+template <bool TOK>
+__global__ __launch_bounds__(256) void upsample_add_image_v2_kernel(const float *__restrict__ lateral, const float *__restrict__ top,
+                                                                    void *__restrict__ img, int N, int C, int H, int W, int h, int w,
+                                                                    const float *__restrict__ lat_scale,
+                                                                    const float *__restrict__ lat_shift, float oscale, int HB,
+                                                                    long long tokS, long long row0) {
+#pragma clang fp contract(off)
+  __shared__ float topt[kUpTR * 64 * kUpTXS];
+  __shared__ __attribute__((aligned(16))) float tr[32 * kUpPix];
+  const int NCC = C / 64, XG = (W + 31) / 32;
+  const int cc = blockIdx.x, xg = blockIdx.y;
+  const int n = (int)blockIdx.z / HB, yb = ((int)blockIdx.z - n * HB) * kUpRows;
+  const int t = threadIdx.x;
+  const float sy = (float)h / (float)H, sx = (float)w / (float)W;
+  auto src_x = [&](int px, int &x0, int &x1, float &l1) {
+    float fx = __builtin_fmaf(sx, (float)px + 0.5f, -0.5f);
+    fx = fx < 0.f ? 0.f : fx;
+    x0 = min((int)fx, w - 1), x1 = x0 + (x0 < w - 1 ? 1 : 0);
+    l1 = fx - (float)x0;
+  };
+  auto src_y = [&](int y, int &y0, int &y1, float &l1) {
+    float fy = __builtin_fmaf(sy, (float)y + 0.5f, -0.5f);
+    fy = fy < 0.f ? 0.f : fy;
+    y0 = min((int)fy, h - 1), y1 = y0 + (y0 < h - 1 ? 1 : 0);
+    l1 = fy - (float)y0;
+  };
+  const int ylast = min(yb + kUpRows, H) - 1;
+  int ty0, ty1, tx0, tx1, unused;
+  float unusedf;
+  src_y(yb, ty0, unused, unusedf);
+  src_y(ylast, unused, ty1, unusedf);
+  src_x(min(32 * xg, W - 1), tx0, unused, unusedf);
+  src_x(min(32 * xg + 31, W - 1), unused, tx1, unusedf);
+  const int nty = min(ty1 - ty0 + 1, kUpTR), ntx = min(tx1 - tx0 + 1, kUpTX);
+  if constexpr (TOK) {
+    const float *tb = top + ((size_t)n * (size_t)tokS + (size_t)row0) * (size_t)C + 64 * cc;
+    for (int i = t; i < nty * ntx * 16; i += 256) {
+      const int c4 = i & 15, p = i >> 4, r = p / ntx, xx = p - r * ntx;
+      const f4 v = *(const f4 *)(tb + ((size_t)(ty0 + r) * w + (tx0 + xx)) * (size_t)C + 4 * c4);
+      float *d = topt + (r * 64 + 4 * c4) * kUpTXS + xx;
+      d[0] = v.x, d[kUpTXS] = v.y, d[2 * kUpTXS] = v.z, d[3 * kUpTXS] = v.w;
+    }
+  } else {
+    for (int i = t; i < nty * 64 * 32; i += 256) {
+      const int xx = i & 31, c = (i >> 5) & 63, r = i >> 11;
+      if (xx < ntx) topt[(r * 64 + c) * kUpTXS + xx] = top[(((size_t)n * C + 64 * cc + c) * h + ty0 + r) * (size_t)w + tx0 + xx];
+    }
+  }
+  const int q = t & 7, ca = t >> 3;
+  const bool packed = (ca & 11) == 11;
+  const int qx = 32 * xg + 4 * q;
+  const bool inside = qx < W;
+  const int qxc = inside ? qx : W - 4;
+  int xr0[4], xr1[4];
+  float lx0[4], lx1[4];
+#pragma unroll
+  for (int j = 0; j < 4; ++j) {
+    int x0, x1;
+    src_x(inside ? qx + j : W - 1, x0, x1, lx1[j]);
+    lx0[j] = 1.f - lx1[j];
+    xr0[j] = min(max(x0 - tx0, 0), kUpTX - 1), xr1[j] = min(max(x1 - tx0, 0), kUpTX - 1);
+  }
+  float sc[2] = {1.f, 1.f}, sh[2] = {0.f, 0.f};
+  const float *lp[2];
+#pragma unroll
+  for (int i = 0; i < 2; ++i) {
+    const size_t pl = (size_t)n * C + 64 * cc + ca + 32 * i;
+    if (lat_scale) sc[i] = lat_scale[pl], sh[i] = lat_shift[pl];
+    lp[i] = lateral + pl * (size_t)H * (size_t)W + qxc;
+  }
+  const __amdgpu_buffer_rsrc_t ri = dvis_make_rsrc_uniform(img, (unsigned)((long long)N * H * XG * NCC * 8192));
+  const int x = t & 31, g = (t >> 5) & 1, S = t >> 6;
+  f4 lat[2], nlat[2];
+#pragma unroll
+  for (int i = 0; i < 2; ++i) nlat[i] = *(const f4 *)(lp[i] + (size_t)yb * W);
+  __syncthreads();
+  for (int y = yb; y <= ylast; ++y) {
+#pragma unroll
+    for (int i = 0; i < 2; ++i) lat[i] = nlat[i];
+    if (y < ylast) {
+#pragma unroll
+      for (int i = 0; i < 2; ++i) nlat[i] = *(const f4 *)(lp[i] + (size_t)(y + 1) * W);
+    }
+    int y0, y1;
+    float ly1;
+    src_y(y, y0, y1, ly1);
+    const float ly0 = 1.f - ly1;
+    const int r0 = min(max(y0 - ty0, 0), kUpTR - 1), r1 = min(max(y1 - ty0, 0), kUpTR - 1);
+#pragma unroll
+    for (int i = 0; i < 2; ++i) {
+      const float *t0 = topt + (r0 * 64 + ca + 32 * i) * kUpTXS, *t1 = topt + (r1 * 64 + ca + 32 * i) * kUpTXS;
+      const float lv[4] = {lat[i].x, lat[i].y, lat[i].z, lat[i].w};
+#pragma unroll
+      for (int j = 0; j < 4; ++j) {
+        float l = inside ? lv[j] : lv[3];
+        if (lat_scale) l = __builtin_fmaf(l, sc[i], sh[i]);
+        const float t00 = t0[xr0[j]], t01 = t0[xr1[j]], t10 = t1[xr0[j]], t11 = t1[xr1[j]];
+        const float h1 = __builtin_fmaf(lx0[j], t10, lx1[j] * t11);
+        const float h0 = packed ? __builtin_fmaf(lx1[j], t01, lx0[j] * t00) : __builtin_fmaf(lx0[j], t00, lx1[j] * t01);
+        const float v = packed ? ly0 * h0 + ly1 * h1 : __builtin_fmaf(ly0, h0, ly1 * h1);
+        tr[(4 * q + j) * kUpPix + ca + 32 * i] = l + v;
+      }
+    }
+    __syncthreads();
+    const f4 p0 = *(const f4 *)(tr + x * kUpPix + 16 * S + 4 * g), p1 = *(const f4 *)(tr + x * kUpPix + 16 * S + 4 * g + 8);
+    h8 hi, lo;
+    split8(p0, p1, oscale, hi, lo);
+    const unsigned G = ((unsigned)n * (unsigned)H + (unsigned)y) * (unsigned)XG + (unsigned)xg;
+    const unsigned off = (G * (unsigned)NCC + (unsigned)cc) * 8192u + (unsigned)(S * 2048 + g * 512 + x * 16);
+    store_fragments2(ri, off, hi, 0, lo, 1024);
+    __syncthreads();
+  }
+}
+
+}
+
+static int g_upsample_v2 = [] {
+  const char *e = getenv("DVIS_UPSAMPLE_IMAGE_V2");
+  return e && e[0] == '0' && e[1] == 0 ? 0 : 1;
+}();
+
+DVIS_EXPORT int dvis_upsample_add_image_set_v2(int on) {
+  if (on < 0) return __atomic_load_n(&g_upsample_v2, __ATOMIC_RELAXED);
+  return __atomic_exchange_n(&g_upsample_v2, on ? 1 : 0, __ATOMIC_RELAXED);
+}
+
+DVIS_EXPORT int dvis_upsample_add_image_v2_supported(int N, int C, int H, int W, int h, int w) {
+  if (N <= 0 || C <= 0 || C % 64 != 0 || H <= 0 || W <= 0 || h <= 0 || w <= 0 || W % 4 != 0) return 0;
+  const int ry = (int)((kUpRows - 1) * (double)h / H + 1e-3) + 3, rx = (int)(31 * (double)w / W + 1e-3) + 3;
+  if ((ry < h ? ry : h) > kUpTR || (rx < w ? rx : w) > kUpTX) return 0;
+  return (int64_t)N * ((H + kUpRows - 1) / kUpRows) <= 65535 && (W + 31) / 32 <= 65535;
+}
+
+static void upsample_add_image_v2_launch(const float *lateral, const float *lat_scale, const float *lat_shift, const float *top,
+                                         int64_t S, int64_t row0, void *image, int N, int C, int H, int W, int h, int w, int oexp,
+                                         void *stream) {
+  const int HB = (H + kUpRows - 1) / kUpRows;
+  const dim3 grid(C / 64, (W + 31) / 32, N * HB);
+  if (S > 0)
+    hipLaunchKernelGGL(upsample_add_image_v2_kernel<true>, grid, dim3(256), 0, (hipStream_t)stream, lateral, top, image, N, C, H, W, h,
+                       w, lat_scale, lat_shift, ldexpf(1.f, oexp), HB, (long long)S, (long long)row0);
+  else
+    hipLaunchKernelGGL(upsample_add_image_v2_kernel<false>, grid, dim3(256), 0, (hipStream_t)stream, lateral, top, image, N, C, H, W, h,
+                       w, lat_scale, lat_shift, ldexpf(1.f, oexp), HB, 0ll, 0ll);
+}
+
+DVIS_EXPORT int dvis_upsample_add_image_tokens(const float *lateral, const float *lat_scale, const float *lat_shift, const float *tokens,
+                                               int64_t S, int64_t row0, void *image, int N, int C, int H, int W, int h, int w, int oexp,
+                                               void *stream) {
+  DVIS_REQUIRE(lateral && tokens && image, "dvis_upsample_add_image_tokens: null pointer");
+  DVIS_REQUIRE((lat_scale == nullptr) == (lat_shift == nullptr), "dvis_upsample_add_image_tokens: scale and shift together");
+  DVIS_REQUIRE(dvis_upsample_add_image_v2_supported(N, C, H, W, h, w), "dvis_upsample_add_image_tokens: (N %d, C %d, %d x %d <- %d x %d) is "
+               "not served (C %% 64 == 0, W %% 4 == 0, up-sampling by about 2 or more)", N, C, H, W, h, w);
+  DVIS_REQUIRE(S > 0 && row0 >= 0 && row0 + (int64_t)h * w <= S, "dvis_upsample_add_image_tokens: rows [%lld, %lld) outside the %lld "
+               "tokens of a frame", (long long)row0, (long long)(row0 + (int64_t)h * w), (long long)S);
+  DVIS_REQUIRE((uintptr_t)lateral % 16 == 0 && (uintptr_t)tokens % 16 == 0, "dvis_upsample_add_image_tokens: lateral and tokens must be "
+               "16-byte aligned");
+  DVIS_REQUIRE((uintptr_t)image % 16 == 0 && dvis_conv_x3_image_bytes(N, C, H, W) < ((int64_t)1 << 31), "dvis_upsample_add_image_tokens: a "
+               "16-byte aligned image below 2 GiB");
+  upsample_add_image_v2_launch(lateral, lat_scale, lat_shift, tokens, S, row0, image, N, C, H, W, h, w, oexp, stream);
+  return dvis_check_launch("dvis_upsample_add_image_tokens");
 }
 
 DVIS_EXPORT int dvis_upsample_add_image(const float *lateral, const float *lat_scale, const float *lat_shift, const float *top, void *image,
@@ -378,6 +541,11 @@
   DVIS_REQUIRE(N > 0 && C > 0 && C % 64 == 0 && H > 0 && W > 0 && h > 0 && w > 0, "dvis_upsample_add_image: bad sizes");
   DVIS_REQUIRE((uintptr_t)image % 16 == 0 && dvis_conv_x3_image_bytes(N, C, H, W) < ((int64_t)1 << 31), "dvis_upsample_add_image: a 16-byte "
                "aligned image below 2 GiB");
+  if (__atomic_load_n(&g_upsample_v2, __ATOMIC_RELAXED) && (uintptr_t)lateral % 16 == 0 &&
+      dvis_upsample_add_image_v2_supported(N, C, H, W, h, w)) {
+    upsample_add_image_v2_launch(lateral, lat_scale, lat_shift, top, 0, 0, image, N, C, H, W, h, w, oexp, stream);
+    return dvis_check_launch("dvis_upsample_add_image");
+  }
   const int per = 16 * 65535 / H;
   DVIS_REQUIRE(per >= 1 && (W + 31) / 32 <= 65535, "dvis_upsample_add_image: map too large (%d x %d)", H, W);
   for (int i = 0; i < N; i += per) {
diff --git a/dvis_plus_amd/csrc/gemm_x3.hip b/dvis_plus_amd/csrc/gemm_x3.hip
--- a/dvis_plus_amd/csrc/gemm_x3.hip
+++ b/dvis_plus_amd/csrc/gemm_x3.hip
@@ -7,18 +7,35 @@
 namespace {
 
 template <int KS>
+__device__ __forceinline__ void load_x_at(const float *p, float s, h8 *xh, h8 *xl, const float *addp = nullptr) {
+  f4 raw[2 * KS];
+#pragma unroll
+  for (int S = 0; S < KS; ++S) raw[2 * S] = *(const f4 *)(p + 16 * S), raw[2 * S + 1] = *(const f4 *)(p + 16 * S + 4);
+  if (addp != nullptr) {
+#pragma unroll
+    for (int S = 0; S < KS; ++S) raw[2 * S] += *(const f4 *)(addp + 16 * S), raw[2 * S + 1] += *(const f4 *)(addp + 16 * S + 4);
+  }
+#pragma unroll
+  for (int S = 0; S < KS; ++S) split8(raw[2 * S], raw[2 * S + 1], s, xh[S], xl[S]);
+}
+template <int KS>
 __device__ __forceinline__ void load_x(const float *x, int64_t ldx, int64_t row, int g, float s, h8 *xh, h8 *xl,
                                        const float *addp = nullptr) {
-  const float *p = x + row * ldx + 8 * g;
-  f4 raw[2 * KS];
-#pragma unroll
-  for (int S = 0; S < KS; ++S) raw[2 * S] = *(const f4 *)(p + 16 * S), raw[2 * S + 1] = *(const f4 *)(p + 16 * S + 4);
-  if (addp != nullptr) {
-#pragma unroll
-    for (int S = 0; S < KS; ++S) raw[2 * S] += *(const f4 *)(addp + 16 * S), raw[2 * S + 1] += *(const f4 *)(addp + 16 * S + 4);
-  }
-#pragma unroll
-  for (int S = 0; S < KS; ++S) split8(raw[2 * S], raw[2 * S + 1], s, xh[S], xl[S]);
+  load_x_at<KS>(x + row * ldx + 8 * g, s, xh, xl, addp);
+}
+
+struct X3Rows {
+  unsigned rows_per_batch;
+  int64_t batch_stride;
+};
+template <bool ROWS>
+__device__ __forceinline__ const float *x3_row(const float *x, int64_t ldx, int64_t row, X3Rows rm) {
+  if constexpr (ROWS) {
+    const unsigned b = (unsigned)row / rm.rows_per_batch;
+    return x + (int64_t)b * rm.batch_stride + (int64_t)((unsigned)row - b * rm.rows_per_batch) * ldx;
+  } else {
+    return x + row * ldx;
+  }
 }
 
 __device__ __forceinline__ void store_block(char *scr, int lane, const f4 *v, float *dst, int64_t ld, int rows_valid,
@@ -156,10 +173,11 @@
   }
 }
 
-template <int NB>
+template <int NB, bool ROWS = false>
 __global__ __launch_bounds__(kThreads) void x3_linear_kernel(const float *__restrict__ x, int64_t ldx, int64_t M,
                                                              const void *__restrict__ wp, float xscale, int npass,
-                                                             const float *__restrict__ xadd, int64_t xadd_rows, EpiArgs e) {
+                                                             const float *__restrict__ xadd, int64_t xadd_rows, EpiArgs e,
+                                                             X3Rows rm) {
   extern __shared__ __attribute__((aligned(1024))) char lds[];
   constexpr int K = 256, KS = K / 16, NI = K / 32;
   const int wave = threadIdx.x >> 6, lane = threadIdx.x & 63, j = lane & 31, g = lane >> 5;
@@ -176,7 +194,7 @@
     const int64_t tok0 = tile * kTileTok + wave * 32;
     const int64_t row = tok0 + j < M ? tok0 + j : M - 1;
     h8 xh[KS], xl[KS];
-    load_x<KS>(x, ldx, row, g, xscale, xh, xl, xadd ? xadd + (row % xadd_rows) * K + 8 * g : nullptr);
+    load_x_at<KS>(x3_row<ROWS>(x, ldx, row, rm) + 8 * g, xscale, xh, xl, xadd ? xadd + (row % xadd_rows) * K + 8 * g : nullptr);
     for (int pass = 0; pass < npass; ++pass) {
       f16v acc[NB];
 #pragma unroll
@@ -196,10 +214,11 @@
 
 constexpr int x3_stream_layout_blocks(int nb) { return 4 * nb % 8 == 0 ? nb : nb + 1; }
 
-template <int NB, bool LN, bool EX = false, bool ADD = false>
+template <int NB, bool LN, bool EX = false, bool ADD = false, bool ROWS = false>
 __global__ __launch_bounds__(512) void x3_linear_stream_kernel(const float *__restrict__ x, int64_t ldx, int64_t M, int K,
                                                                const void *__restrict__ wp, float xscale, int npass,
-                                                               const float *__restrict__ xadd, int64_t xadd_rows, EpiArgs e) {
+                                                               const float *__restrict__ xadd, int64_t xadd_rows, EpiArgs e,
+                                                               X3Rows rm) {
   extern __shared__ __attribute__((aligned(1024))) char lds[];
   constexpr int NBL = x3_stream_layout_blocks(NB);
   constexpr int NW = 8, PW = 4 * NBL / NW, kTile = NW * 32;
@@ -240,12 +259,12 @@
       }
     };
     int64_t r0 = row_of(blockIdx.x);
-    const float *rowp = x + r0 * ldx + 8 * g, *posp = xadd + (r0 % xadd_rows) * K + 8 * g;
+    const float *rowp = x3_row<ROWS>(x, ldx, r0, rm) + 8 * g, *posp = xadd + (r0 % xadd_rows) * K + 8 * g;
     load_raw(rowp, posp, 0);
     for (int64_t tile = blockIdx.x; tile < ntiles; tile += gridDim.x) {
       const int64_t tok0 = tile * kTile + wave * 32;
       const int64_t rn = row_of(tile + gridDim.x < ntiles ? tile + gridDim.x : tile);
-      const float *nrowp = x + rn * ldx + 8 * g, *nposp = xadd + (rn % xadd_rows) * K + 8 * g;
+      const float *nrowp = x3_row<ROWS>(x, ldx, rn, rm) + 8 * g, *nposp = xadd + (rn % xadd_rows) * K + 8 * g;
       for (int pass = 0; pass < npass; ++pass) {
         f16v acc[NB];
 #pragma unroll
@@ -279,7 +298,7 @@
 #pragma unroll
     for (int s = 0; s < 4; ++s) raw[2 * s] = *(const f4 *)(rowp + 64 * kc + 16 * s), raw[2 * s + 1] = *(const f4 *)(rowp + 64 * kc + 16 * s + 4);
   };
-  auto row_ptr = [&](int64_t tile) { return x + row_of(tile) * ldx + 8 * g; };
+  auto row_ptr = [&](int64_t tile) { return x3_row<ROWS>(x, ldx, row_of(tile), rm) + 8 * g; };
   const float *rowp = row_ptr(blockIdx.x);
   load_raw(rowp, 0);
   for (int64_t tile = blockIdx.x; tile < ntiles; tile += gridDim.x) {
@@ -518,7 +537,7 @@
 
 static int x3_linear_impl(const float *x, int64_t ldx, int64_t M, int K, const void *wp, int N, int xexp, int wexp, const float *xadd,
                           int64_t xadd_rows, const float *bias, int relu, float *out, int64_t ldo, void *stream,
-                          const float *radd = nullptr, int64_t ldr = 0);
+                          const float *radd = nullptr, int64_t ldr = 0, int64_t rows_per_batch = 0, int64_t batch_stride = 0);
 
 DVIS_EXPORT int dvis_x3_linear(const float *x, int64_t ldx, int64_t M, int K, const void *wp, int N, int xexp, int wexp,
                                const float *bias, int relu, float *out, int64_t ldo, void *stream) {
@@ -541,9 +560,38 @@
   return x3_linear_impl(x, ldx, M, K, wp, N, xexp, wexp, nullptr, 0, bias, act, out, ldo, stream, res, ldres);
 }
 
+static int x3_check_rows(const char *what, int64_t ldx, int64_t M, int K, int64_t rows_per_batch, int64_t batch_stride) {
+  DVIS_REQUIRE(rows_per_batch > 0 && rows_per_batch < ((int64_t)1 << 31) && M % rows_per_batch == 0,
+               "%s: M = %lld must be a whole number of batches of rows_per_batch = %lld rows", what, (long long)M, (long long)rows_per_batch);
+  DVIS_REQUIRE(ldx >= K, "%s: row stride %lld below K = %d", what, (long long)ldx, K);
+  DVIS_REQUIRE(batch_stride % 4 == 0 && batch_stride >= rows_per_batch * ldx && batch_stride < ((int64_t)1 << 40),
+               "%s: batch_stride = %lld must be a multiple of 4 floats and at least rows_per_batch * ldx", what, (long long)batch_stride);
+  return DVIS_OK;
+}
+
+DVIS_EXPORT int dvis_x3_linear_rows(const float *x, int64_t ldx, int64_t rows_per_batch, int64_t batch_stride, int64_t M, int K,
+                                    const void *wp, int N, int xexp, int wexp, const float *bias, int relu, float *out, int64_t ldo,
+                                    void *stream) {
+  const int rc = x3_check_rows("dvis_x3_linear_rows", ldx, M, K, rows_per_batch, batch_stride);
+  if (rc != DVIS_OK) return rc;
+  DVIS_REQUIRE(relu == 0 || relu == 1, "dvis_x3_linear_rows: relu must be 0 or 1");
+  return x3_linear_impl(x, ldx, M, K, wp, N, xexp, wexp, nullptr, 0, bias, relu, out, ldo, stream, nullptr, 0, rows_per_batch, batch_stride);
+}
+
+DVIS_EXPORT int dvis_x3_linear_add_rows(const float *x, int64_t ldx, int64_t rows_per_batch, int64_t batch_stride, int64_t M, int K,
+                                        const void *wp, int N, int xexp, int wexp, const float *xadd, int64_t xadd_rows,
+                                        const float *bias, int relu, float *out, int64_t ldo, void *stream) {
+  const int rc = x3_check_rows("dvis_x3_linear_add_rows", ldx, M, K, rows_per_batch, batch_stride);
+  if (rc != DVIS_OK) return rc;
+  DVIS_REQUIRE(relu == 0 || relu == 1, "dvis_x3_linear_add_rows: relu must be 0 or 1");
+  DVIS_REQUIRE(xadd && xadd_rows > 0 && (uintptr_t)xadd % 16 == 0, "dvis_x3_linear_add_rows: xadd (xadd_rows x K, 16-byte aligned) is required");
+  DVIS_REQUIRE(K == 256 && dvis_x3_linear_supported(N, K, 0), "dvis_x3_linear_add_rows: served for K = 256 (N %d, K %d)", N, K);
+  return x3_linear_impl(x, ldx, M, K, wp, N, xexp, wexp, xadd, xadd_rows, bias, relu, out, ldo, stream, nullptr, 0, rows_per_batch, batch_stride);
+}
+
 static int x3_linear_impl(const float *x, int64_t ldx, int64_t M, int K, const void *wp, int N, int xexp, int wexp, const float *xadd,
                           int64_t xadd_rows, const float *bias, int relu, float *out, int64_t ldo, void *stream, const float *radd,
-                          int64_t ldr) {
+                          int64_t ldr, int64_t rows_per_batch, int64_t batch_stride) {
   DVIS_REQUIRE(dvis_x3_linear_supported(N, K, 0), "dvis_x3_linear: (N, K) = (%d, %d) is not served (K %% 64 == 0; N in 128 / 192 / 256 or N %% 256 == 0; N = 288 at K = 256)", N, K);
   const int rc = x3_check_common(x, ldx, M, wp, out, ldo);
   if (rc != DVIS_OK) return rc;
@@ -557,36 +605,43 @@
   hipStream_t st = (hipStream_t)stream;
   int NB;
   const int npass = x3_passes(N, &NB);
-#define DVIS_X3_STREAM_FORM(NBV, LNV, EXV, ADDV, XADD, XROWS, WHAT, LDS_EXTRA)                                        \
+  const bool rows = rows_per_batch > 0;
+  const X3Rows rm = {(unsigned)rows_per_batch, batch_stride};
+#define DVIS_X3_STREAM_FORM(NBV, LNV, EXV, ADDV, ROWSV, XADD, XROWS, WHAT, LDS_EXTRA)                                      \
   {                                                                                                                  \
     static DvisLdsOptIn opted;                                                                                       \
     typedef Ring<4 * x3_stream_layout_blocks(NBV) / 8, 8, 8> R;                                                      \
     const size_t lds_bytes = kStages * R::kItemBytes + 8 * kScratch + (LDS_EXTRA);                                   \
-    const int rc2 = dvis_lds_opt_in((const void *)x3_linear_stream_kernel<NBV, LNV, EXV, ADDV>, lds_bytes, &opted, WHAT);  \
+    const int rc2 = dvis_lds_opt_in((const void *)x3_linear_stream_kernel<NBV, LNV, EXV, ADDV, ROWSV>, lds_bytes, &opted, WHAT);  \
     if (rc2 != DVIS_OK) return rc2;                                                                                  \
     const int64_t ntiles = (M + 255) / 256;                                                                          \
-    hipLaunchKernelGGL((x3_linear_stream_kernel<NBV, LNV, EXV, ADDV>), dim3(x3_grid(ntiles)), dim3(512), lds_bytes, st, x, ldx, M, K, wp, \
-                       xs, npass, XADD, XROWS, e);                                                                   \
+    hipLaunchKernelGGL((x3_linear_stream_kernel<NBV, LNV, EXV, ADDV, ROWSV>), dim3(x3_grid(ntiles)), dim3(512), lds_bytes, st, x, ldx, M, K, wp, \
+                       xs, npass, XADD, XROWS, e, rm);                                                               \
     return dvis_check_launch(WHAT);                                                                                  \
   }
-#define DVIS_X3_STREAM_EX(NBV, LNV, EXV, WHAT, LDS_EXTRA) DVIS_X3_STREAM_FORM(NBV, LNV, EXV, false, (const float *)nullptr, (int64_t)0, WHAT, LDS_EXTRA)
+#define DVIS_X3_STREAM_EX(NBV, LNV, EXV, WHAT, LDS_EXTRA) DVIS_X3_STREAM_FORM(NBV, LNV, EXV, false, false, (const float *)nullptr, (int64_t)0, WHAT, LDS_EXTRA)
 #define DVIS_X3_STREAM(NBV, LNV, WHAT, LDS_EXTRA) DVIS_X3_STREAM_EX(NBV, LNV, false, WHAT, LDS_EXTRA)
-#define DVIS_X3_RESIDENT(NBV)                                                                                        \
+#define DVIS_X3_RESIDENT(NBV, ROWSV)                                                                                 \
   {                                                                                                                  \
     static DvisLdsOptIn opted;                                                                                       \
-    return x3_launch(x3_linear_kernel<NBV>, &opted, kStages * Ring<NBV>::kItemBytes + kWaves * kScratch + (size_t)N * 4, \
-                     M, st, "dvis_x3_linear", x, ldx, M, wp, xs, npass, xadd, xadd_rows, e);                         \
+    return x3_launch(x3_linear_kernel<NBV, ROWSV>, &opted, kStages * Ring<NBV>::kItemBytes + kWaves * kScratch + (size_t)N * 4, \
+                     M, st, "dvis_x3_linear", x, ldx, M, wp, xs, npass, xadd, xadd_rows, e, rm);                     \
   }
   if (relu == 2 || radd) {
     DVIS_REQUIRE(NB == 8 && !xadd, "dvis_x3_linear_res: the GELU / residual epilogue is served for N %% 256 == 0 (N = %d)", N);
     DVIS_X3_STREAM_EX(8, false, true, "dvis_x3_linear_res", (size_t)N * 4)
   }
+  if (rows) {
+    DVIS_REQUIRE(NB == 8 && relu != 2 && !radd, "dvis_x3_linear_rows: served for N %% 256 == 0 (N = %d)", N);
+    if (xadd) DVIS_X3_RESIDENT(8, true)
+    DVIS_X3_STREAM_FORM(8, false, false, false, true, (const float *)nullptr, (int64_t)0, "dvis_x3_linear_rows", (size_t)N * 4)
+  }
   if (xadd) {
     switch (NB) {
-      case 4: DVIS_X3_RESIDENT(4)
-      case 6: DVIS_X3_RESIDENT(6)
-      case 8: DVIS_X3_RESIDENT(8)
-      default: DVIS_X3_STREAM_FORM(9, false, false, true, xadd, xadd_rows, "dvis_x3_linear_add", (size_t)N * 4)
+      case 4: DVIS_X3_RESIDENT(4, false)
+      case 6: DVIS_X3_RESIDENT(6, false)
+      case 8: DVIS_X3_RESIDENT(8, false)
+      default: DVIS_X3_STREAM_FORM(9, false, false, true, false, xadd, xadd_rows, "dvis_x3_linear_add", (size_t)N * 4)
     }
   }
   switch (NB) {
@@ -617,6 +672,7 @@
   e.flag = gd.flag, e.tag = gd.tag;
   const float xs = x3_pow2(xexp);
   const int npass = 1;
+  const X3Rows rm = {};
   hipStream_t st = (hipStream_t)stream;
   DVIS_X3_STREAM(8, true, "dvis_x3_linear_ln", (size_t)3 * 256 * 4)
 #undef DVIS_X3_STREAM
diff --git a/dvis_plus_amd/functions.py b/dvis_plus_amd/functions.py
--- a/dvis_plus_amd/functions.py
+++ b/dvis_plus_amd/functions.py
@@ -1745,8 +1745,43 @@
     return x2, ld
 
 
+X3_LINEAR_ROWS = os.environ.get("DVIS_X3_LINEAR_ROWS", "1") != "0"
+
+
+def x3_rows_in_place(x, N):
+    return (X3_LINEAR_ROWS and x.dim() == 3 and not x.is_contiguous() and x.shape[0] > 0 and x.shape[1] > 0 and N % 256 == 0
+            and x.stride(2) == 1 and x.stride(1) == x.shape[2] and x.stride(0) % 4 == 0 and x.stride(0) >= x.shape[1] * x.shape[2]
+            and x.data_ptr() % 16 == 0)
+
+
+def _x3_linear_rows(x, weight, bias, relu, xexp, xadd):
+    N, K = weight.shape
+    B, S, _ = x.shape
+    buf, wexp = x3_pack(weight)
+    out = torch.empty((B, S, N), dtype=torch.float32, device=x.device)
+    lib = native.lib()
+    bptr = None if bias is None else native.dev_ptr(bias.detach(), "bias")
+    xe = X3_XEXP if xexp is None else xexp
+    with torch.cuda.device(x.device):
+        if xadd is not None:
+            if xadd.numel() != S * K or xadd.dtype != torch.float32 or not xadd.is_cuda:
+                raise RuntimeError("x3_linear: xadd must be a float32 GPU (S, K) embedding for x of shape (B, S, K)")
+            xadd = xadd.contiguous()
+            native.check(lib.dvis_x3_linear_add_rows(
+                ctypes.c_void_p(x.data_ptr()), K, S, x.stride(0), B * S, K, ctypes.c_void_p(buf.data_ptr()), N, xe, wexp,
+                ctypes.c_void_p(xadd.data_ptr()), S, bptr, int(relu), ctypes.c_void_p(out.data_ptr()), N,
+                native.stream_ptr(x.device)), "dvis_x3_linear_add_rows")
+        else:
+            native.check(lib.dvis_x3_linear_rows(
+                ctypes.c_void_p(x.data_ptr()), K, S, x.stride(0), B * S, K, ctypes.c_void_p(buf.data_ptr()), N, xe, wexp,
+                bptr, int(relu), ctypes.c_void_p(out.data_ptr()), N, native.stream_ptr(x.device)), "dvis_x3_linear_rows")
+    return out
+
+
 def x3_linear(x, weight, bias, relu=False, xexp=None, xadd=None, act=None, residual=None):
     N, K = weight.shape
+    if act is None and residual is None and x3_rows_in_place(x, N):
+        return _x3_linear_rows(x, weight, bias, relu, xexp, xadd)
     x2, ldx = _x3_rows(x, "x")
     buf, wexp = x3_pack(weight)
     out = torch.empty((*x.shape[:-1], N), dtype=torch.float32, device=x.device)
@@ -2118,11 +2153,30 @@
     return max(1, min(N, (2 ** 31 - 1) // per))
 
 
+def _token_major_rows(top):
+    N, C, h, w = top.shape
+    if not (top.stride(1) == 1 and top.stride(3) == C and top.stride(2) == w * C and top.data_ptr() % 16 == 0):
+        return 0
+    if N == 1:
+        return h * w
+    return top.stride(0) // C if top.stride(0) % C == 0 and top.stride(0) >= h * w * C else 0
+
+
+def upsample_add_image_reads_tokens(lateral, top):
+    N, C, H, W = lateral.shape
+    lib = native.lib()
+    return bool(lateral.is_cuda and top.is_cuda and top.dtype == torch.float32 and not top.is_contiguous() and _token_major_rows(top)
+                and lateral.data_ptr() % 16 == 0 and lib.dvis_upsample_add_image_set_v2(-1)
+                and lib.dvis_upsample_add_image_v2_supported(N, C, H, W, top.shape[-2], top.shape[-1]))
+
+
 def upsample_add_image(lateral, top, lat_affine=None, oexp=None):
     N, C, H, W = lateral.shape
     lib = native.lib()
     oe = X3_CONV_XEXP if oexp is None else oexp
-    top = top.contiguous()
+    S = _token_major_rows(top) if upsample_add_image_reads_tokens(lateral, top) else 0
+    if not S:
+        top = top.contiguous()
     data = torch.empty(lib.dvis_conv_x3_image_bytes(N, C, H, W), dtype=torch.uint8, device=lateral.device)
     img = OperandImage(data, N, C, H, W, oe)
     step = _image_chunks(N, C, C, H, W, H, W)
@@ -2131,6 +2185,12 @@
             n = min(step, N - i)
             sc = None if lat_affine is None else native.dev_ptr(lat_affine[0].reshape(N, C)[i:i + n], "scale")
             sh = None if lat_affine is None else native.dev_ptr(lat_affine[1].reshape(N, C)[i:i + n], "shift")
+            if S:
+                native.check(lib.dvis_upsample_add_image_tokens(
+                    native.dev_ptr(lateral[i:i + n], "lateral"), sc, sh, ctypes.c_void_p(top[i:i + n].data_ptr()), S, 0,
+                    ctypes.c_void_p(img.images(i, n).data_ptr()), n, C, H, W, top.shape[-2], top.shape[-1], oe,
+                    native.stream_ptr(lateral.device)), "dvis_upsample_add_image_tokens")
+                continue
             native.check(lib.dvis_upsample_add_image(native.dev_ptr(lateral[i:i + n], "lateral"), sc, sh, native.dev_ptr(top[i:i + n], "top"),
                                                      ctypes.c_void_p(img.images(i, n).data_ptr()), n, C, H, W, top.shape[-2], top.shape[-1], oe,
                                                      native.stream_ptr(lateral.device)), "dvis_upsample_add_image")
diff --git a/dvis_plus_amd/native.py b/dvis_plus_amd/native.py
--- a/dvis_plus_amd/native.py
+++ b/dvis_plus_amd/native.py
@@ -108,6 +108,8 @@
     "dvis_x3_tile_linear": (_i, [_p, _i64, _i64, _i, _p, _i, _i, _i, _p, _i, _p, _i64, _p, _i64, _p]),
     "dvis_x3_linear_res": (_i, [_p, _i64, _i64, _i, _p, _i, _i, _i, _p, _i, _p, _i64, _p, _i64, _p]),
     "dvis_x3_linear_add": (_i, [_p, _i64, _i64, _i, _p, _i, _i, _i, _p, _i64, _p, _i, _p, _i64, _p]),
+    "dvis_x3_linear_rows": (_i, [_p, _i64, _i64, _i64, _i64, _i, _p, _i, _i, _i, _p, _i, _p, _i64, _p]),
+    "dvis_x3_linear_add_rows": (_i, [_p, _i64, _i64, _i64, _i64, _i, _p, _i, _i, _i, _p, _i64, _p, _i, _p, _i64, _p]),
     "dvis_x3_linear_ln": (_i, [_p, _i64, _i64, _i, _p, _i, _i, _i, _p, _p, _i64, _p, _p, _f, _p, _i64, _p, _p, _i64, _p]),
     "dvis_x3_ffn_packed_bytes": (_i64, [_i, _i, _i]),
     "dvis_x3_ffn_pack": (_i, [_p, _i64, _p, _i64, _i, _i, _i, _i, _i, _p, _p]),
@@ -131,6 +133,9 @@
     "dvis_conv_x3_pack_image": (_i, [_p, _i, _i, _i, _i, _p, _p]),
     "dvis_conv_x3_image": (_i, [_p, _p, _p, _p, _p, _p, _p, _i, _i, _i, _i, _i, _i, _i, _i, _i, _i, _i, _p, _p]),
     "dvis_upsample_add_image": (_i, [_p, _p, _p, _p, _p, _i, _i, _i, _i, _i, _i, _i, _p]),
+    "dvis_upsample_add_image_v2_supported": (_i, [_i, _i, _i, _i, _i, _i]),
+    "dvis_upsample_add_image_set_v2": (_i, [_i]),
+    "dvis_upsample_add_image_tokens": (_i, [_p, _p, _p, _p, _i64, _i64, _p, _i, _i, _i, _i, _i, _i, _i, _p]),
     "dvis_gemm_num_configs": (_i, []),
     "dvis_gemm_pick_config": (_i, [_i, _i, _i, _i]),
     "dvis_gemm_pick_config_nw": (_i, [_i, _i, _i, _i, _i]),
diff --git a/dvis_plus_amd/pixel_decoder.py b/dvis_plus_amd/pixel_decoder.py
--- a/dvis_plus_amd/pixel_decoder.py
+++ b/dvis_plus_amd/pixel_decoder.py
@@ -499,13 +499,11 @@
             with Fn.x3_stage("encoder"):
                 y, _, _, shapes_py = self.transformer(srcs, pos, affines)
             bs = y.shape[0]
-            out, tokens, start = [], [], 0
+            memory, out, tokens, start = y, [], [], 0
             for li, (h, w) in enumerate(shapes_py):
                 tokens.append(y[:, start:start + h * w])
-                if li + 1 == len(shapes_py) and self.num_fpn_levels > 0:
-                    out.append(Fn.tokens_to_map(y, start, h, w))
-                else:
-                    out.append(tokens[-1].transpose(1, 2).reshape(bs, -1, h, w))
+                out.append(tokens[-1].transpose(1, 2).reshape(bs, -1, h, w))
+                finest = (start, h, w)
                 start += h * w
             with Fn.x3_stage("mask_path"):
                 deferred = None
@@ -513,8 +511,11 @@
                     x = features[f].float().contiguous()
                     cur_fpn, affine = self.lateral_convs[idx].conv_and_affine(x)
                     oc = self.output_convs[idx]
-                    if cur_fpn.is_cuda and cur_fpn.dtype == torch.float32 and cur_fpn.is_contiguous() and out[-1].dtype == torch.float32 \
-                            and oc.image_input_ok(*cur_fpn.shape, cur_fpn.device):
+                    as_image = cur_fpn.is_cuda and cur_fpn.dtype == torch.float32 and cur_fpn.is_contiguous() \
+                        and out[-1].dtype == torch.float32 and oc.image_input_ok(*cur_fpn.shape, cur_fpn.device)
+                    if idx == 0 and not (as_image and Fn.upsample_add_image_reads_tokens(cur_fpn, out[-1])):
+                        out[-1] = Fn.tokens_to_map(memory, *finest)
+                    if as_image:
                         last = idx + 1 == self.num_fpn_levels and len(out) >= self.maskformer_num_feature_levels
                         y = oc(Fn.upsample_add_image(cur_fpn, out[-1], affine), defer_to=self.mask_features if last else None)
                         if isinstance(y, tuple):
diff --git a/dvis_plus_amd/transformer_decoder.py b/dvis_plus_amd/transformer_decoder.py
--- a/dvis_plus_amd/transformer_decoder.py
+++ b/dvis_plus_amd/transformer_decoder.py
@@ -263,7 +263,8 @@
                     tok = tokens[lvl]
                     pos_t = self.pe_layer.compute(h, w, tok.device).flatten(2).transpose(1, 2)
                     if Fn.x3_on() and Fn.x3_ok(tok, Wk.shape[0], Wk.shape[1], add=True):
-                        tok = tok.contiguous()
+                        if not Fn.x3_rows_in_place(tok, Wk.shape[0]):
+                            tok = tok.contiguous()
                         kall = Fn.x3_linear(tok, Wk, bk, xadd=pos_t + le).transpose(0, 1)
                         vall = Fn.x3_linear(tok, Wv, bv_le).transpose(0, 1)
                     else:
diff --git a/include/dvis_hip.h b/include/dvis_hip.h
--- a/include/dvis_hip.h
+++ b/include/dvis_hip.h
@@ -210,6 +210,11 @@
                    const float *bias, int relu, float *out, int64_t ldo, void *stream);
 int dvis_x3_linear_add(const float *x, int64_t ldx, int64_t M, int K, const void *packed, int N, int xexp, int wexp,
                        const float *xadd, int64_t xadd_rows, const float *bias, int relu, float *out, int64_t ldo, void *stream);
+int dvis_x3_linear_rows(const float *x, int64_t ldx, int64_t rows_per_batch, int64_t batch_stride, int64_t M, int K, const void *packed,
+                        int N, int xexp, int wexp, const float *bias, int relu, float *out, int64_t ldo, void *stream);
+int dvis_x3_linear_add_rows(const float *x, int64_t ldx, int64_t rows_per_batch, int64_t batch_stride, int64_t M, int K,
+                            const void *packed, int N, int xexp, int wexp, const float *xadd, int64_t xadd_rows, const float *bias,
+                            int relu, float *out, int64_t ldo, void *stream);
 int dvis_x3_linear_res(const float *x, int64_t ldx, int64_t M, int K, const void *wp, int N, int xexp, int wexp, const float *bias, int act,
                        const float *res, int64_t ldres, float *out, int64_t ldo, void *stream);
 
@@ -264,6 +269,10 @@
                        double *gn_part);
 int dvis_upsample_add_image(const float *lateral, const float *lat_scale, const float *lat_shift, const float *top, void *image, int N,
                             int C, int H, int W, int h, int w, int oexp, void *stream);
+int dvis_upsample_add_image_v2_supported(int N, int C, int H, int W, int h, int w);
+int dvis_upsample_add_image_set_v2(int on);
+int dvis_upsample_add_image_tokens(const float *lateral, const float *lat_scale, const float *lat_shift, const float *tokens, int64_t S,
+                                   int64_t row0, void *image, int N, int C, int H, int W, int h, int w, int oexp, void *stream);
 int dvis_x3_ffn_pack(const float *W1, int64_t ldw1, const float *W2, int64_t ldw2, int K, int H, int N, int w1exp, int w2exp,
                      void *packed, void *stream);
 int dvis_x3_ffn_ln(const float *x, int64_t ldx, int64_t M, int K, int H, int N, const void *packed, int xexp, int w1exp,
```
